# DiltheyLab/MetaMaps

Hardware: AMD Instinct MI355X
Metric: Gbp long reads mapped+classified per sec (whole node), miniSeq+H DB (higher is better)
Workload: dtype u32

## Files before the change

### include/metamaps_hip.h

```cpp
#ifndef METAMAPS_HIP_H
#define METAMAPS_HIP_H

#include <stddef.h>
#include <stdint.h>

#ifdef __cplusplus
extern "C" {
#endif

#define MM_ABI_VERSION 6

typedef enum {
  MM_OK = 0,
  MM_ERR_ARG = -1,
  MM_ERR_DEVICE = -2,
  MM_ERR_NOMEM = -3,
  MM_ERR_STATE = -4,
  MM_ERR_LIMIT = -5,
  MM_ERR_NUMERIC = -6,
  MM_ERR_COMM = -7,
  MM_ERR_DATA = -8
} mm_status;

typedef struct mm_ctx mm_ctx;
// ... 82 lines not shown
} mm_synth_community_params;
int mm_synth_community(mm_ctx* ctx, const mm_synth_community_params* p, mm_seqset** out, int32_t* contig_genome);
int mm_synth_community_species(const mm_synth_community_params* p, int32_t* genome_species);
int mm_synth_reads(mm_ctx* ctx, const mm_seqset* reference, const mm_synth_read_params* p, mm_seqset** out,
                   int32_t* truth_genome);

int mm_minimizers(mm_ctx* ctx, const mm_seqset* s, int k, int w, int64_t* offsets, uint32_t* hash, int32_t* wpos,
                  int32_t* strand, int64_t cap);

typedef struct {
  int64_t n_contigs, n_entries, n_unique_hashes, n_dup_flagged;
  int64_t hbm_bytes;
} mm_index_info;
int mm_index_build(mm_ctx* ctx, const mm_seqset* contigs, int k, int w, mm_index** out);
void mm_index_destroy(mm_index* idx);
int mm_index_save(mm_index* idx, const char* path);
int mm_index_load(mm_ctx* ctx, const char* path, mm_index** out);
int mm_index_plan_chunks(mm_ctx* ctx, const mm_index* whole, uint64_t max_memory_bytes, int32_t* first_contig, int32_t cap, int32_t* n_chunks);
int mm_index_get_info(const mm_index* idx, mm_index_info* out);
int mm_index_freq_hist(mm_index* idx, int64_t* counts, int64_t* n_hashes, int64_t cap, int64_t* n_out);
int mm_freq_threshold_from_hist(const int64_t* counts, const int64_t* n_hashes, int64_t n, int64_t n_unique_hashes,
                                int prev_threshold);
int mm_index_set_freq_threshold(mm_index* idx, int threshold);
int mm_index_entries(mm_index* idx, uint32_t* hash, int32_t* contig, int32_t* wpos, int32_t* strand, int64_t cap);
int mm_index_dup_neighbours(mm_index* idx, int32_t* prev_dist, int32_t* next_dist, int64_t cap);

int mm_recommended_window(double p_value, int k, float pi, int min_read_len, uint64_t reference_size);
double mm_estimate_pvalue(int s, int k, float pi, int min_read_len, uint64_t reference_size);
int mm_min_hits_relaxed(int s, int k, float pi);
void mm_identity(int shared, int s, int k, float* ident, float* ident_upper );

typedef struct {
  int32_t k, w;
  float perc_identity;
  int32_t min_read_len;
} mm_map_params;

typedef struct {
  int32_t read;
  int32_t ref_contig;
  int32_t ref_start;
  int32_t shared;
  int32_t sketch;
  int32_t strand;
  double mapq;
} mm_map_record;

typedef struct {
  int64_t n_reads, n_reads_long_enough, n_reads_mapped, n_mappings;
  int64_t bases_long_enough;
  int64_t sum_sketch, sum_hits, n_candidates, sum_l2_stream_entries, sum_l2_evals;
  int64_t n_ambiguous_sketch_reads;
  int64_t sum_hits_kept;
  int64_t n_l2_rebuilds;
  int64_t n_l2_wide_redo;
  double ms_minimizer, ms_sketch, ms_probe_gather, ms_sort_hits, ms_l1_scan, ms_l2, ms_compact, ms_total, ms_hit_filter;
  int64_t n_reads_giant;
} mm_map_stats;

int mm_map_batch(mm_ctx* ctx, const mm_index* idx, const mm_seqset* reads, const mm_map_params* p, mm_mapping** out);
int mm_map_batch_phased(mm_ctx* ctx, const mm_index* idx, const mm_seqset* reads, const mm_map_params* p, void (*at_stage)(void* user, int stage), void* user,
                        mm_mapping** out);
int mm_map_batch_reusing(mm_ctx* ctx, const mm_index* idx, const mm_seqset* reads, const mm_map_params* p, const mm_mapping* sketch_of, mm_mapping** out);
int mm_sketch_batch(mm_ctx* ctx, const mm_seqset* reads, const mm_map_params* p, mm_mapping** out);
void mm_mapping_destroy(mm_mapping* m);
int mm_mapping_get_stats(const mm_mapping* m, mm_map_stats* out);
int mm_mapping_release_intermediates(mm_mapping* m);
int mm_mapping_fetch(mm_mapping* m, int64_t* offsets, mm_map_record* records, int64_t cap);
int mm_mapping_add_qualities(mm_ctx* ctx, mm_mapping* m, const mm_seqset* reads, int k);
int mm_mapping_keep_best(mm_ctx* ctx, mm_mapping* m, int k);
int mm_mapping_concat(mm_ctx* ctx, mm_mapping* const* parts, const int32_t* contig_base, int n_parts, mm_mapping** out);
int mm_mapping_from_parts(mm_ctx* ctx, int64_t n_reads, const int32_t* read_len, const mm_map_params* p, int n_parts,
                          const int64_t* const* offsets, const mm_map_record* const* records, const int32_t* contig_base, mm_mapping** out);

int mm_mapping_gather(mm_ctx* ctx, int owner, int64_t n_reads, const int32_t* read_len, const mm_map_params* p, mm_mapping* const* parts, const int32_t* chunk_id,
                      int n_parts, int n_chunks, const int32_t* chunk_rank, const int32_t* contig_base, mm_mapping** out);

int mm_debug_sketch(mm_mapping* m, int64_t* offsets, uint32_t* hash, int32_t* strand, int64_t cap);
int mm_debug_hits(mm_mapping* m, int64_t* offsets, int32_t* contig, int32_t* wpos, int64_t cap);
int mm_debug_candidates(mm_mapping* m, int64_t* offsets, int32_t* triples , int64_t cap);
int mm_debug_l2(mm_mapping* m, int64_t* per_cand , int64_t cap);
int mm_debug_min_hits(mm_mapping* m, int32_t* min_hits );
int mm_debug_probed_lists(mm_mapping* m, const mm_index* idx, int64_t* hist, int32_t n_bins);

int mm_em_create(mm_ctx* ctx, int64_t n_reads, const int64_t* read_off, const int32_t* taxon, const double* mapq,
                 const double* inv_nloc, int32_t n_taxa, mm_em** out);
int mm_em_create_from_mapping(mm_ctx* ctx, const mm_mapping* m, const int32_t* contig_taxon, const int32_t* contig_len, int32_t n_contigs,
                              int32_t n_taxa, mm_em** out);
int mm_em_taxon_counts(mm_em* em, int64_t* counts);
int mm_em_sizes(const mm_em* em, int64_t* n_reads, int64_t* n_entries, int32_t* n_taxa);
void mm_em_destroy(mm_em* em);
int mm_em_iterate(mm_em* em, const double* f, double* f_partial, double* ll_partial);
int mm_em_iterate_allreduce(mm_em* em, const double* f, double* f_next, double* ll);
int mm_em_run(mm_em* em, const double* f0, int max_iter, double* f_out, double* ll_trace, int ll_cap, int* n_iter);
int mm_em_continue(mm_em* em, int max_iter, double* f_out, double* ll_trace, int ll_cap, int* n_iter, int* stopped);
int mm_em_posteriors(mm_em* em, const double* f, double* post , int64_t* best );
int mm_em_bootstrap(mm_em* em, const double* f_start, int32_t rep0, int32_t n_rep, uint64_t seed, const uint8_t* weights,
                    int max_iter, double* f_out, double* ll_out, int32_t* n_iter, int32_t* stopped);
int mm_em_lca(mm_em* em, const double* f, int32_t n_nodes, const int32_t* parent, const int32_t* taxon_node, double threshold,
              int32_t* node_out, double* mass_out, int64_t* direct_out);

int mm_gene_overlap(mm_ctx* ctx, int32_t n_contigs, const int64_t* contig_gene_off, const int32_t* gene_start, const int32_t* gene_stop,
                    const int32_t* gene_group, int32_t n_groups,
                    const int64_t* group_feat_off , const int32_t* group_feat, int32_t n_feats,
                    int64_t n_maps, const int32_t* map_contig, const int32_t* map_start, const int32_t* map_stop, const double* map_ident,
                    int64_t* group_reads , double* group_median ,
                    int64_t* feat_reads , int64_t* maps_on_annotated );

int mm_ident_filter(mm_ctx* ctx, int64_t n_reads, const int64_t* read_off , const int32_t* taxon, const double* ident,
                    const int64_t* best , int32_t n_taxa, double thr_percent,
                    double* sorted_max , int64_t* n_with_entries, int64_t* n_le,
                    int64_t* taxon_reads , double* taxon_median , uint8_t* taxon_removed ,
                    uint8_t* read_removed ,
                    int64_t* read_src, int64_t* entry_src, int64_t* read_off_out, int64_t* n_reads_out, int64_t* n_entries_out);

int mm_edit_infix(mm_ctx* ctx, const mm_seqset* reads, const mm_seqset* reference, int64_t n_jobs, const int32_t* read, const int32_t* strand,
                  const int32_t* contig, const int64_t* ws, const int64_t* we, const int32_t* max_dist,
                  int32_t* dist_out, int64_t* begin_out, int64_t* end_out);
int mm_mapping_edit_distances(mm_ctx* ctx, const mm_mapping* mapping, const mm_seqset* reads, const mm_seqset* reference, float perc_identity,
                              int32_t* dist_out, int64_t* first_out, int64_t* last_out, int64_t cap);

int mm_edit_infix_align(mm_ctx* ctx, const mm_seqset* reads, const mm_seqset* reference, int64_t n_jobs, const int32_t* read, const int32_t* strand,
                        const int32_t* contig, const int64_t* ws, const int64_t* we, const int32_t* max_dist, mm_alignment** out);
int mm_mapping_align(mm_ctx* ctx, const mm_mapping* mapping, const mm_seqset* reads, const mm_seqset* reference, float perc_identity, mm_alignment** out);
int mm_alignment_sizes(const mm_alignment* al, int64_t* n_jobs, int64_t* n_ops);
int mm_alignment_fetch(const mm_alignment* al, int32_t* dist , int64_t* first, int64_t* last, int64_t* op_off , uint32_t* ops );
void mm_alignment_destroy(mm_alignment* al);

int mm_bam_encode(mm_ctx* ctx, const mm_seqset* reads, const mm_seqset* reference, int64_t n_jobs,
                  const int32_t* read, const int32_t* strand, const int32_t* contig,
                  const int32_t* dist, const int64_t* first,
                  const int64_t* op_off , const uint32_t* ops,
                  const uint16_t* flag, const uint8_t* mapq,
                  const int64_t* name_off , const char* names,
                  int64_t group_bytes, mm_bam** out);
int mm_bam_sizes(const mm_bam* bam, int64_t* n_records, int64_t* raw_bytes, int64_t* bgzf_bytes);
int mm_bam_fetch(const mm_bam* bam, uint8_t* bgzf );
void mm_bam_destroy(mm_bam* bam);

#define MM_COMM_ID_BYTES 128
int mm_comm_unique_id(char id[MM_COMM_ID_BYTES]);
int mm_comm_init(mm_ctx* ctx, const char id[MM_COMM_ID_BYTES], int rank, int nranks);
int mm_comm_info(mm_ctx* ctx, int* n_ranks, int* rank);
int mm_comm_share(mm_ctx* ctx, mm_ctx* owner);
int mm_comm_allreduce_f64(mm_ctx* ctx, double* host_inout, int64_t n);
void mm_comm_destroy(mm_ctx* ctx);

#ifdef __cplusplus
}
#endif
#endif
```

### metamaps_amd/capi.py

```python
from __future__ import annotations

import ctypes as C
import os
import re

import numpy as np

_HERE = os.path.dirname(os.path.abspath(__file__))
LIB_PATH = os.path.join(_HERE, "csrc", "libmetamaps_hip.so")
HEADER_PATH = os.path.join(os.path.dirname(_HERE), "include", "metamaps_hip.h")

COMM_ID_BYTES = 128
MM_ERR_ARG = -1
MM_ERR_LIMIT = -5
MM_ERR_DATA = -8


class MMError(RuntimeError):
    def __init__(self, status: int, msg: str):
        super().__init__(f"libmetamaps_hip status {status}: {msg}")
        self.status = status


SEED_STAGE_CB = C.CFUNCTYPE(None, C.c_void_p, C.c_int)
# ... 64 lines not shown
            raise FileNotFoundError(f"{path} is missing — run `python -c 'import __graft_entry__ as g; g.build()'`")
        L = C.CDLL(path)
        vp, i32, i64, u64, f32, f64 = C.c_void_p, C.c_int32, C.c_int64, C.c_uint64, C.c_float, C.c_double
        P = C.POINTER
        sig = {
            "mm_abi_version": (C.c_int, []),
            "mm_ctx_release_cached": (C.c_int, [vp]),
            "mm_device_count": (C.c_int, []),
            "mm_ctx_create": (C.c_int, [C.c_int, P(vp)]),
            "mm_ctx_destroy": (None, [vp]),
            "mm_last_error": (C.c_char_p, [vp]),
            "mm_ctx_device_info": (C.c_int, [vp, C.c_char_p, C.c_size_t, P(C.c_int), P(u64), P(u64)]),
            "mm_ctx_synchronize": (C.c_int, [vp]),
            "mm_ctx_stream": (vp, [vp]),
            "mm_seqset_create": (C.c_int, [vp, P(vp)]),
            "mm_seqset_destroy": (None, [vp]),
            "mm_seqset_add": (C.c_int, [vp, C.c_char_p, i64]),
            "mm_seqset_add_view": (C.c_int, [vp, C.c_char_p, i64]),
            "mm_seqset_add_nt16": (C.c_int, [vp, C.c_char_p, i64, C.c_int]),
            "mm_bgzf_inflate": (C.c_int, [vp, C.c_char_p, i64, vp, vp, C.c_int32, vp, i64, vp, vp]),
            "mm_bgzf_deflate_bound": (i64, [i64]),
            "mm_bgzf_deflate": (C.c_int, [vp, C.c_char_p, i64, vp, i64, P(i64), P(C.c_int32)]),
            "mm_gzip_open": (C.c_int, [vp, i64, i64, P(vp)]),
            "mm_gzip_feed": (C.c_int, [vp, C.c_char_p, i64, C.c_int, P(i64)]),
            "mm_gzip_read": (C.c_int, [vp, vp, i64, P(i64)]),
            "mm_gzip_stats": (C.c_int, [vp, P(i64), P(f64)]),
            "mm_gzip_close": (None, [vp]),
            "mm_seqset_save": (C.c_int, [vp, C.c_char_p]),
            "mm_seqset_load": (C.c_int, [vp, C.c_char_p, P(vp)]),
            "mm_seqset_upload": (C.c_int, [vp]),
            "mm_seqset_slice": (C.c_int, [vp, vp, i64, i64, P(vp)]),
            "mm_seqset_concat": (C.c_int, [vp, P(vp), C.c_int, P(vp)]),
            "mm_seqset_count": (i64, [vp]),
            "mm_seqset_total_bases": (i64, [vp]),
            "mm_seqset_lengths": (C.c_int, [vp, vp]),
            "mm_seqset_fetch": (C.c_int, [vp, i64, C.c_char_p, i64]),
            "mm_seqset_fetch_range": (C.c_int, [vp, i64, i64, C.c_void_p, i64]),
            "mm_seqset_hpc": (C.c_int, [vp, vp, P(vp), P(vp)]),
            "mm_hpc_map_to_raw": (C.c_int, [vp, vp, vp, i64, vp, vp]),
            "mm_hpc_map_lengths": (C.c_int, [vp, vp, vp]),
            "mm_hpc_map_device_bytes": (i64, [vp]),
            "mm_mapping_to_raw": (C.c_int, [vp, vp, vp, vp, i64]),
            "mm_hpc_map_destroy": (None, [vp]),
            "mm_synth_reference": (C.c_int, [vp, P(SynthRefParams), P(vp)]),
            "mm_synth_reads": (C.c_int, [vp, vp, P(SynthReadParams), P(vp), vp]),
            "mm_synth_community": (C.c_int, [vp, P(SynthCommunityParams), P(vp), vp]),
            "mm_synth_community_species": (C.c_int, [P(SynthCommunityParams), vp]),
            "mm_minimizers": (C.c_int, [vp, vp, C.c_int, C.c_int, vp, vp, vp, vp, i64]),
            "mm_index_build": (C.c_int, [vp, vp, C.c_int, C.c_int, P(vp)]),
            "mm_index_save": (C.c_int, [vp, C.c_char_p]),
            "mm_index_load": (C.c_int, [vp, C.c_char_p, P(vp)]),
            "mm_index_destroy": (None, [vp]),
            "mm_index_get_info": (C.c_int, [vp, P(IndexInfo)]),
            "mm_index_freq_hist": (C.c_int, [vp, vp, vp, i64, P(i64)]),
            "mm_freq_threshold_from_hist": (C.c_int, [vp, vp, i64, i64, C.c_int]),
            "mm_index_set_freq_threshold": (C.c_int, [vp, C.c_int]),
            "mm_index_entries": (C.c_int, [vp, vp, vp, vp, vp, i64]),
            "mm_index_dup_neighbours": (C.c_int, [vp, vp, vp, i64]),
            "mm_recommended_window": (C.c_int, [f64, C.c_int, f32, C.c_int, u64]),
            "mm_estimate_pvalue": (f64, [C.c_int, C.c_int, f32, C.c_int, u64]),
            "mm_min_hits_relaxed": (C.c_int, [C.c_int, C.c_int, f32]),
            "mm_identity": (None, [C.c_int, C.c_int, C.c_int, P(f32), P(f32)]),
            "mm_map_batch": (C.c_int, [vp, vp, vp, P(MapParams), P(vp)]),
            "mm_map_batch_phased": (C.c_int, [vp, vp, vp, P(MapParams), SEED_STAGE_CB, vp, P(vp)]),
            "mm_map_batch_reusing": (C.c_int, [vp, vp, vp, P(MapParams), vp, P(vp)]),
            "mm_sketch_batch": (C.c_int, [vp, vp, P(MapParams), P(vp)]),
            "mm_mapping_destroy": (None, [vp]),
            "mm_mapping_get_stats": (C.c_int, [vp, P(MapStats)]),
            "mm_comm_info": (C.c_int, [vp, C.POINTER(C.c_int), C.POINTER(C.c_int)]),
            "mm_mapping_gather": (C.c_int, [vp, C.c_int, i64, vp, vp, vp, vp, C.c_int, C.c_int, vp, vp, vp]),
            "mm_mapping_release_intermediates": (C.c_int, [vp]),
            "mm_mapping_fetch": (C.c_int, [vp, vp, vp, i64]),
            "mm_mapping_add_qualities": (C.c_int, [vp, vp, vp, C.c_int]),
            "mm_mapping_concat": (C.c_int, [vp, P(vp), vp, C.c_int, P(vp)]),
            "mm_mapping_keep_best": (C.c_int, [vp, vp, C.c_int]),
            "mm_mapping_from_parts": (C.c_int, [vp, i64, vp, P(MapParams), C.c_int, P(vp), P(vp), vp, P(vp)]),
            "mm_index_plan_chunks": (C.c_int, [vp, vp, u64, vp, i32, P(i32)]),
            "mm_debug_sketch": (C.c_int, [vp, vp, vp, vp, i64]),
            "mm_debug_hits": (C.c_int, [vp, vp, vp, vp, i64]),
            "mm_debug_candidates": (C.c_int, [vp, vp, vp, i64]),
            "mm_debug_l2": (C.c_int, [vp, vp, i64]),
            "mm_debug_min_hits": (C.c_int, [vp, vp]),
            "mm_debug_probed_lists": (C.c_int, [vp, vp, vp, i32]),
            "mm_em_create": (C.c_int, [vp, i64, vp, vp, vp, vp, i32, P(vp)]),
            "mm_em_create_from_mapping": (C.c_int, [vp, vp, vp, vp, i32, i32, P(vp)]),
            "mm_em_taxon_counts": (C.c_int, [vp, vp]),
            "mm_em_sizes": (C.c_int, [vp, P(i64), P(i64), P(i32)]),
            "mm_em_destroy": (None, [vp]),
            "mm_em_iterate": (C.c_int, [vp, vp, vp, P(f64)]),
            "mm_em_iterate_allreduce": (C.c_int, [vp, vp, vp, P(f64)]),
            "mm_em_posteriors": (C.c_int, [vp, vp, vp, vp]),
            "mm_em_run": (C.c_int, [vp, vp, C.c_int, vp, vp, C.c_int, P(C.c_int)]),
            "mm_em_continue": (C.c_int, [vp, C.c_int, vp, vp, C.c_int, P(C.c_int), P(C.c_int)]),
            "mm_em_bootstrap": (C.c_int, [vp, vp, i32, i32, u64, vp, C.c_int, vp, vp, vp, vp]),
            "mm_em_lca": (C.c_int, [vp, vp, i32, vp, vp, f64, vp, vp, vp]),
            "mm_gene_overlap": (C.c_int, [vp, i32, vp, vp, vp, vp, i32, vp, vp, i32, i64, vp, vp, vp, vp, vp, vp, vp, P(i64)]),
            "mm_ident_filter": (C.c_int, [vp, i64, vp, vp, vp, vp, i32, f64, vp, P(i64), P(i64), vp, vp, vp, vp, vp, vp, vp, P(i64), P(i64)]),
            "mm_edit_infix": (C.c_int, [vp, vp, vp, i64, vp, vp, vp, vp, vp, vp, vp, vp, vp]),
            "mm_mapping_edit_distances": (C.c_int, [vp, vp, vp, vp, f32, vp, vp, vp, i64]),
            "mm_edit_infix_align": (C.c_int, [vp, vp, vp, i64, vp, vp, vp, vp, vp, vp, vp]),
            "mm_mapping_align": (C.c_int, [vp, vp, vp, vp, f32, vp]),
            "mm_alignment_sizes": (C.c_int, [vp, vp, vp]),
            "mm_alignment_fetch": (C.c_int, [vp, vp, vp, vp, vp, vp]),
            "mm_alignment_destroy": (None, [vp]),
            "mm_bam_encode": (C.c_int, [vp, vp, vp, i64, vp, vp, vp, vp, vp, vp, vp, vp, vp, vp, vp, i64, vp]),
            "mm_bam_sizes": (C.c_int, [vp, vp, vp, vp]),
            "mm_bam_fetch": (C.c_int, [vp, vp]),
            "mm_bam_destroy": (None, [vp]),
            "mm_comm_unique_id": (C.c_int, [C.c_char_p]),
            "mm_comm_init": (C.c_int, [vp, C.c_char_p, C.c_int, C.c_int]),
            "mm_comm_allreduce_f64": (C.c_int, [vp, vp, i64]),
            "mm_comm_share": (C.c_int, [vp, vp]),
            "mm_comm_destroy": (None, [vp]),
        }
        for name, (res, args) in sig.items():
            fn = getattr(L, name)
            fn.restype = res
            fn.argtypes = args
        _lib = L
    return _lib


def _ptr(a):
    return None if a is None else a.ctypes.data_as(C.c_void_p)


class Context:
    def __init__(self, device: int = 0):
        self.h = C.c_void_p()
        st = lib().mm_ctx_create(device, C.byref(self.h))
        if st != 0:
            raise MMError(st, "mm_ctx_create failed (no gfx950 GPU visible? this library has no CPU fallback)")

    def check(self, st: int):
        if st != 0:
            raise MMError(st, lib().mm_last_error(self.h).decode(errors="replace"))

    def close(self):
        if self.h:
            lib().mm_ctx_destroy(self.h)
            self.h = C.c_void_p()

    def device_info(self) -> dict:
        name = C.create_string_buffer(256)
        cus = C.c_int()
        tot, free = C.c_uint64(), C.c_uint64()
        self.check(lib().mm_ctx_device_info(self.h, name, 256, C.byref(cus), C.byref(tot), C.byref(free)))
        return {"name": name.value.decode(), "cus": cus.value, "hbm_total": tot.value, "hbm_free": free.value}

    def release_cached(self):
        self.check(lib().mm_ctx_release_cached(self.h))

    def synchronize(self):
        self.check(lib().mm_ctx_synchronize(self.h))

    @property
    def stream(self) -> int:
        return lib().mm_ctx_stream(self.h) or 0

    def seqset(self, seqs) -> "SeqSet":
        h = C.c_void_p()
        self.check(lib().mm_seqset_create(self.h, C.byref(h)))
        s = SeqSet(self, h)
        for q in seqs:
            if isinstance(q, str):
                q = q.encode()
# ... 632 lines not shown
```

### metamaps_amd/csrc/mm_api.hip

```cpp
#include "mm_env.hpp"
#include "mm_map.hpp"
#include "mm_em.hpp"
#include "mm_stats.hpp"
#include "mm_synth.hpp"
#include "mm_hpc.hpp"
#include "mm_lca.hpp"
#include "mm_gene.hpp"
#include "mm_ident.hpp"
#include "mm_edit.hpp"
#include "mm_bam.hpp"
#include <chrono>
#include <new>
#include <rccl/rccl.h>
#include "mm_prims.hpp"

namespace mm {
void seqset_upload(mm_seqset* s);
void seqset_upload_nt16(mm_seqset* s);
int64_t bgzf_inflate(mm_ctx* ctx, const uint8_t* comp, int64_t comp_bytes, const int64_t* comp_off, const int32_t* comp_len, int32_t n,
                     uint8_t* out, int64_t out_cap, const int64_t* out_off, int32_t* status);
void bgzf_deflate(mm_ctx* ctx, const uint8_t* in, int64_t in_bytes, uint8_t* out, int64_t out_cap, int64_t* out_bytes, int32_t* n_blocks);
int64_t bgzf_deflate_bound(int64_t in_bytes);
mm_gzip* gzip_open(mm_ctx* ctx, int64_t chunk, int64_t segment);
void gzip_close(mm_gzip* g);
// ... 12 lines not shown
namespace {
void bind(mm_ctx* ctx) {
  if (ctx->device >= 0 && ctx->stream) (void)hipSetDevice(ctx->device);
  mm::current_stream() = ctx->stream; mm::current_alloc() = &ctx->alloc;
}
template <typename F>
int guarded(mm_ctx* ctx, F&& f) {
  if (ctx) bind(ctx);
  try { f(); return MM_OK; }
  catch (const mm::Error& e) { if (ctx) ctx->err = e.what(); return e.status; }
  catch (const std::bad_alloc&) { if (ctx) ctx->err = "host allocation failed"; return MM_ERR_NOMEM; }
  catch (const std::exception& e) { if (ctx) ctx->err = e.what(); return MM_ERR_DEVICE; }
}
}

extern "C" {

int mm_abi_version(void) { return MM_ABI_VERSION; }

namespace {
struct CtxTrace {
  const bool on = getenv("MM_CTX_TRACE") != nullptr;
  std::chrono::steady_clock::time_point t = std::chrono::steady_clock::now();
  void lap(const char* what) {
    if (!on) return;
    const auto n = std::chrono::steady_clock::now();
    fprintf(stderr, "MM_CTX_TRACE %s %.3f ms\n", what, std::chrono::duration<double, std::milli>(n - t).count());
    t = n;
  }
};
}

int mm_device_count(void) {
  int n = 0;
  CtxTrace tr;
  if (hipGetDeviceCount(&n) != hipSuccess) { (void)hipGetLastError(); return 0; }
  tr.lap("hipGetDeviceCount");
  return n;
}
int mm_ctx_create(int device_id, mm_ctx** out) {
  if (!out) return MM_ERR_ARG;
  *out = nullptr;
  if (mm::env_strict()) {
    const std::string bad = mm::env_unknown();
    if (!bad.empty()) { fprintf(stderr, "mm_ctx_create: unknown MM_* environment switch(es): %s (MM_STRICT_ENV is set; the table is metamaps_amd/csrc/mm_env.hpp / INTEGRATION.md)\n", bad.c_str()); return MM_ERR_ARG; }
  }
  int n = 0;
  if (hipGetDeviceCount(&n) != hipSuccess || n <= 0) return MM_ERR_DEVICE;
  if (device_id < 0 || device_id >= n) return MM_ERR_ARG;
  mm_ctx* c = new (std::nothrow) mm_ctx;
  if (!c) return MM_ERR_NOMEM;
  c->device = device_id;
  int st = guarded(c, [&] {
    CtxTrace tr;
    MM_HIP(hipSetDevice(device_id));
    tr.lap("hipSetDevice");
    hipDeviceProp_t p;
    MM_HIP(hipGetDeviceProperties(&p, device_id));
    tr.lap("hipGetDeviceProperties");
    MM_REQUIRE(std::string(p.gcnArchName).rfind("gfx950", 0) == 0, MM_ERR_DEVICE,
               std::string("device is ") + p.gcnArchName + ", this library is built for gfx950 only");
    c->cus = p.multiProcessorCount;
    MM_HIP(hipStreamCreateWithFlags(&c->stream, hipStreamNonBlocking));
    mm::stream_event_register(c->stream);
    tr.lap("hipStreamCreateWithFlags");
    if (tr.on) { void* q = nullptr; if (hipMalloc(&q, 1 << 20) == hipSuccess) { tr.lap("first hipMalloc (1 MiB)"); (void)hipFree(q); } }
    c->alloc.stream = c->stream;
    mm::alloc_register(&c->alloc, c->device);
  });
  if (st != MM_OK) { delete c; return st; }
  *out = c;
  return MM_OK;
}
void mm_ctx_destroy(mm_ctx* ctx) {
  if (!ctx) return;
  mm::alloc_unregister(&ctx->alloc);
  (void)hipSetDevice(ctx->device);
  (void)mm::stream_sync(ctx->stream);
  ctx->alloc.trim();
  mm::big_pool_trim(ctx->device);
  mm::comm_destroy(ctx);
  if (ctx->pinned) (void)hipHostFree(ctx->pinned);
  if (ctx->pinned_up) (void)hipHostFree(ctx->pinned_up);
  ctx->l2_codes.release(); ctx->l2_masks.release();
  if (ctx->ev_fork) (void)hipEventDestroy(ctx->ev_fork);
  if (ctx->ev_join) (void)hipEventDestroy(ctx->ev_join);
  if (ctx->aux_stream) { mm::stream_event_unregister(ctx->aux_stream); (void)hipStreamDestroy(ctx->aux_stream); }
  if (ctx->stream) { mm::stream_event_unregister(ctx->stream); (void)hipStreamDestroy(ctx->stream); }
  delete ctx;
}
const char* mm_last_error(const mm_ctx* ctx) { return ctx ? ctx->err.c_str() : "null context"; }
int mm_ctx_device_info(mm_ctx* ctx, char* name, size_t name_cap, int* cus, uint64_t* hbm_total, uint64_t* hbm_free) {
  if (!ctx) return MM_ERR_ARG;
  return guarded(ctx, [&] {
    MM_HIP(hipSetDevice(ctx->device));
    hipDeviceProp_t p;
    MM_HIP(hipGetDeviceProperties(&p, ctx->device));
    if (name && name_cap) { snprintf(name, name_cap, "%s (%s)", p.name, p.gcnArchName); }
    if (cus) *cus = p.multiProcessorCount;
    size_t f = 0, t = 0;
    MM_HIP(mm::dev_mem_info(&f, &t));
    if (hbm_total) *hbm_total = t;
    if (hbm_free) *hbm_free = f;
  });
}
int mm_ctx_synchronize(mm_ctx* ctx) {
  if (!ctx) return MM_ERR_ARG;
  return guarded(ctx, [&] { MM_HIP(mm::stream_sync(ctx->stream)); });
}
int mm_ctx_release_cached(mm_ctx* ctx) {
  if (!ctx) return MM_ERR_ARG;
  return guarded(ctx, [&] { MM_HIP(hipSetDevice(ctx->device)); ctx->alloc.trim(); mm::big_pool_trim(ctx->device); });
}
void* mm_ctx_stream(mm_ctx* ctx) { return ctx ? (void*)ctx->stream : nullptr; }

int mm_seqset_create(mm_ctx* ctx, mm_seqset** out) {
  if (!ctx || !out) return MM_ERR_ARG;
  return guarded(ctx, [&] { auto* s = new mm_seqset; s->ctx = ctx; *out = s; });
}
void mm_seqset_destroy(mm_seqset* s) { if (s) { bind(s->ctx); delete s; } }
int mm_seqset_add(mm_seqset* s, const char* ascii, int64_t len) {
  if (!s || (!ascii && len > 0) || len < 0) return MM_ERR_ARG;
  return guarded(s->ctx, [&] {
    MM_REQUIRE(!s->frozen, MM_ERR_STATE, "sequence set already uploaded");
    MM_REQUIRE(s->staged_kind != 2, MM_ERR_STATE, "this sequence set holds 4-bit codes (mm_seqset_add_nt16): ASCII cannot join it");
    s->staged_kind = 1;
    s->owned.emplace_back(ascii ? ascii : "", (size_t)len);
    s->staged.emplace_back(s->owned.back().data(), (size_t)len);
  });
}
int mm_seqset_add_view(mm_seqset* s, const char* ascii, int64_t len) {
  if (!s || (!ascii && len > 0) || len < 0) return MM_ERR_ARG;
  return guarded(s->ctx, [&] {
    MM_REQUIRE(!s->frozen, MM_ERR_STATE, "sequence set already uploaded");
    MM_REQUIRE(s->staged_kind != 2, MM_ERR_STATE, "this sequence set holds 4-bit codes (mm_seqset_add_nt16): ASCII cannot join it");
    s->staged_kind = 1;
    s->staged.emplace_back(ascii, (size_t)len);
  });
}
int mm_seqset_add_nt16(mm_seqset* s, const uint8_t* nt16, int64_t n_bases, int reverse) {
  if (!s || (!nt16 && n_bases > 0) || n_bases < 0) return MM_ERR_ARG;
  return guarded(s->ctx, [&] {
    MM_REQUIRE(!s->frozen, MM_ERR_STATE, "sequence set already uploaded");
    MM_REQUIRE(s->staged_kind != 1, MM_ERR_STATE, "this sequence set holds ASCII sequences: 4-bit codes (mm_seqset_add_nt16) cannot join it");
    s->staged_kind = 2;
    s->staged.emplace_back((const char*)nt16, (size_t)n_bases);
    s->staged_rev.push_back(reverse ? 1 : 0);
  });
}
int mm_bgzf_inflate(mm_ctx* ctx, const uint8_t* comp, int64_t comp_bytes, const int64_t* comp_off, const int32_t* comp_len, int32_t n,
                    uint8_t* out, int64_t out_cap, const int64_t* out_off, int32_t* status) {
  if (!ctx || n < 0 || comp_bytes < 0 || out_cap < 0 || (n > 0 && (!comp || !comp_off || !comp_len || !out_off)) || (!out && out_cap > 0)) return MM_ERR_ARG;
  int64_t bad = 0;
  const int rc = guarded(ctx, [&] { MM_HIP(hipSetDevice(ctx->device)); bad = mm::bgzf_inflate(ctx, comp, comp_bytes, comp_off, comp_len, n, out, out_cap, out_off, status); });
  if (rc != MM_OK) return rc;
  if (bad) { ctx->err = "mm_bgzf_inflate: " + std::to_string(bad) + " corrupt BGZF block(s)"; return MM_ERR_DATA; }
  return MM_OK;
}
int64_t mm_bgzf_deflate_bound(int64_t in_bytes) { return in_bytes < 0 ? 0 : mm::bgzf_deflate_bound(in_bytes); }
int mm_bgzf_deflate(mm_ctx* ctx, const uint8_t* in, int64_t in_bytes, uint8_t* out, int64_t out_cap, int64_t* out_bytes, int32_t* n_blocks) {
  if (!ctx || !out_bytes || !n_blocks || in_bytes < 0 || (in_bytes > 0 && (!in || !out))) return MM_ERR_ARG;
  return guarded(ctx, [&] { MM_HIP(hipSetDevice(ctx->device)); mm::bgzf_deflate(ctx, in, in_bytes, out, out_cap, out_bytes, n_blocks); });
}
int mm_gzip_open(mm_ctx* ctx, int64_t chunk_bytes, int64_t segment_bytes, mm_gzip** out) {
  if (!ctx || !out || chunk_bytes < 0 || segment_bytes < 0) return MM_ERR_ARG;
  *out = nullptr;
// ... 566 lines not shown
    m->n_rec = (int64_t)kept.size();
    m->rec.alloc(std::max<size_t>(kept.size(), 1)); m->rec.upload(kept.data(), kept.size(), ctx->stream);
    m->rec_off.upload(off.data(), off.size(), ctx->stream);
    m->h_rec_off = off;
    m->stats.n_mappings = m->n_rec; m->stats.n_reads_mapped = mapped;
    MM_HIP(mm::stream_sync(ctx->stream));
  });
}

int mm_debug_sketch(mm_mapping* m, int64_t* offsets, uint32_t* hash, int32_t* strand, int64_t cap) {
  if (m && m->released) return MM_ERR_STATE;
  if (!m) return MM_ERR_ARG;
  return guarded(m->ctx, [&] {
    hipStream_t st = m->ctx->stream;
    int64_t tot = 0;
    for (int64_t r = 0; r < m->n_reads; ++r) { if (offsets) offsets[r] = tot; tot += m->h_sk_n[(size_t)r]; }
    if (offsets) offsets[m->n_reads] = tot;
    if (!hash && !strand) return;
    MM_REQUIRE(cap >= tot, MM_ERR_ARG, "output capacity too small");
    auto hh = m->sk_hash.to_host(st); auto hs = m->sk_strand.to_host(st);
    int64_t o = 0;
    for (int64_t r = 0; r < m->n_reads; ++r)
      for (int i = 0; i < m->h_sk_n[(size_t)r]; ++i, ++o) {
        size_t src = (size_t)m->mz.h_off[(size_t)r] + (size_t)i;
        if (hash) hash[o] = hh[src];
        if (strand) strand[o] = (hs[src] & 1) ? 1 : -1;
      }
  });
}
int mm_debug_hits(mm_mapping* m, int64_t* offsets, int32_t* contig, int32_t* wpos, int64_t cap) {
  if (m && m->released) return MM_ERR_STATE;
  if (!m) return MM_ERR_ARG;
  return guarded(m->ctx, [&] {
    const int64_t tot = (int64_t)m->h_read_hit_off[(size_t)m->n_reads];
    if (offsets) for (size_t i = 0; i < m->h_read_hit_off.size(); ++i) offsets[i] = (int64_t)m->h_read_hit_off[i];
    if (!contig && !wpos) return;
    MM_REQUIRE(cap >= tot, MM_ERR_ARG, "output capacity too small");
    auto h = m->hits.to_host(m->ctx->stream, (size_t)tot);
    for (int64_t i = 0; i < tot; ++i) {
      if (contig) contig[i] = (int32_t)(h[(size_t)i] >> 32);
      if (wpos) wpos[i] = mm::pw_wpos((uint32_t)h[(size_t)i]);
    }
  });
}
int mm_debug_candidates(mm_mapping* m, int64_t* offsets, int32_t* triples, int64_t cap) {
  if (m && m->released) return MM_ERR_STATE;
  if (!m) return MM_ERR_ARG;
  return guarded(m->ctx, [&] {
    if (offsets) for (size_t i = 0; i < m->h_cand_off.size(); ++i) offsets[i] = (int64_t)m->h_cand_off[i];
    if (!triples) return;
    MM_REQUIRE(cap >= m->n_cand, MM_ERR_ARG, "output capacity too small");
    m->cand.download(triples, (size_t)(3 * m->n_cand), m->ctx->stream);
    MM_HIP(mm::stream_sync(m->ctx->stream));
  });
}
int mm_debug_l2(mm_mapping* m, int64_t* per_cand, int64_t cap) {
  if (m && m->released) return MM_ERR_STATE;
  if (!m || !per_cand) return MM_ERR_ARG;
  return guarded(m->ctx, [&] {
    MM_REQUIRE(cap >= m->n_cand, MM_ERR_ARG, "output capacity too small");
    auto h = m->l2.to_host(m->ctx->stream, (size_t)m->n_cand);
    for (int64_t i = 0; i < m->n_cand; ++i) {
      per_cand[6 * i] = h[(size_t)i].contig; per_cand[6 * i + 1] = h[(size_t)i].mean_pos; per_cand[6 * i + 2] = h[(size_t)i].shared;
      per_cand[6 * i + 3] = h[(size_t)i].opt_beg; per_cand[6 * i + 4] = h[(size_t)i].opt_end; per_cand[6 * i + 5] = h[(size_t)i].accepted;
    }
  });
}
int mm_debug_min_hits(mm_mapping* m, int32_t* min_hits) {
  if (m && m->released) return MM_ERR_STATE;
  if (!m || !min_hits) return MM_ERR_ARG;
  memcpy(min_hits, m->h_min_hits.data(), m->h_min_hits.size() * sizeof(int32_t));
  return MM_OK;
}

int mm_debug_probed_lists(mm_mapping* m, const mm_index* idx, int64_t* hist, int32_t n_bins) {
  if (m && m->released) return MM_ERR_STATE;
  if (!m || !idx || !hist || n_bins < 3) return MM_ERR_ARG;
  return guarded(m->ctx, [&] {
    MM_HIP(hipSetDevice(m->ctx->device));
    mm::probed_list_hist(m->ctx, idx, m, n_bins, hist);
  });
}

int mm_em_create(mm_ctx* ctx, int64_t n_reads, const int64_t* read_off, const int32_t* taxon, const double* mapq, const double* inv_nloc,
                 int32_t n_taxa, mm_em** out) {
  if (!ctx || !read_off || !out || n_reads < 0 || n_taxa <= 0) return MM_ERR_ARG;
  return guarded(ctx, [&] {
    MM_HIP(hipSetDevice(ctx->device));
    auto* E = new mm_em;
    try { mm::em_create(ctx, n_reads, read_off, taxon, mapq, inv_nloc, n_taxa, E); } catch (...) { delete E; throw; }
    *out = E;
  });
}
int mm_em_create_from_mapping(mm_ctx* ctx, const mm_mapping* m, const int32_t* contig_taxon, const int32_t* contig_len, int32_t n_contigs,
                              int32_t n_taxa, mm_em** out) {
  if (!ctx || !m || !contig_taxon || !contig_len || !out || n_contigs < 0 || n_taxa <= 0) return MM_ERR_ARG;
  return guarded(ctx, [&] {
    MM_HIP(hipSetDevice(ctx->device));
    auto* E = new mm_em;
    try { mm::em_create_from_mapping(ctx, m, contig_taxon, contig_len, n_contigs, n_taxa, E); } catch (...) { delete E; throw; }
    *out = E;
  });
}
int mm_em_taxon_counts(mm_em* em, int64_t* counts) {
  if (!em || !counts) return MM_ERR_ARG;
  return guarded(em->ctx, [&] {
    auto ts = em->tstart.to_host(em->ctx->stream, (size_t)em->n_taxa + 1);
    for (int32_t t = 0; t < em->n_taxa; ++t) counts[t] = ts[(size_t)t + 1] - ts[(size_t)t];
  });
}
int mm_em_sizes(const mm_em* em, int64_t* n_reads, int64_t* n_entries, int32_t* n_taxa) {
  if (!em) return MM_ERR_ARG;
  if (n_reads) *n_reads = em->n_reads;
  if (n_entries) *n_entries = em->n_entries;
  if (n_taxa) *n_taxa = em->n_taxa;
  return MM_OK;
}
void mm_em_destroy(mm_em* em) { if (em) { bind(em->ctx); delete em; } }
int mm_em_iterate(mm_em* em, const double* f, double* f_partial, double* ll_partial) {
  if (!em || !f || !f_partial || !ll_partial) return MM_ERR_ARG;
  return guarded(em->ctx, [&] { MM_HIP(hipSetDevice(em->ctx->device)); mm::em_iterate(em, f, f_partial, ll_partial); });
}
int mm_em_iterate_allreduce(mm_em* em, const double* f, double* f_next, double* ll) {
  if (!em || !f || !f_next || !ll) return MM_ERR_ARG;
  return guarded(em->ctx, [&] { MM_HIP(hipSetDevice(em->ctx->device)); mm::em_iterate_allreduce(em, f, f_next, ll); });
}
int mm_em_run(mm_em* em, const double* f0, int max_iter, double* f_out, double* ll_trace, int ll_cap, int* n_iter) {
  if (!em || !f0 || max_iter <= 0 || !n_iter) return MM_ERR_ARG;
  return guarded(em->ctx, [&] { MM_HIP(hipSetDevice(em->ctx->device)); *n_iter = mm::em_run(em, f0, max_iter, f_out, ll_trace, ll_cap, nullptr); });
}
int mm_em_continue(mm_em* em, int max_iter, double* f_out, double* ll_trace, int ll_cap, int* n_iter, int* stopped) {
  if (!em || max_iter <= 0 || !n_iter) return MM_ERR_ARG;
  return guarded(em->ctx, [&] {
    MM_HIP(hipSetDevice(em->ctx->device));
    bool st = false;
    *n_iter = mm::em_run(em, nullptr, max_iter, f_out, ll_trace, ll_cap, &st);
    if (stopped) *stopped = st ? 1 : 0;
  });
}
int mm_em_posteriors(mm_em* em, const double* f, double* post, int64_t* best) {
  if (!em || !f) return MM_ERR_ARG;
  return guarded(em->ctx, [&] { MM_HIP(hipSetDevice(em->ctx->device)); mm::em_posteriors(em, f, post, best); });
}
int mm_em_bootstrap(mm_em* em, const double* f_start, int32_t rep0, int32_t n_rep, uint64_t seed, const uint8_t* weights,
                    int max_iter, double* f_out, double* ll_out, int32_t* n_iter, int32_t* stopped) {
  if (!em || !f_start || n_rep <= 0 || rep0 < 0 || (int64_t)rep0 + n_rep - 1 > INT32_MAX || max_iter <= 0 || !f_out || !ll_out || !n_iter || !stopped) return MM_ERR_ARG;
  return guarded(em->ctx, [&] { MM_HIP(hipSetDevice(em->ctx->device)); mm::boot_run(em, f_start, rep0, n_rep, seed, weights, max_iter, f_out, ll_out, n_iter, stopped); });
}
int mm_em_lca(mm_em* em, const double* f, int32_t n_nodes, const int32_t* parent, const int32_t* taxon_node, double threshold,
              int32_t* node_out, double* mass_out, int64_t* direct_out) {
  if (!em || !f || !parent || !taxon_node || !node_out || n_nodes <= 0) return MM_ERR_ARG;
  return guarded(em->ctx, [&] { MM_HIP(hipSetDevice(em->ctx->device)); mm::lca_run(em, f, n_nodes, parent, taxon_node, threshold, node_out, mass_out, direct_out); });
}
int mm_gene_overlap(mm_ctx* ctx, int32_t n_contigs, const int64_t* contig_gene_off, const int32_t* gene_start, const int32_t* gene_stop,
                    const int32_t* gene_group, int32_t n_groups, const int64_t* group_feat_off, const int32_t* group_feat, int32_t n_feats,
                    int64_t n_maps, const int32_t* map_contig, const int32_t* map_start, const int32_t* map_stop, const double* map_ident,
                    int64_t* group_reads, double* group_median, int64_t* feat_reads, int64_t* maps_on_annotated) {
  if (!ctx) return MM_ERR_ARG;
  return guarded(ctx, [&] {
    MM_HIP(hipSetDevice(ctx->device));
    MM_REQUIRE(n_contigs >= 0 && n_groups >= 0 && n_feats >= 0 && n_maps >= 0 && contig_gene_off && group_feat_off, MM_ERR_ARG, "mm_gene_overlap: a negative size or no offsets");
    const int64_t ng = n_contigs > 0 ? contig_gene_off[n_contigs] : 0;
    MM_REQUIRE((ng <= 0 || (gene_start && gene_stop && gene_group)) && (n_maps == 0 || (map_contig && map_start && map_stop && map_ident)) &&
               (n_groups == 0 || (group_reads && group_median)) && (group_feat_off[n_groups] <= 0 || group_feat), MM_ERR_ARG, "mm_gene_overlap: a null array");
    mm::gene_overlap_run(ctx, mm::GeneIn{n_contigs, contig_gene_off, gene_start, gene_stop, gene_group, n_groups, group_feat_off, group_feat, n_feats,
                                         n_maps, map_contig, map_start, map_stop, map_ident}, group_reads, group_median, feat_reads, maps_on_annotated);
// ... 141 lines not shown
```

### metamaps_amd/csrc/mm_common.hpp

```cpp
#pragma once
#include <hip/hip_runtime.h>
#include <cstdint>
#include <cstdio>
#include <cstdlib>
#include <cstring>
#include <string>
#include <deque>
#include <vector>
#include <stdexcept>
#include <memory>
#include <chrono>
#include <map>
#include <iterator>
#include <mutex>
#include <atomic>
#include <algorithm>
#include "../../include/metamaps_hip.h"
#include "mm_slab.hpp"
#include "task_pool.hpp"
#include "cpu_budget.hpp"

namespace mm {

struct Error : std::runtime_error {
// ... 23 lines not shown
__host__ __device__ inline int32_t pw_strand(uint32_t pw) { return (pw & PW_STRAND) ? 1 : -1; }

__host__ __device__ inline uint64_t rotl64(uint64_t v, int r) { return (v << r) | (v >> (64 - r)); }
__host__ __device__ inline uint64_t fmix64(uint64_t v) {
  v ^= v >> 33; v *= 0xff51afd7ed558ccdULL;
  v ^= v >> 33; v *= 0xc4ceb9fe1a85ec53ULL;
  v ^= v >> 33;
  return v;
}
constexpr uint64_t MUR_C1 = 0x87c37b91114253d5ULL, MUR_C2 = 0x4cf5ad432745937fULL;
constexpr uint32_t MUR_SEED = 42u;

__host__ __device__ inline uint32_t murmur16(uint64_t lo, uint64_t hi) {
  uint64_t a = MUR_SEED, b = MUR_SEED;
  lo *= MUR_C1; lo = rotl64(lo, 31); lo *= MUR_C2; a ^= lo;
  a = rotl64(a, 27); a += b; a = a * 5 + 0x52dce729;
  hi *= MUR_C2; hi = rotl64(hi, 33); hi *= MUR_C1; b ^= hi;
  b = rotl64(b, 31); b += a; b = b * 5 + 0x38495ab5;
  a ^= 16; b ^= 16;
  a += b; b += a;
  a = fmix64(a); b = fmix64(b);
  a += b;
  return (uint32_t)a;
}
template <bool REV>
__host__ __device__ inline uint32_t murmur_bytes(const uint8_t* p, int k) {
  auto at = [&](int i) -> uint64_t { return REV ? p[-i] : p[i]; };
  uint64_t a = MUR_SEED, b = MUR_SEED;
  int nb = k >> 4;
  for (int blk = 0; blk < nb; ++blk) {
    uint64_t lo = 0, hi = 0;
    for (int j = 0; j < 8; ++j) { lo |= at(16 * blk + j) << (8 * j); hi |= at(16 * blk + 8 + j) << (8 * j); }
    lo *= MUR_C1; lo = rotl64(lo, 31); lo *= MUR_C2; a ^= lo;
    a = rotl64(a, 27); a += b; a = a * 5 + 0x52dce729;
    hi *= MUR_C2; hi = rotl64(hi, 33); hi *= MUR_C1; b ^= hi;
    b = rotl64(b, 31); b += a; b = b * 5 + 0x38495ab5;
  }
  int rem = k & 15, base = nb << 4;
  uint64_t lo = 0, hi = 0;
  for (int j = 8; j < rem; ++j) hi |= at(base + j) << (8 * (j - 8));
  if (rem > 8) { hi *= MUR_C2; hi = rotl64(hi, 33); hi *= MUR_C1; b ^= hi; }
  for (int j = 0; j < rem && j < 8; ++j) lo |= at(base + j) << (8 * j);
  if (rem > 0) { lo *= MUR_C1; lo = rotl64(lo, 31); lo *= MUR_C2; a ^= lo; }
  a ^= (uint64_t)k; b ^= (uint64_t)k;
  a += b; b += a;
  a = fmix64(a); b = fmix64(b);
  a += b;
  return (uint32_t)a;
}

__host__ __device__ inline uint8_t ascii_of_code(uint32_t c) {
  return (uint8_t)(0x41 + 2 * (c & 1) + 6 * (c >> 1) + 11 * ((c & 1) & (c >> 1)));
}
__host__ __device__ inline uint8_t complement_ascii(uint8_t c) {
  return c == 'A' ? 'T' : c == 'T' ? 'A' : c == 'C' ? 'G' : c == 'G' ? 'C' : c;
}

inline int64_t ceil_div(int64_t a, int64_t b) { return (a + b - 1) / b; }

}

struct mm_ctx {
  int device = -1;
  hipStream_t stream = nullptr;
  hipStream_t aux_stream = nullptr;
  hipEvent_t ev_fork = nullptr, ev_join = nullptr;
  void aux_ready() {
    if (aux_stream) return;
    MM_HIP(hipStreamCreateWithFlags(&aux_stream, hipStreamNonBlocking));
    mm::stream_event_register(aux_stream);
    MM_HIP(hipEventCreateWithFlags(&ev_fork, hipEventDisableTiming));
    MM_HIP(hipEventCreateWithFlags(&ev_join, hipEventDisableTiming));
  }
  mm::DevAlloc alloc;
  std::string err;
  int cus = 0;
  void* comm = nullptr;
  bool comm_shared = false;
  int comm_rank = 0, comm_size = 1;
  std::shared_ptr<void> lut_cache;
  int lut_k = 0; float lut_pi = 0;
  mm::GrowBuf l2_codes, l2_masks;
  void* pinned = nullptr; size_t pinned_bytes = 0;
  void* pinned_up = nullptr; size_t pinned_up_bytes = 0;
  std::unique_ptr<TaskPool> pack_pool;
  void* pinned_up_at_least(size_t bytes) {
    if (bytes > pinned_up_bytes) {
      if (pinned_up) { MM_HIP(mm::stream_sync(stream)); (void)hipHostFree(pinned_up); }
      pinned_up = nullptr; pinned_up_bytes = 0;
      const size_t want = bytes + bytes / 8;
      MM_HIP(hipHostMalloc(&pinned_up, want, hipHostMallocDefault));
      pinned_up_bytes = want;
    }
    return pinned_up;
  }
  void* pinned_at_least(size_t bytes) {
    if (bytes > pinned_bytes) {
      if (pinned) (void)hipHostFree(pinned);
      pinned = nullptr; pinned_bytes = 0;
      size_t want = bytes + bytes / 2 + (1 << 20);
      MM_HIP(hipHostMalloc(&pinned, want, hipHostMallocDefault));
      pinned_bytes = want;
    }
    return pinned;
  }
};

struct mm_seqset {
  mm_ctx* ctx = nullptr;
  bool frozen = false;
  std::deque<std::string> owned;
  std::vector<std::pair<const char*, size_t>> staged;
  std::vector<uint8_t> staged_rev;
  int staged_kind = 0;
  std::vector<int32_t> len;
  std::vector<uint64_t> base;
  int64_t total_bases = 0;
  mm::DBuf<uint32_t> packed;
  mm::DBuf<uint64_t> d_base;
  mm::DBuf<int32_t> d_len;
  mm::DBuf<uint64_t> exc_start;
  mm::DBuf<uint32_t> exc_len;
  mm::DBuf<uint8_t> exc_byte;
  int64_t n_exc = 0;
  int64_t count() const { return (int64_t)len.size(); }
};
```

### metamaps_amd/csrc/mm_map.hip

```cpp
#include "mm_map.hpp"
#include <functional>
#include <memory>
#include "mm_prims.hpp"
#include "mm_l2_core.hpp"
#include "mm_size_classes.hpp"
#include "mm_l2.hpp"
#include "mm_l2z.hpp"
#include "mm_l2_dense.hpp"
#include <cstdlib>
#include <atomic>
#include <thread>
#include "mm_stats.hpp"
#include <algorithm>
#include <numeric>
#include "mm_sketch.hpp"
#include "mm_seed.hpp"
#include "mm_l1.hpp"

namespace mm {

namespace {
struct HostLap {
  const bool on = getenv("MM_HOST_TIMING") != nullptr; std::chrono::steady_clock::time_point t = std::chrono::steady_clock::now();
  void operator()(const char* what) { if (!on) return; const auto n = std::chrono::steady_clock::now(); fprintf(stderr, "host %-28s %8.1f us\n", what, std::chrono::duration<double, std::micro>(n - t).count()); t = n; }
};

struct ReadBins { std::vector<int32_t> order; std::vector<std::pair<int, size_t>> runs; };
template <typename F>
ReadBins bin_reads(int64_t n, int n_classes, F&& class_of) {
  ReadBins b;
  std::vector<size_t> start((size_t)n_classes + 2, 0);
  std::vector<uint8_t> cls((size_t)std::max<int64_t>(n, 0));
  for (int64_t r = 0; r < n; ++r) { const unsigned c = (unsigned)class_of(r); cls[(size_t)r] = (uint8_t)c; ++start[(size_t)c + 1]; }
  for (int c = 0; c <= n_classes; ++c) start[(size_t)c + 1] += start[(size_t)c];
  b.order.resize((size_t)std::max<int64_t>(n, 0));
  std::vector<size_t> at(start.begin(), start.end() - 1);
  for (int64_t r = 0; r < n; ++r) b.order[at[cls[(size_t)r]]++] = (int32_t)r;
  b.order.resize(start[(size_t)n_classes]);
  for (int c = 0; c < n_classes; ++c) if (start[(size_t)c + 1] > start[(size_t)c]) b.runs.emplace_back(c, start[(size_t)c + 1] - start[(size_t)c]);
  return b;
}

struct HostMz { uint32_t hash; int32_t wpos, strand; };
static bool host_less_by_hash(const HostMz& a, const HostMz& b) { return a.hash < b.hash; }
static bool host_eq_by_hash(const HostMz& a, const HostMz& b) { return a.hash == b.hash; }
}

namespace {
struct StageTimer {
  hipStream_t st;
  std::vector<std::pair<hipEvent_t, hipEvent_t>> ev;
  std::vector<double*> dst;
  explicit StageTimer(hipStream_t s) : st(s) {}
  ~StageTimer() { for (auto& e : ev) { (void)hipEventDestroy(e.first); (void)hipEventDestroy(e.second); } }
  size_t begin(double* target) {
    hipEvent_t a, b;
    MM_HIP(hipEventCreate(&a)); MM_HIP(hipEventCreate(&b));
    ev.push_back({a, b}); dst.push_back(target);
    MM_HIP(hipEventRecord(a, st));
    return ev.size() - 1;
  }
  void end(size_t i) { MM_HIP(hipEventRecord(ev[i].second, st)); }
  void collect() {
    MM_HIP(mm::stream_sync(st));
    for (size_t i = 0; i < ev.size(); ++i) { float ms = 0; MM_HIP(hipEventElapsedTime(&ms, ev[i].first, ev[i].second)); *dst[i] += ms; }
  }
};
}

struct AmbState {
  std::thread bg;
  std::vector<Rec> hr; std::vector<uint64_t> dof; std::vector<int32_t> expect; DBuf<uint64_t> d_so, d_do;
  std::vector<uint8_t> sv; std::vector<int32_t> scnt; std::atomic<int> mismatch{0};
  ~AmbState() { if (bg.joinable()) bg.join(); }
};

namespace {
struct MapSwitches {
  struct OptInt { bool set; int v; };
  static bool on(const char* e) { return e != nullptr; }
  static bool is1(const char* e) { return e && e[0] == '1'; }
  static int num(const char* e, int dflt) { return e ? atoi(e) : dflt; }
  static OptInt opt(const char* e) { return OptInt{e != nullptr, e ? atoi(e) : 0}; }
  const bool eager_tiebreak = on(getenv("MM_EAGER_TIEBREAK"));
  const bool use_filter = !is1(getenv("MM_NO_HIT_FILTER"));
  const bool use_fused = use_filter && !on(getenv("MM_NO_FUSED_FILTER"));
  const int hf_wide_env = num(getenv("MM_HF_WIDE_FROM"), 13000);
  const int hf_wide_from = hf_wide_env > 0 ? hf_wide_env : INT_MAX;
  const OptInt hf_stage_cap = opt(getenv("MM_HF_STAGE_CAP"));
  const int hf_dbg = num(getenv("MM_HF_DBG"), 0);
  const bool sf_prof = on(getenv("MM_SF_PROF"));
  const OptInt sf_grid = opt(getenv("MM_SF_GRID"));
  const OptInt segsort_max_env = opt(getenv("MM_SEGSORT_MAX_KEYS"));
  const uint64_t segsort_max_keys = segsort_max_env.set ? (uint64_t)std::max(segsort_max_env.v, 1) : 0xffffffffull;
  const bool l1_serial = on(getenv("MM_L1_SERIAL"));
  const bool l2_no_fuse = on(getenv("MM_L2_NO_FUSE"));
  const bool l2_no_ranges = on(getenv("MM_L2_NO_RANGES"));
  const bool l2_skip = !is1(getenv("MM_L2_FULL"));
  const int dense_from = num(getenv("MM_L2_DENSE_FROM"), 13000);
  const bool dense_no_stop = on(getenv("MM_L2_DENSE_NO_STOP"));
  const bool no_small_groups = on(getenv("MM_L2_NO_SMALL_GROUPS"));
  const bool dev_groups = l2_skip && !on(getenv("MM_L2_HOST_GROUPS"));
  const bool l2_no_slots = on(getenv("MM_L2_NO_SLOTS"));
  const OptInt l2_slots_env = opt(getenv("MM_L2_SLOTS"));
  const size_t l2_slots = l2_slots_env.set ? ((size_t)std::max(l2_slots_env.v, 1) + 7) / 8 * 8 : 0;
  const bool v2 = !on(getenv("MM_L2_V1"));
  const bool v2_long = v2 && !on(getenv("MM_L2_V1_LONG"));
  const bool sort_groups = !on(getenv("MM_L2_NO_GROUP_SORT"));
  const OptInt group_sort_env = opt(getenv("MM_L2_GROUP_SORT_MIN"));
  const size_t group_sort_from = group_sort_env.set ? (size_t)std::max(group_sort_env.v, 1) : 2048;
  const bool one_stream = on(getenv("MM_L2_ONE_STREAM"));
  const OptInt l2_stop = opt(getenv("MM_L2_STOP"));
  const bool l2_phases = on(getenv("MM_L2_PHASES"));
  const bool force_amb_redo = on(getenv("MM_FORCE_AMB_REDO"));
  const OptInt l2z_dbg = opt(getenv("MM_L2Z_DBG"));
  const bool l2z_force_handback = on(getenv("MM_L2Z_FORCE_HANDBACK"));
  const bool l2z_walk_search = on(getenv("MM_L2Z_WALK_SEARCH"));
  bool has_l2_debug_word() const { return l2_stop.set || l2_phases || force_amb_redo || l2z_dbg.set || l2z_force_handback || l2z_walk_search; }
  unsigned long long l2_debug_word() const {
    int v = l2_stop.set ? l2_stop.v & 0xff : 0;
    if (l2_phases) v |= 0x100;
    if (force_amb_redo) v |= 0x200;
    if (l2z_dbg.set) v |= l2z_dbg.v == 2 ? 0xc00 : 0x400;
    if (l2z_force_handback) v |= 0x1000;
    if (l2z_walk_search) v |= 0x2000;
    return (unsigned long long)v;
  }
};

template <int First, int... Rest, typename F>
void dispatch(int ipt, F&& f) {
  if constexpr (sizeof...(Rest) == 0) f(std::integral_constant<int, First>{});
  else if (ipt == First) f(std::integral_constant<int, First>{});
  else dispatch<Rest...>(ipt, f);
}

void set_lds(const void* fn, size_t bytes) { if (bytes > 64 * 1024) MM_HIP(hipFuncSetAttribute(fn, hipFuncAttributeMaxDynamicSharedMemorySize, (int)bytes)); }

struct MapRun {
  mm_ctx* const ctx; const mm_index* const I; const mm_seqset* const reads; const mm_map_params& P; mm_mapping* const M;
  const hipStream_t st;
  const MapSwitches sw;
  StageTimer T;
  const int64_t n;
  size_t t_total = 0, t_l1 = 0;
  int64_t total_mz = 0, total_hits = 0, ncand = 0;
  HostLap hl;
  std::vector<uint8_t> h_amb;
  std::function<void()> amb_finish;
  std::vector<int64_t> eager_reads, lazy_reads;
  std::vector<std::unique_ptr<AmbState>> amb_states;
  IndexView IV{};
  DBuf<uint32_t> probe_cnt;
  DBuf<uint64_t> probe_start;
  DBuf<uint64_t> hit_off, scan_tmp;
  DBuf<uint8_t> need_old; DBuf<uint32_t> raw_per_read;
  int64_t n_fused = 0, n_wide = 0;
  uint64_t raw_hits = 0;
  DBuf<unsigned long long> raw_sum;
  DBuf<uint32_t> surv;
  DBuf<uint64_t> stage, stage_off;
  const uint8_t* only = nullptr;
  DBuf<uint32_t> cand_n;
  DBuf<int32_t> cand_hint;
  DBuf<int64_t> cand_rng;
  DBuf<int32_t> d_gA0, d_gAn, d_gS0, d_gSn;
  DBuf<unsigned int> grp_ctr;
  std::vector<int32_t> listG; int smG = 0;
  DBuf<unsigned long long> counters;
  DBuf<int32_t> ovf;
  DBuf<unsigned int> ovf_n;
  DBuf<uint8_t> amb_used;
  uint8_t* amb_used_p = nullptr;
  struct SkipClasses {
    DBuf<unsigned int> slot_flags;
    DBuf<int32_t> big;
    DBuf<unsigned int> big_n;
    std::vector<int32_t> gA0, gAn, gB0, gBn, gD0, gDn, listC, gS0, gSn;
    int smA = 0, smB = 0, smC = 0, smD = 0;
    std::vector<int32_t> listL; int smL = 0;
    std::vector<unsigned int> gctr = std::vector<unsigned int>(4, 0);
    size_t nA = 0, nS = 0;
    DBuf<int32_t> d_gB0, d_gBn, d_listC, d_gD0, d_gDn;
    int64_t n_fallback = 0, n_big = 0, n_redo = 0;
  };
  std::unique_ptr<SkipClasses> sk;

  MapRun(mm_ctx* ctx_, const mm_index* I_, const mm_seqset* reads_, const mm_map_params& P_, mm_mapping* M_)
      : ctx(ctx_), I(I_), reads(reads_), P(P_), M(M_), st(ctx_->stream), T(st), n(reads_->count()) {}

  const std::vector<uint64_t>& hoff() const { return M->mz.h_off; }
  int min_mapped_len() const { return P.w + P.k + 1; }
  bool dense_read(int64_t r, int sr) const { return sr >= sw.dense_from && sr < L2_SKETCH_LIMIT && M->read_len[(size_t)r] >= min_mapped_len(); }
  bool filtering() const { return sw.use_filter && n > 0; }

  void begin() {
    MM_REQUIRE(M->sketch_only || (I && I->k == P.k && I->w == P.w), MM_ERR_ARG, "index was built with different k / window size");
    MM_REQUIRE(n < (1LL << 31), MM_ERR_LIMIT, "more than 2^31 reads in one batch");
    M->ctx = ctx; M->n_reads = n; M->params = P; M->stats = mm_map_stats{};
    M->stats.n_reads = n;
    M->read_len = reads->len;
    M->active.assign((size_t)n, 0);
    for (int64_t r = 0; r < n; ++r) {
      int L = reads->len[(size_t)r];
      bool ok = !(L < P.w || L < P.k || L < P.min_read_len);
      M->active[(size_t)r] = ok;
      if (ok) { M->stats.n_reads_long_enough++; M->stats.bases_long_enough += L; }
    }
    t_total = T.begin(&M->stats.ms_total);
  }

  void minimizers() {
    const mm_mapping* const donor = M->sketch_donor;
    if (donor) {
      const size_t t = T.begin(&M->stats.ms_minimizer);
      auto dcopy = [&](auto& dst, const auto& src) { dst.alloc(src.n); if (src.n) MM_HIP(hipMemcpyAsync(dst.p, src.p, src.bytes(), hipMemcpyDeviceToDevice, st)); };
      mm_mapping* const dn = const_cast<mm_mapping*>(donor);
      const bool same_ctx = donor->ctx == ctx;
      if (same_ctx) M->mz.rec.share_from(dn->mz.rec); else dcopy(M->mz.rec, donor->mz.rec);
      dcopy(M->mz.off, donor->mz.off);
      M->mz.h_off = donor->mz.h_off; M->mz.total = donor->mz.total;
      if (same_ctx) M->sk_hash.share_from(dn->sk_hash); else dcopy(M->sk_hash, donor->sk_hash);
      dcopy(M->sk_strand, donor->sk_strand); dcopy(M->sk_n, donor->sk_n); dcopy(M->amb, donor->amb);
      T.end(t);
    } else { size_t t = T.begin(&M->stats.ms_minimizer); run_minimizers(ctx, reads, P.k, P.w, M->active, false, M->mz); T.end(t); }
    total_mz = M->mz.total;
    if (!donor) {
      M->sk_hash.alloc((size_t)std::max<int64_t>(total_mz, 1));
      M->sk_strand.alloc((size_t)std::max<int64_t>(total_mz, 1));
      M->sk_n.alloc((size_t)std::max<int64_t>(n, 1)); M->sk_n.zero(st);
      M->amb.alloc((size_t)std::max<int64_t>(n, 1)); M->amb.zero(st);
    }
  }

  void sketch() {
    if (M->sketch_donor) return;
    size_t t_sk = T.begin(&M->stats.ms_sketch);
    static_assert(ipt_list_is<4, 6, 8, 10, 12, 16, 20, 24, 32, 40, 48, 64>(SKETCH_IPTS), "the dispatch below lists the classes of mm_size_classes.hpp");
    uint64_t big_seen = 0;
    HostLap hl;
    const ReadBins RB = bin_reads(n, N_SKETCH_CLASSES, [&](int64_t r) -> int {
      const uint64_t c = hoff()[(size_t)r + 1] - hoff()[(size_t)r];
      big_seen |= (uint64_t)(c > SKETCH_LDS_MAX);
      return sketch_class_index(c);
    });
    const bool any_big = big_seen != 0;
    {
      hl("K2 bin");
      DBuf<int32_t> list(std::max<size_t>(RB.order.size(), 1));
      list.upload(RB.order.data(), RB.order.size(), st);
      hl("K2 list upload");
      size_t at = 0;
      for (auto& run : RB.runs) {
        const unsigned nb = (unsigned)run.second;
        const int32_t* lp = list.p + at;
        dispatch<4, 6, 8, 10, 12, 16, 20, 24, 32, 40, 48, 64>(SKETCH_IPTS[run.first], [&](auto ipt_tag) {
          constexpr int IPT = decltype(ipt_tag)::value;
          using SortT = rocprim::block_radix_sort<uint32_t, 256, IPT, uint16_t>;
          using ScanT = rocprim::block_scan<int, 256>;
          const size_t lds = std::max(sizeof(typename SortT::storage_type), sizeof(typename ScanT::storage_type)) + 16;
          if (lds > 48 * 1024) MM_HIP(hipFuncSetAttribute((const void*)sketch_radix_kernel<IPT>, hipFuncAttributeMaxDynamicSharedMemorySize, (int)lds));
          sketch_radix_kernel<IPT><<<dim3(nb), dim3(256), lds, st>>>(M->mz.rec.p, M->mz.off.p, lp, M->sk_hash.p, M->sk_strand.p, M->sk_n.p, M->amb.p);
        });
        MM_KERNEL_CHECK();
        at += run.second;
      }
      hl("K2 launches");
      MM_HIP(mm::stream_sync(st));
      hl("K2 sync (kernels)");
    }
    if (any_big) sketch_big_segmented();
    T.end(t_sk);
  }

  void sketch_big_segmented() {
    std::vector<int32_t> big; std::vector<uint64_t> koff{0};
    for (int64_t r = 0; r < n; ++r) { const uint64_t c = hoff()[(size_t)r + 1] - hoff()[(size_t)r]; if (c > SKETCH_LDS_MAX) { big.push_back((int32_t)r); koff.push_back(koff.back() + c); } }
    const size_t nb = big.size(); const uint64_t nk = koff.back();
    MM_REQUIRE(nk < ((uint64_t)1 << 32), MM_ERR_LIMIT, "more than 2^32 minimizers of reads beyond 16384 minimizers in one batch");
    DBuf<int32_t> d_big(nb); d_big.upload(big.data(), nb, st);
    DBuf<uint64_t> d_koff(nb + 1); d_koff.upload(koff.data(), nb + 1, st);
    DBuf<uint64_t> keys((size_t)nk), sorted((size_t)nk);
    sketch_keys_kernel<<<dim3((unsigned)nb), dim3(256), 0, st>>>(M->mz.rec.p, M->mz.off.p, d_big.p, d_koff.p, keys.p);
    MM_KERNEL_CHECK();
    DBuf<uint8_t> tmp;
    with_scratch(tmp, [&](void* t, size_t& b) { return rocprim::segmented_radix_sort_keys(t, b, keys.p, sorted.p, (unsigned int)nk, (unsigned int)nb, d_koff.p, d_koff.p + 1, 0, 64, st); });
    sketch_finish_kernel<<<dim3((unsigned)nb), dim3(256), 0, st>>>(M->mz.rec.p, M->mz.off.p, d_big.p, d_koff.p, sorted.p, M->sk_hash.p, M->sk_strand.p, M->sk_n.p, M->amb.p);
    MM_KERNEL_CHECK();
    MM_HIP(mm::stream_sync(st));
  }

  bool after_sketch() {
    hl.t = std::chrono::steady_clock::now();
    M->h_sk_n = M->sk_n.to_host(st, (size_t)n);
    if (M->sketch_only) {
      for (int64_t r = 0; r < n; ++r) M->stats.sum_sketch += M->h_sk_n[(size_t)r];
      M->h_rec_off.assign((size_t)n + 1, 0); M->n_rec = 0;
      T.end(t_total);
      T.collect();
      return false;
    }
    if (M->at_stage) M->at_stage(M->at_stage_user, 1);
    h_amb = M->amb.to_host(st, (size_t)n);
    hl("post-K2 downloads");
    int64_t giant = 0;
    for (int64_t r = 0; r < n; ++r) if (M->h_sk_n[(size_t)r] >= L2_SKETCH_LIMIT) ++giant;
    M->stats.n_reads_giant = giant;
    return true;
// ... 17 lines not shown
      dof[i + 1] = dof[i] + (hoff()[(size_t)r + 1] - hoff()[(size_t)r]);
      expect[i] = M->h_sk_n[(size_t)r];
    }
    DBuf<uint64_t> d_so(na), d_do(na + 1);
    d_so.upload(so.data(), na, st); d_do.upload(dof.data(), na + 1, st);
    DBuf<Rec> comp((size_t)dof[na]);
    gather_amb_kernel<<<dim3((unsigned)na), dim3(256), 0, st>>>(M->mz.rec.p, d_so.p, d_do.p, comp.p);
    MM_KERNEL_CHECK();
    amb_states.push_back(std::make_unique<AmbState>());
    AmbState* const A = amb_states.back().get();
    A->hr = comp.to_host(st);
    A->dof = dof; A->expect = std::move(expect); A->d_so = std::move(d_so); A->d_do = std::move(d_do);
    A->sv.assign((size_t)dof[na], 0);
    A->scnt.assign(na, 0);
    A->bg = std::thread([A, na]() {
      std::atomic<size_t> next{0};
      auto worker = [&]() {
        std::vector<HostMz> v;
        for (size_t i = next.fetch_add(1); i < na; i = next.fetch_add(1)) {
          const size_t cntr = (size_t)(A->dof[i + 1] - A->dof[i]);
          v.resize(cntr);
          for (size_t j = 0; j < cntr; ++j) { const Rec& x = A->hr[(size_t)A->dof[i] + j]; v[j] = HostMz{x.hash, pw_wpos(x.pw), pw_strand(x.pw)}; }
          std::sort(v.begin(), v.end(), host_less_by_hash);
          auto ue = std::unique(v.begin(), v.end(), host_eq_by_hash);
          const size_t sN = (size_t)(ue - v.begin());
          if ((int64_t)sN != A->expect[i]) A->mismatch = 1;
          for (size_t j = 0; j < sN; ++j) A->sv[(size_t)A->dof[i] + j] = v[j].strand == 1 ? 1 : 0;
          A->scnt[i] = (int32_t)sN;
        }
      };
      const unsigned nthr = std::max(1u, std::min(32u, std::min<unsigned>(mm::cpu_budget(), (unsigned)((na + 15) / 16))));
      std::vector<std::thread> pool;
      for (unsigned t = 1; t < nthr; ++t) pool.emplace_back(worker);
      worker();
      for (auto& t : pool) t.join();
    });
    return [M = M, A, na, st = st]() {
      if (A->bg.joinable()) A->bg.join();
      MM_REQUIRE(A->mismatch == 0, MM_ERR_DEVICE, "sketch size disagrees between device and host tie-break");
      DBuf<uint8_t> d_sv(A->sv.size()); d_sv.upload(A->sv.data(), A->sv.size(), st);
      DBuf<int32_t> d_cnt(na); d_cnt.upload(A->scnt.data(), na, st);
      scatter_strand_kernel<<<dim3((unsigned)na), dim3(256), 0, st>>>(d_sv.p, A->d_so.p, A->d_do.p, d_cnt.p, M->sk_strand.p);
      MM_KERNEL_CHECK();
      MM_HIP(mm::stream_sync(st));
    };
  }
  void finish_tiebreak() { if (amb_finish) { amb_finish(); amb_finish = nullptr; } }

  void thresholds() {
    if (!ctx->lut_cache || ctx->lut_k != P.k || ctx->lut_pi != P.perc_identity) {
      ctx->lut_cache = stats::LutCache::for_params(P.k, P.perc_identity);
      ctx->lut_k = P.k; ctx->lut_pi = P.perc_identity;
    }
    stats::LutCache& lut = *static_cast<stats::LutCache*>(ctx->lut_cache.get());
    std::vector<int32_t> mh((size_t)n, 0), am((size_t)n, 0);
    int smax = 0, s_hi = 0;
    for (int64_t r = 0; r < n; ++r) s_hi = std::max(s_hi, (int)M->h_sk_n[(size_t)r]);
    std::vector<int32_t> slot((size_t)s_hi + 1, -1);
    std::vector<int> sizes;
    for (int64_t r = 0; r < n; ++r) { const int s = M->h_sk_n[(size_t)r]; if (s > 0 && slot[(size_t)s] < 0) { slot[(size_t)s] = (int32_t)sizes.size(); sizes.push_back(s); } }
    const std::vector<stats::SketchLut> luts = lut.get_many(sizes);
    for (int64_t r = 0; r < n; ++r) {
      int s = M->h_sk_n[(size_t)r];
      if (s <= 0) continue;
      const stats::SketchLut L = luts[(size_t)slot[(size_t)s]];
      mh[(size_t)r] = L.min_hits; am[(size_t)r] = L.accept_min;
      if (s < L2_SKETCH_LIMIT) smax = std::max(smax, s);
      M->stats.sum_sketch += s;
    }
    M->smax = smax;
    M->min_hits.alloc((size_t)std::max<int64_t>(n, 1)); M->min_hits.upload(mh.data(), (size_t)n, st);
    M->accept_min.alloc((size_t)std::max<int64_t>(n, 1)); M->accept_min.upload(am.data(), (size_t)n, st);
    M->h_min_hits = mh;
    MM_HIP(mm::stream_sync(st));
    hl("K7 thresholds + uploads");
    M->d_read_len.alloc((size_t)std::max<int64_t>(n, 1));
    M->d_read_len.upload(reads->len.data(), (size_t)n, st);
    IV = make_view(I);
  }

  void seed_hits() {
    probe_cnt.alloc((size_t)total_mz + 1);
    probe_start.alloc((size_t)total_mz + 1);
    if (filtering()) { raw_per_read.alloc((size_t)n); raw_per_read.zero(st); }
    else if (total_mz > 0) probe_cnt.zero(st);
    if (filtering()) {
      std::vector<uint8_t> h_need((size_t)n, 0);
      for (int64_t r = 0; r < n; ++r) {
        const int sr = M->h_sk_n[(size_t)r];
        const uint8_t c = sr > sw.hf_wide_from ? 2 : ((sw.use_fused && sr <= SF_SMAX) ? 0 : 1);
        h_need[(size_t)r] = c; n_fused += c == 0; n_wide += c == 2;
      }
      need_old.alloc((size_t)n + 4); need_old.upload(h_need.data(), (size_t)n, st);
      MM_HIP(mm::stream_sync(st));
    }
    hl("K3 prep (need_old etc.)");
    const size_t t_pg = T.begin(&M->stats.ms_probe_gather);
    M->read_hit_off.alloc((size_t)n + 1);
    raw_sum.alloc(1);
    if (filtering()) seed_stage_and_fused();
    only = filtering() ? need_old.p : nullptr;
    if (n > 0 && total_mz > 0) {
      probe_kernel<<<dim3((unsigned)n), dim3(256), 0, st>>>(IV, M->sk_hash.p, M->mz.off.p, M->sk_n.p, probe_cnt.p, probe_start.p, only);
      MM_KERNEL_CHECK();
    }
    if (!filtering()) {
      hit_off.alloc((size_t)total_mz + 2);
      exclusive_scan_u32_u64(probe_cnt.p, total_mz, hit_off.p, scan_tmp, st);
      MM_HIP(hipMemcpyAsync(&raw_hits, hit_off.p + total_mz, sizeof raw_hits, hipMemcpyDeviceToHost, st));
    }
    if (filtering()) {
      const bool time_old = !(sw.use_fused && n_fused > 0);
      const size_t t_hf = time_old ? T.begin(&M->stats.ms_hit_filter) : 0;
      launch_hit_filter<false>(nullptr, nullptr, sw.hf_dbg, raw_per_read.p);
      if (time_old) T.end(t_hf);
      raw_sum.zero(st);
      sum_u32_kernel<<<dim3(256), dim3(256), 0, st>>>(raw_per_read.p, n, raw_sum.p);
      MM_KERNEL_CHECK();
      MM_HIP(hipMemcpyAsync(&raw_hits, raw_sum.p, sizeof raw_hits, hipMemcpyDeviceToHost, st));
      exclusive_scan_u32_u64(surv.p, n, M->read_hit_off.p, scan_tmp, st);
    } else {
      read_hit_bounds_kernel<<<dim3((unsigned)ceil_div(n + 1, 256)), dim3(256), 0, st>>>(M->mz.off.p, hit_off.p, n, M->read_hit_off.p);
      MM_KERNEL_CHECK();
    }
    hl("K3 launches");
    M->h_read_hit_off = M->read_hit_off.to_host(st);
    hl("K3 wait + hit_off download");
    total_hits = (int64_t)M->h_read_hit_off[(size_t)n];
    M->stats.sum_hits = (int64_t)raw_hits;
    M->stats.sum_hits_kept = total_hits;
    M->hits.alloc((size_t)std::max<int64_t>(total_hits, 1));
    if (total_hits > 0) {
      if (sw.use_filter) launch_hit_filter<true>(M->read_hit_off.p, M->hits.p, 100, nullptr);
      else {
        gather_hits_kernel<<<dim3((unsigned)n), dim3(256), 0, st>>>(IV, M->mz.off.p, M->sk_n.p, probe_cnt.p, probe_start.p, hit_off.p, M->hits.p);
        MM_KERNEL_CHECK();
      }
    }
    T.end(t_pg);
  }

  template <bool WRITE>
  void launch_hit_filter(const uint64_t* hit_off_p, uint64_t* hits_p, int dbg, uint32_t* raw_p) {
    using HfN = HitFilterCfg<HF_SLOT_BITS_NARROW>; using HfW = HitFilterCfg<HF_SLOT_BITS_WIDE>;
    hit_filter_kernel<WRITE, HF_SLOT_BITS_NARROW><<<dim3((unsigned)n), dim3(HfN::THREADS), HfN::LDS, st>>>(IV, M->mz.off.p, M->sk_n.p, probe_cnt.p, probe_start.p, M->d_read_len.p,
                                                                   M->min_hits.p, surv.p, hit_off_p, hits_p, stage.p, stage_off.p, dbg, only, raw_p);
    if (n_wide > 0) {
      MM_KERNEL_CHECK();
      MM_HIP(hipFuncSetAttribute((const void*)hit_filter_kernel<WRITE, HF_SLOT_BITS_WIDE>, hipFuncAttributeMaxDynamicSharedMemorySize, (int)HfW::LDS));
      hit_filter_kernel<WRITE, HF_SLOT_BITS_WIDE><<<dim3((unsigned)n), dim3(HfW::THREADS), HfW::LDS, st>>>(IV, M->mz.off.p, M->sk_n.p, probe_cnt.p, probe_start.p, M->d_read_len.p,
                                                                   M->min_hits.p, surv.p, hit_off_p, hits_p, stage.p, stage_off.p, dbg, only, raw_p);
    }
    MM_KERNEL_CHECK();
  }

  void seed_stage_and_fused() {
    surv.alloc((size_t)n + 1); surv.zero(st);
    std::vector<uint64_t> h_stage_off((size_t)n + 1, 0);
    for (int64_t r = 0; r < n; ++r)
      h_stage_off[(size_t)r + 1] = h_stage_off[(size_t)r] + (M->h_sk_n[(size_t)r] > 0 ? (sw.hf_stage_cap.set ? (uint64_t)sw.hf_stage_cap.v : 1024 + 2 * (uint64_t)M->h_sk_n[(size_t)r]) : 0);
    stage_off.alloc((size_t)n + 1); stage_off.upload(h_stage_off.data(), h_stage_off.size(), st);
    stage.alloc((size_t)std::max<uint64_t>(h_stage_off[(size_t)n], 1));
    MM_HIP(mm::stream_sync(st));
    hl("K3 stage_off loop + upload");
    if (!(sw.use_fused && n_fused > 0)) return;
    const size_t lds = sizeof(SeedFilterStreamLds);
    MM_HIP(hipFuncSetAttribute((const void*)seed_filter_stream_kernel<false>, hipFuncAttributeMaxDynamicSharedMemorySize, (int)lds));
    MM_HIP(hipFuncSetAttribute((const void*)seed_filter_stream_kernel<true>, hipFuncAttributeMaxDynamicSharedMemorySize, (int)lds));
    DBuf<uint32_t> sf_ticket(1);
    sf_ticket.zero(st);
    DBuf<unsigned long long> sf_prof;
    if (sw.sf_prof) { sf_prof.alloc(16); sf_prof.zero(st); }
    int sf_grid = (int)std::min<int64_t>(n, std::max(ctx->cus, 1));
    if (sw.sf_grid.set) sf_grid = std::max(1, std::min(sf_grid, sw.sf_grid.v));
    const size_t t_sf = T.begin(&M->stats.ms_hit_filter);
    if (sf_prof.p)
      seed_filter_stream_kernel<true><<<dim3((unsigned)sf_grid), dim3(SF_THREADS), lds, st>>>(IV, M->sk_hash.p, M->mz.off.p, M->sk_n.p, M->d_read_len.p, M->min_hits.p, surv.p, stage.p, stage_off.p,
                                                                         need_old.p, reinterpret_cast<const uint32_t*>(need_old.p), raw_per_read.p, (int)n, sf_ticket.p, sf_prof.p);
    else
      seed_filter_stream_kernel<false><<<dim3((unsigned)sf_grid), dim3(SF_THREADS), lds, st>>>(IV, M->sk_hash.p, M->mz.off.p, M->sk_n.p, M->d_read_len.p, M->min_hits.p, surv.p, stage.p, stage_off.p,
                                                                         need_old.p, reinterpret_cast<const uint32_t*>(need_old.p), raw_per_read.p, (int)n, sf_ticket.p, nullptr);
    MM_KERNEL_CHECK();
    T.end(t_sf);
    if (sf_prof.p) {
      auto h = sf_prof.to_host(st);
      const double tot = (double)std::accumulate(h.begin(), h.end(), 0ull);
      fprintf(stderr, "MM_SF_PROF share of cycles: zero+top %.3f | next head + resolve %.3f | scan %.3f | lists+count %.3f | window sums+alive+issue %.3f | phase 2 %.3f | survivors+end %.3f | total %.3g cycles over %d workgroups\n",
              h[0] / tot, (h[1] + h[7]) / tot, h[2] / tot, (h[3] + h[8]) / tot, (h[4] + h[9] + h[10] + h[11]) / tot, (h[5] + h[12]) / tot, h[6] / tot, tot, sf_grid);
      fprintf(stderr, "MM_SF_PROF in detail: top %.3f | first answers + second probes issued %.3f, their answers %.3f | scan %.3f | pieces loaded, counted, parked %.3f, next hashes asked for + barrier %.3f | "
                      "window sums %.3f, alive %.3f, barrier %.3f, hashes there + look-ups issued %.3f | bit tests + slots %.3f, barrier %.3f | survivors+end %.3f\n",
              h[0] / tot, h[7] / tot, h[1] / tot, h[2] / tot, h[8] / tot, h[3] / tot, h[9] / tot, h[10] / tot, h[4] / tot, h[11] / tot, h[12] / tot, h[5] / tot, h[6] / tot);
    }
  }

  int64_t hits_of(int64_t r) const { return (int64_t)(M->h_read_hit_off[(size_t)r + 1] - M->h_read_hit_off[(size_t)r]); }

  void sort_hits() {
    if (total_hits > 0) {
      const size_t t_sh = T.begin(&M->stats.ms_sort_hits);
      hl("K4 hits alloc + emit launch");
      int key_bits = 32; while (key_bits < 64 && ((int64_t)1 << (key_bits - 32)) < I->n_contigs) ++key_bits;
      if (sort_hits_radix(key_bits)) sort_hits_segmented(key_bits);
      T.end(t_sh);
    }
    hl("K4 launches + sync");
  }

  bool sort_hits_radix(int key_bits) {
    static_assert(ipt_list_is<1, 2, 3, 4, 6, 8, 12, 16>(HIT_SORT_IPTS), "the dispatch below lists the classes of mm_size_classes.hpp");
    uint64_t left_seen = 0;
    const ReadBins RB = bin_reads(n, N_HIT_SORT_CLASSES, [&](int64_t r) -> int {
      const uint64_t c = (uint64_t)hits_of(r);
      left_seen |= (uint64_t)(c > HIT_SORT_LDS_MAX);
      return hit_sort_class_index(c);
    });
    hl("K4 bin");
    DBuf<int32_t> list(std::max<size_t>(RB.order.size(), 1));
    list.upload(RB.order.data(), RB.order.size(), st);
    hl("K4 list upload");
    size_t at = 0;
    for (auto& run : RB.runs) {
      const int32_t* lp = list.p + at;
      dispatch<1, 2, 3, 4, 6, 8, 12, 16>(HIT_SORT_IPTS[run.first], [&](auto tag) {
        constexpr int IPT = decltype(tag)::value;
        using SortT = rocprim::block_radix_sort<uint64_t, 256, IPT>;
        const size_t lds = sizeof(typename SortT::storage_type) + 16;
        if (lds > 48 * 1024) MM_HIP(hipFuncSetAttribute((const void*)sort_hits_radix_kernel<IPT>, hipFuncAttributeMaxDynamicSharedMemorySize, (int)lds));
        sort_hits_radix_kernel<IPT><<<dim3((unsigned)run.second), dim3(256), lds, st>>>(M->hits.p, M->read_hit_off.p, lp, key_bits, sw.use_filter ? stage.p : nullptr, sw.use_filter ? stage_off.p : nullptr);
      });
      MM_KERNEL_CHECK();
      at += run.second;
    }
    MM_HIP(mm::stream_sync(st));
    return left_seen != 0;
  }

  void sort_hits_segmented(int key_bits) {
    const uint64_t max_keys = sw.segsort_max_keys;
    std::vector<int32_t> seg_reads;
    std::vector<uint64_t> hb, he, cb, ce;
    std::vector<size_t> run_at{0};
    uint64_t in_run = 0, longest_run = 0;
    for (int64_t r = 0; r < n; ++r) {
      const uint64_t c = (uint64_t)hits_of(r);
      if (c <= HIT_SORT_LDS_MAX) continue;
      MM_REQUIRE(c < max_keys, MM_ERR_LIMIT, "one read has more seed hits than a segmented sort takes (2^32 - 1, or MM_SEGSORT_MAX_KEYS)");
      if (in_run + c >= max_keys) { run_at.push_back(seg_reads.size()); in_run = 0; }
      seg_reads.push_back((int32_t)r);
      hb.push_back(M->h_read_hit_off[(size_t)r]); he.push_back(M->h_read_hit_off[(size_t)r + 1]);
      cb.push_back(in_run); in_run += c; ce.push_back(in_run);
      longest_run = std::max(longest_run, in_run);
    }
    const size_t ns = seg_reads.size();
    run_at.push_back(ns);
    const bool compact = run_at.size() > 2 || 2 * longest_run <= (uint64_t)total_hits || (uint64_t)total_hits >= max_keys;
    DBuf<uint64_t> d_hb(ns), d_he(ns), d_cb(ns), d_ce(ns);
    d_hb.upload(hb.data(), ns, st); d_he.upload(he.data(), ns, st);
    auto seg_sort = [&](uint64_t* in, uint64_t* out, uint64_t count, size_t nseg, uint64_t* begins, uint64_t* ends) {
      with_scratch([&](void* t, size_t& b) { return rocprim::segmented_radix_sort_keys(t, b, in, out, (unsigned int)count, (unsigned int)nseg, begins, ends, 0, key_bits, st); });
    };
    if (compact) {
      d_cb.upload(cb.data(), ns, st); d_ce.upload(ce.data(), ns, st);
      DBuf<uint64_t> packed((size_t)longest_run), sorted((size_t)longest_run);
      for (size_t k = 0; k + 1 < run_at.size(); ++k) {
        const size_t i0 = run_at[k], nr = run_at[k + 1] - i0;
        move_ranges_kernel<<<dim3((unsigned)nr), dim3(256), 0, st>>>(M->hits.p, d_hb.p + i0, d_he.p + i0, packed.p, d_cb.p + i0);
        MM_KERNEL_CHECK();
        seg_sort(packed.p, sorted.p, ce[i0 + nr - 1], nr, d_cb.p + i0, d_ce.p + i0);
        move_ranges_kernel<<<dim3((unsigned)nr), dim3(256), 0, st>>>(sorted.p, d_cb.p + i0, d_ce.p + i0, M->hits.p, d_hb.p + i0);
        MM_KERNEL_CHECK();
      }
      MM_HIP(mm::stream_sync(st));
    } else {
      DBuf<uint64_t> sorted((size_t)total_hits);
      seg_sort(M->hits.p, sorted.p, (uint64_t)total_hits, ns, d_hb.p, d_he.p);
      move_ranges_kernel<<<dim3((unsigned)ns), dim3(256), 0, st>>>(sorted.p, d_hb.p, d_he.p, M->hits.p, d_hb.p);
      MM_KERNEL_CHECK();
      MM_HIP(mm::stream_sync(st));
    }
  }

  void l1_candidates() {
    t_l1 = T.begin(&M->stats.ms_l1_scan);
    cand_n.alloc((size_t)n + 1); cand_n.zero(st);
    M->cand_off.alloc((size_t)n + 2);
    const unsigned rblk = (unsigned)ceil_div(std::max<int64_t>(n, 1), 128);
    if (n > 0) {
      if (sw.l1_serial) l1_scan_kernel<false><<<dim3(rblk), dim3(128), 0, st>>>(M->hits.p, M->read_hit_off.p, M->d_read_len.p, M->min_hits.p, n, cand_n.p, nullptr, nullptr, nullptr);
      else l1_wave_kernel<false><<<dim3((unsigned)ceil_div(n, 4)), dim3(256), 0, st>>>(M->hits.p, M->read_hit_off.p, M->d_read_len.p, M->min_hits.p, n, cand_n.p, nullptr, nullptr, nullptr, nullptr);
      MM_KERNEL_CHECK();
    }
    exclusive_scan_u32_u64(cand_n.p, n, M->cand_off.p, scan_tmp, st);
    M->h_cand_off = M->cand_off.to_host(st, (size_t)n + 1);
    hl("L1 count + cand_off download");
    ncand = (int64_t)M->h_cand_off[(size_t)n];
    M->n_cand = ncand;
    M->stats.n_candidates = ncand;
    MM_REQUIRE(ncand < (1LL << 31), MM_ERR_LIMIT, "more than 2^31 L1 candidates in one batch");
    M->cand.alloc((size_t)std::max<int64_t>(3 * ncand, 1));
    M->cand_read.alloc((size_t)std::max<int64_t>(ncand, 1));
    M->l2.alloc((size_t)std::max<int64_t>(ncand, 1));
    cand_hint.alloc((size_t)std::max<int64_t>(ncand, 1));
    const bool no_hint = sw.l1_serial || sw.l2_no_fuse;
    if (no_hint) cand_hint.zero(st);
    M->rec_off.alloc((size_t)n + 1);
    if (ncand == 0) return;
    if (sw.l1_serial) l1_scan_kernel<true><<<dim3(rblk), dim3(128), 0, st>>>(M->hits.p, M->read_hit_off.p, M->d_read_len.p, M->min_hits.p, n, nullptr, M->cand_off.p, M->cand.p, M->cand_read.p);
    else l1_wave_kernel<true><<<dim3((unsigned)ceil_div(n, 4)), dim3(256), 0, st>>>(M->hits.p, M->read_hit_off.p, M->d_read_len.p, M->min_hits.p, n, nullptr, M->cand_off.p, M->cand.p, M->cand_read.p, no_hint ? nullptr : cand_hint.p);
    MM_KERNEL_CHECK();
    T.end(t_l1);
  }

  template <bool SKIP, typename CNT, int NW, int NWQ>
  void launch_l2(size_t grid, hipStream_t s, int sm, const int32_t* g0, const int32_t* gn, const int32_t* list, uint8_t* amb_ptr, void* codes, uint8_t* masks, int n_slots) {
    const size_t lds = l2_lds_bytes<CNT>(sm, SKIP, NW, NWQ);
    set_lds((const void*)l2_kernel<SKIP, CNT, NW, NWQ>, lds);
    l2_kernel<SKIP, CNT, NW, NWQ><<<dim3((unsigned)grid), dim3(64 * NW), lds, s>>>(IV, M->cand.p, M->cand_read.p, M->sk_hash.p, M->sk_strand.p,
        M->mz.off.p, M->sk_n.p, M->d_read_len.p, M->accept_min.p, P.k, P.w, sm, M->l2.p, counters.p, g0, gn, list, SKIP ? ovf.p : nullptr, SKIP ? ovf_n.p : nullptr, amb_ptr,
        codes, masks, SKIP ? slot_flags_p() : nullptr, n_slots);
    MM_KERNEL_CHECK();
  }
  template <int NW, int NWQ, bool QLDS>
  void launch_l2z(size_t grid, hipStream_t s, int sm, const int32_t* g0, const int32_t* gn, void* lists, uint8_t* masks, int n_slots) {
    const int bbl = l2z_bloom_log2(sm);
    const size_t lds = l2z_lds_bytes(sm, NWQ, QLDS, bbl, NW);
    set_lds((const void*)l2z_kernel<NW, NWQ, QLDS>, lds);
    l2z_kernel<NW, NWQ, QLDS><<<dim3((unsigned)grid), dim3(64 * NW), lds, s>>>(IV, M->cand.p, M->cand_read.p, M->sk_hash.p, M->sk_strand.p, M->mz.off.p, M->sk_n.p, M->d_read_len.p,
        M->accept_min.p, P.k, P.w, sm, bbl, M->l2.p, counters.p, g0, gn, ovf.p, ovf_n.p, sk->big.p, sk->big_n.p, amb_used_p, (uint32_t*)lists, masks, slot_flags_p(), n_slots, cand_hint.p, cand_rng.p);
    MM_KERNEL_CHECK();
  }
  void launch_l2_wide(const int32_t* list, size_t nl, int sm, uint8_t* amb_ptr) {
    launch_l2<true, uint16_t, 1, 8>(nl, st, sm, nullptr, nullptr, list, amb_ptr, nullptr, masks_for(nl), (int)slots_of(nl));
  }
  void launch_l2_full(const int32_t* list, size_t nl, uint8_t* amb_ptr) {
    launch_l2<false, uint16_t, 1, 8>(nl, st, M->smax, nullptr, nullptr, list, amb_ptr, nullptr, nullptr, 0);
  }

  unsigned int* slot_flags_p() const { return sw.l2_no_slots ? nullptr : sk->slot_flags.p; }
  size_t max_slots(int nwq) const { return sw.l2_no_slots ? (size_t)1 << 40 : sw.l2_slots ? sw.l2_slots : (size_t)ctx->cus * (nwq == 2 ? 64 : 32); }
  size_t slots_of(size_t n_waves, int nwq = 8) const { return std::min((std::max<size_t>(n_waves, 1) + 7) / 8 * 8, max_slots(nwq)); }
  uint8_t* masks_for(size_t n_waves, int nwq = 8) { return (uint8_t*)ctx->l2_masks.at_least(ctx->alloc, slots_of(n_waves, nwq) * l2_skip_bytes(nwq)); }
  void* codes_for(size_t n_waves, int nwq) {
    return ctx->l2_codes.at_least(ctx->alloc, slots_of(n_waves, nwq) * (size_t)(64 * 64 * nwq) * (nwq == 2 ? sizeof(uint16_t) : sizeof(uint32_t)));
  }
  void* lists_for(size_t n_waves, int nwq) { return ctx->l2_codes.at_least(ctx->alloc, slots_of(n_waves, nwq) * l2z_list_bytes(nwq)); }
  uint8_t* zmasks_for(size_t n_waves, int nwq) { return (uint8_t*)ctx->l2_masks.at_least(ctx->alloc, slots_of(n_waves, nwq) * l2z_mask_bytes(nwq)); }

  void l2() {
    l2_setup();
    const size_t t_l2 = T.begin(&M->stats.ms_l2);
    l2_dense_beyond_limit();
    if (!sw.l2_skip) l2_full_slide(); else l2_skip_classes();
    l2_stats_kernel<<<dim3((unsigned)std::min<int64_t>(ceil_div(ncand, 256), 1024)), dim3(256), 0, st>>>(M->l2.p, ncand, counters.p);
    MM_KERNEL_CHECK();
    T.end(t_l2);
    hl("K5 wait");
    auto hc = counters.to_host(st);
    M->stats.sum_l2_stream_entries = (int64_t)hc[0];
    M->stats.sum_l2_evals = (int64_t)hc[1];
    M->stats.n_l2_rebuilds = (int64_t)hc[2];
    if (sw.l2_phases) { fprintf(stderr, "l2 rounds %llu zone passes %llu; ", hc[15], hc[12]); fprintf(stderr, "l2 phase clocks [setup passA bounds rebuild slide passB vote]:"); for (int i = 0; i < 7; ++i) fprintf(stderr, " %.3g", (double)hc[3 + i]); fprintf(stderr, "\n"); }
  }

  void l2_setup() {
    if (!sw.l2_no_ranges) {
      cand_rng.alloc(2 * (size_t)ncand);
      l2_ranges_kernel<<<dim3((unsigned)ceil_div(ncand, 256)), dim3(256), 0, st>>>(IV, M->cand.p, M->cand_read.p, M->d_read_len.p, ncand, cand_rng.p);
      MM_KERNEL_CHECK();
    }
    grp_ctr.alloc(4);
    if (sw.dev_groups) {
      d_gA0.alloc((size_t)ncand); d_gAn.alloc((size_t)ncand); d_gS0.alloc((size_t)ncand); d_gSn.alloc((size_t)ncand);
      grp_ctr.zero(st);
      l2_group_kernel<<<dim3((unsigned)ceil_div(n, 256)), dim3(256), 0, st>>>(M->cand_off.p, M->sk_n.p, M->d_read_len.p, n, min_mapped_len(), sw.dense_from,
                                                                            sw.no_small_groups ? 1 : 0, d_gA0.p, d_gAn.p, d_gS0.p, d_gSn.p, grp_ctr.p);
      MM_KERNEL_CHECK();
    }
    const size_t lds_wide = l2_lds_bytes<uint16_t>(M->smax, sw.l2_skip, 1, 8);
    for (int64_t r = 0; r < n && M->stats.n_reads_giant > 0; ++r) {
      const int sr = M->h_sk_n[(size_t)r];
      if (sr < L2_SKETCH_LIMIT) continue;
      smG = std::max(smG, sr);
      for (uint64_t c0 = M->h_cand_off[(size_t)r]; c0 < M->h_cand_off[(size_t)r + 1]; ++c0) listG.push_back((int32_t)c0);
    }
    MM_REQUIRE(lds_wide <= 160 * 1024, MM_ERR_LIMIT, "L2 window state does not fit LDS");
    counters.alloc(16); counters.zero(st);
    if (sw.has_l2_debug_word()) {
      const unsigned long long v = sw.l2_debug_word();
      MM_HIP(hipMemcpyAsync(counters.p + 11, &v, sizeof v, hipMemcpyHostToDevice, st));
      MM_HIP(mm::stream_sync(st));
    }
    ovf.alloc((size_t)ncand);
    ovf_n.alloc(1); ovf_n.zero(st);
    if (!lazy_reads.empty()) { amb_used.alloc((size_t)n); amb_used.zero(st); }
    amb_used_p = lazy_reads.empty() ? nullptr : amb_used.p;
    finish_tiebreak();
  }

  void l2_dense(const std::vector<int32_t>& list, int smax_l, uint8_t* amb_ptr) {
    if (list.empty()) return;
    const size_t nl = list.size();
    DBuf<int32_t> d_list(nl); d_list.upload(list.data(), nl, st);
    DBuf<L2Range> d_rng(nl);
    l2_range_kernel<<<dim3((unsigned)ceil_div((int64_t)nl, 4)), dim3(256), 0, st>>>(IV, M->cand.p, M->cand_read.p, M->d_read_len.p, d_list.p, (int)nl, d_rng.p);
    MM_KERNEL_CHECK();
    std::vector<L2Range> rng = d_rng.to_host(st);
    std::vector<uint64_t> coff(nl + 1, 0);
    for (size_t i = 0; i < nl; ++i) coff[i + 1] = coff[i] + (uint64_t)std::max(rng[i].m, 0);
    std::vector<int32_t> cr = M->cand_read.to_host(st, (size_t)ncand);
    std::vector<int32_t> gfirst;
    for (size_t i = 0; i < nl; ++i) if (i == 0 || cr[(size_t)list[i]] != cr[(size_t)list[i - 1]]) gfirst.push_back((int32_t)i);
    gfirst.push_back((int32_t)nl);
    DBuf<uint64_t> d_coff(nl + 1); d_coff.upload(coff.data(), nl + 1, st);
    DBuf<int32_t> d_gf(gfirst.size()); d_gf.upload(gfirst.data(), gfirst.size(), st);
    DBuf<uint32_t> codes((size_t)std::max<uint64_t>(coff[nl], 1));
    const int q_in_lds = smax_l <= LD_Q_LDS_MAX ? 1 : 0;
    const size_t lds = ((size_t)((LD_TSIZE + 3) & ~3) + (q_in_lds ? (size_t)smax_l + 4 : 0)) * 4;
    set_lds((const void*)l2_codes_kernel, lds);
    l2_codes_kernel<<<dim3((unsigned)(gfirst.size() - 1)), dim3(256), lds, st>>>(IV, M->cand_read.p, M->sk_hash.p, M->mz.off.p, M->sk_n.p, d_list.p, d_gf.p,
                                                                                d_rng.p, d_coff.p, codes.p, q_in_lds);
    MM_KERNEL_CHECK();
    const unsigned slots = (unsigned)std::min<size_t>(nl, (size_t)ctx->cus * 12);
    DBuf<uint32_t> scratch((size_t)slots * l2_dense_slot_words(smax_l));
    DBuf<unsigned int> next(1); next.zero(st);
    l2_dense_kernel<<<dim3(slots), dim3(64), 0, st>>>(IV, M->cand.p, M->cand_read.p, M->sk_strand.p, M->mz.off.p, M->sk_n.p, M->d_read_len.p, M->accept_min.p,
                                                    P.k, P.w, smax_l, M->l2.p, d_list.p, (int)nl, d_rng.p, d_coff.p, codes.p, scratch.p, next.p, amb_ptr, sw.force_amb_redo ? 1 : 0,
                                                    sw.dense_no_stop ? 0 : 1);
    MM_KERNEL_CHECK();
    MM_HIP(mm::stream_sync(st));
  }

  void l2_dense_beyond_limit() { l2_dense(listG, smG, amb_used_p); }

  void l2_full_slide() {
    std::vector<int32_t> listF;
    for (int64_t r = 0; r < n; ++r) if (M->h_sk_n[(size_t)r] < L2_SKETCH_LIMIT)
      for (uint64_t c0 = M->h_cand_off[(size_t)r]; c0 < M->h_cand_off[(size_t)r + 1]; ++c0) listF.push_back((int32_t)c0);
    DBuf<int32_t> d_listF(listF.size());
    if (!listF.empty()) {
      d_listF.upload(listF.data(), listF.size(), st);
      launch_l2_full(d_listF.p, listF.size(), amb_used_p);
    }
    MM_HIP(mm::stream_sync(st));
  }

  void l2_skip_classes() {
    sk = std::make_unique<SkipClasses>();
    sk->slot_flags.alloc(std::max((size_t)ctx->cus * 64, sw.l2_slots)); sk->slot_flags.zero(st);
    sk->big.alloc((size_t)(sw.v2 ? ncand : 1));
    sk->big_n.alloc(1); sk->big_n.zero(st);
    l2_host_groups();
    l2_dense(sk->listL, sk->smL, amb_used_p);
    sk->d_gB0.alloc(sk->gB0.size()); sk->d_gBn.alloc(sk->gBn.size()); sk->d_listC.alloc(sk->listC.size());
    sk->nA = sk->gctr[0]; sk->nS = sk->gctr[1];
    if (!sw.dev_groups) {
      const size_t nA = sk->nA = sk->gA0.size(), nS = sk->nS = sk->gS0.size();
      d_gA0.alloc(std::max<size_t>(nA, 1)); d_gAn.alloc(std::max<size_t>(nA, 1)); d_gS0.alloc(std::max<size_t>(nS, 1)); d_gSn.alloc(std::max<size_t>(nS, 1));
      d_gA0.upload(sk->gA0.data(), nA, st); d_gAn.upload(sk->gAn.data(), nA, st); d_gS0.upload(sk->gS0.data(), nS, st); d_gSn.upload(sk->gSn.data(), nS, st);
    }
    sort_by_position(d_gA0, d_gAn, sk->nA);
    sort_by_position(d_gS0, d_gSn, sk->nS);
    l2_short_class();
    l2_long_class(sk->gB0, sk->gBn, sk->d_gB0, sk->d_gBn, sk->smB);
    sk->d_gD0.alloc(sk->gD0.size()); sk->d_gDn.alloc(sk->gDn.size());
    l2_long_class(sk->gD0, sk->gDn, sk->d_gD0, sk->d_gDn, sk->smD);
    if (!sk->listC.empty()) {
      sk->d_listC.upload(sk->listC.data(), sk->listC.size(), st);
      launch_l2_wide(sk->d_listC.p, sk->listC.size(), sk->smC, amb_used_p);
    }
    hl("K5 uploads + launches");
    if (M->at_stage) M->at_stage(M->at_stage_user, 2);
    l2_handbacks();
    l2_redo_ambiguous();
    M->stats.n_l2_wide_redo = sk->n_redo + sk->n_fallback + sk->n_big;
    sk.reset();
  }

  void l2_host_groups() {
    SkipClasses& s = *sk;
    hl("K5 prep before grouping");
    if (sw.dev_groups) s.gctr = grp_ctr.to_host(st);
    s.smA = (int)s.gctr[3];
    for (int64_t r = 0; r < n && (!sw.dev_groups || s.gctr[2] > 0); ++r) {
      const uint64_t c_lo = M->h_cand_off[(size_t)r], c_hi = M->h_cand_off[(size_t)r + 1];
      if (c_lo == c_hi) continue;
      const int sr = M->h_sk_n[(size_t)r];
      if (sw.dev_groups && sr <= 3072 && !dense_read(r, sr)) continue;
      if (dense_read(r, sr)) {
        s.smL = std::max(s.smL, sr);
        for (uint64_t c0 = c_lo; c0 < c_hi; ++c0) s.listL.push_back((int32_t)c0);
        continue;
      }
      if (sr <= 7168) {
        auto& g0 = sr <= 3072 ? s.gA0 : s.gB0; auto& gn = sr <= 3072 ? s.gAn : s.gBn;
        (sr <= 3072 ? s.smA : s.smB) = std::max(sr <= 3072 ? s.smA : s.smB, sr);
        for (uint64_t c0 = c_lo; c0 < c_hi; c0 += 4) {
          const int32_t cnt = (int32_t)std::min<uint64_t>(4, c_hi - c0);
          if (sr <= 3072 && cnt <= 2 && !sw.no_small_groups) { s.gS0.push_back((int32_t)c0); s.gSn.push_back(cnt); }
          else { g0.push_back((int32_t)c0); gn.push_back(cnt); }
        }
      } else if (sr <= 16384) {
        s.smD = std::max(s.smD, sr);
        for (uint64_t c0 = c_lo; c0 < c_hi; c0 += 4) { s.gD0.push_back((int32_t)c0); s.gDn.push_back((int32_t)std::min<uint64_t>(4, c_hi - c0)); }
      } else if (sr < L2_SKETCH_LIMIT) {
        s.smC = std::max(s.smC, sr);
        for (uint64_t c0 = c_lo; c0 < c_hi; ++c0) s.listC.push_back((int32_t)c0);
      }
    }
    hl("K5 grouping");
  }

  void sort_by_position(DBuf<int32_t>& g0, DBuf<int32_t>& gn, size_t ng) {
    if (!sw.sort_groups || ng < sw.group_sort_from || I->n_contigs <= 0) return;
    DBuf<uint64_t> key(ng), val(ng), key2(ng), val2(ng);
    l2_group_keys_kernel<<<dim3((unsigned)ceil_div((int64_t)ng, 256)), dim3(256), 0, st>>>(g0.p, gn.p, M->cand.p, (int64_t)ng, key.p, val.p);
    int cbits = 1; while (cbits < 31 && ((int64_t)1 << cbits) < I->n_contigs) ++cbits;
    DBuf<uint8_t> tmp;
    sort_pairs(tmp, key.p, key2.p, val.p, val2.p, ng, 12, 32 + cbits, st);
    l2_group_unpack_kernel<<<dim3((unsigned)ceil_div((int64_t)ng, 256)), dim3(256), 0, st>>>(val2.p, (int64_t)ng, g0.p, gn.p);
    MM_KERNEL_CHECK();
  }

  void l2_short_class() {
    const size_t nA = sk->nA, nS = sk->nS; const int smA = sk->smA;
    const bool side_by_side = nA && nS && !sw.l2_no_slots && !sw.one_stream;
    const size_t n_waves = side_by_side ? nA * 4 + nS * 2 : std::max(nA * 4, nS * 2);
    void* const codes = !(nA || nS) ? nullptr : sw.v2 ? lists_for(n_waves, 2) : codes_for(n_waves, 2);
    uint8_t* const masks = !(nA || nS) ? nullptr : sw.v2 ? zmasks_for(n_waves, 2) : masks_for(n_waves, 2);
    const int n_slots = (int)slots_of(n_waves, 2);
    hipStream_t st_small = st;
    if (side_by_side) {
      ctx->aux_ready();
      st_small = ctx->aux_stream;
      MM_HIP(hipEventRecord(ctx->ev_fork, st));
      MM_HIP(hipStreamWaitEvent(st_small, ctx->ev_fork, 0));
    }
    if (sw.v2) {
      if (nA) launch_l2z<4, 2, true>(nA, st, smA, d_gA0.p, d_gAn.p, codes, masks, n_slots);
      if (nS) launch_l2z<2, 2, false>(nS, st_small, smA, d_gS0.p, d_gSn.p, codes, masks, n_slots);
    } else {
      if (nA) launch_l2<true, uint8_t, 4, 2>(nA, st, smA, d_gA0.p, d_gAn.p, nullptr, amb_used_p, codes, masks, n_slots);
      if (nS) launch_l2<true, uint8_t, 2, 2>(nS, st_small, smA, d_gS0.p, d_gSn.p, nullptr, amb_used_p, codes, masks, n_slots);
    }
    if (side_by_side) {
      MM_HIP(hipEventRecord(ctx->ev_join, st_small));
      MM_HIP(hipStreamWaitEvent(st, ctx->ev_join, 0));
    }
  }

  void l2_long_class(const std::vector<int32_t>& g0, const std::vector<int32_t>& gn, DBuf<int32_t>& d_g0, DBuf<int32_t>& d_gn, int sm) {
    if (g0.empty()) return;
    const size_t ng = g0.size();
    d_g0.upload(g0.data(), ng, st); d_gn.upload(gn.data(), gn.size(), st);
    sort_by_position(d_g0, d_gn, ng);
    if (sw.v2_long) launch_l2z<4, 8, false>(ng, st, sm, d_g0.p, d_gn.p, lists_for(ng * 4, 8), zmasks_for(ng * 4, 8), (int)slots_of(ng * 4));
    else launch_l2<true, uint8_t, 4, 8>(ng, st, sm, d_g0.p, d_gn.p, nullptr, amb_used_p, codes_for(ng * 4, 8), masks_for(ng * 4), (int)slots_of(ng * 4));
  }

  void l2_fallback(uint8_t* amb_ptr, bool read_ovf, unsigned int h_ovf) {
    if (read_ovf) {
      MM_HIP(hipMemcpyAsync(&h_ovf, ovf_n.p, sizeof h_ovf, hipMemcpyDeviceToHost, st));
      MM_HIP(mm::stream_sync(st));
    }
    if (!h_ovf) return;
    launch_l2_full(ovf.p, h_ovf, amb_ptr);
    ovf_n.zero(st);
    sk->n_fallback += h_ovf;
  }

  void l2_handbacks() {
    unsigned int h_ovf0 = 0;
    if (sw.v2) {
      unsigned int h_big = 0;
      MM_HIP(hipMemcpyAsync(&h_big, sk->big_n.p, sizeof h_big, hipMemcpyDeviceToHost, st));
      MM_HIP(hipMemcpyAsync(&h_ovf0, ovf_n.p, sizeof h_ovf0, hipMemcpyDeviceToHost, st));
      MM_HIP(mm::stream_sync(st));
      if (h_big) {
        launch_l2_wide(sk->big.p, h_big, std::max(std::max(sk->smA, sk->smB), sk->smD), amb_used_p);
        sk->n_big = h_big;
      }
    }
    l2_fallback(amb_used_p, !sw.v2, h_ovf0);
  }

  void l2_redo_ambiguous() {
    if (lazy_reads.empty()) return;
    std::vector<uint8_t> used = amb_used.to_host(st, (size_t)n);
    std::vector<int64_t> fix;
    for (int64_t r : lazy_reads) if (used[(size_t)r]) fix.push_back(r);
    if (fix.empty()) return;
    start_tiebreak(fix)();
    std::vector<int32_t> redo, redoL; int smR = 0, smRL = 0;
    for (int64_t r : fix) {
      const int sr = M->h_sk_n[(size_t)r];
      const bool dense_r = sr >= L2_SKETCH_LIMIT || (sr >= sw.dense_from && M->read_len[(size_t)r] >= min_mapped_len());
      (dense_r ? smRL : smR) = std::max(dense_r ? smRL : smR, sr);
      for (uint64_t c0 = M->h_cand_off[(size_t)r]; c0 < M->h_cand_off[(size_t)r + 1]; ++c0) (dense_r ? redoL : redo).push_back((int32_t)c0);
    }
    l2_dense(redoL, smRL, nullptr);
    sk->n_redo += (int64_t)redoL.size();
    DBuf<int32_t> d_redo(std::max<size_t>(redo.size(), 1)); d_redo.upload(redo.data(), redo.size(), st);
    if (!redo.empty()) {
      launch_l2_wide(d_redo.p, redo.size(), smR, nullptr);
      l2_fallback(nullptr, true, 0);
    }
    MM_HIP(mm::stream_sync(st));
    sk->n_redo += (int64_t)redo.size();
  }

  void compact() {
    finish_tiebreak();
    const size_t t_cp = T.begin(&M->stats.ms_compact);
    DBuf<uint32_t> flag((size_t)ncand);
    DBuf<uint64_t> rank((size_t)ncand + 1);
    accept_flags_kernel<<<dim3((unsigned)ceil_div(ncand, 256)), dim3(256), 0, st>>>(M->l2.p, ncand, flag.p);
    MM_KERNEL_CHECK();
    exclusive_scan_u32_u64(flag.p, ncand, rank.p, scan_tmp, st);
    uint64_t nrec = 0;
    MM_HIP(hipMemcpyAsync(&nrec, rank.p + ncand, sizeof nrec, hipMemcpyDeviceToHost, st));
    MM_HIP(mm::stream_sync(st));
    M->n_rec = (int64_t)nrec;
    M->rec.alloc((size_t)std::max<uint64_t>(nrec, 1));
    write_records_kernel<<<dim3((unsigned)ceil_div(ncand, 256)), dim3(256), 0, st>>>(M->l2.p, M->cand_read.p, M->sk_n.p, flag.p, rank.p, ncand, M->rec.p);
    MM_KERNEL_CHECK();
    read_rec_bounds_kernel<<<dim3((unsigned)ceil_div(n + 1, 256)), dim3(256), 0, st>>>(M->cand_off.p, rank.p, n, M->rec_off.p);
    MM_KERNEL_CHECK();
    T.end(t_cp);
    MM_HIP(mm::stream_sync(st));
  }

  void no_candidates() {
    T.end(t_l1);
    finish_tiebreak();
    M->n_rec = 0;
    M->rec.alloc(1);
    M->rec_off.zero(st);
    MM_HIP(mm::stream_sync(st));
  }

  void finish() {
    M->h_rec_off = M->rec_off.to_host(st, (size_t)n + 1);
    T.end(t_total);
    T.collect();
    M->stats.n_mappings = M->n_rec;
    for (int64_t r = 0; r < n; ++r) if (M->h_rec_off[(size_t)r + 1] > M->h_rec_off[(size_t)r]) M->stats.n_reads_mapped++;
  }
};
}

void map_batch(mm_ctx* ctx, const mm_index* I, const mm_seqset* reads, const mm_map_params& P, mm_mapping* M) {
  MapRun R(ctx, I, reads, P, M);
  R.begin();
  R.minimizers();
  R.sketch();
  if (!R.after_sketch()) return;
  R.tiebreak_lists();
  R.thresholds();
  R.seed_hits();
  R.sort_hits();
  R.l1_candidates();
  if (R.ncand > 0) { R.l2(); R.compact(); } else R.no_candidates();
  R.finish();
}

void probed_list_hist(mm_ctx* ctx, const mm_index* I, const mm_mapping* M, int nb, int64_t* hist) {
  hipStream_t st = ctx->stream;
  DBuf<unsigned long long> d((size_t)nb);
  d.zero(st);
  if (M->n_reads > 0)
    probed_list_hist_kernel<<<dim3((unsigned)M->n_reads), dim3(256), 0, st>>>(make_view(I), M->sk_hash.p, M->mz.off.p, M->sk_n.p, nb, d.p);
  MM_KERNEL_CHECK();
  auto h = d.to_host(st);
  for (int i = 0; i < nb; ++i) hist[i] = (int64_t)h[(size_t)i];
}

}
```

### metamaps_amd/csrc/mm_minimizer.hpp

```cpp
#pragma once
#include <type_traits>
#include "mm_common.hpp"
#include "mm_scan.hpp"

namespace mm {

constexpr int MZ_THREADS = 256;
constexpr int MZ_TILE = 2048;
constexpr int MZ_MAX_W = 4096;
constexpr int MZ_STAGE = 1024;
constexpr int MZ_MAX_K = 64;

struct SeqView {
  const uint32_t* packed;
  const uint64_t* base;
  const int32_t* len;
  const uint64_t* exc_start;
  const uint32_t* exc_len;
  const uint8_t* exc_byte;
  int64_t n_exc;
  int64_t n;
};

__device__ inline uint32_t code_at(const SeqView& S, uint64_t g) { return (S.packed[g >> 4] >> (2 * (g & 15))) & 3u; }
// ... 277 lines not shown
    }
    cps[j] = c;
  }
  __syncthreads();
  if (dbgs == 3) { if (MODE != 1 && tid == 0) tile_count[tile] = 0; return; }
  const int js = jstar[s];
  const int j0 = (P0 - H0) + tid * (MZ_TILE / MZ_THREADS);
  uint32_t mask = 0;
  static_assert(MZ_TILE / MZ_THREADS == 8, "eight positions per thread");
  bool fast = false;
  if (w >= 2 && j0 + 8 <= np && H0 + j0 - 1 >= w - 1 && j0 >= 1) {
    const uint2 fw = *reinterpret_cast<const uint2*>(flg + j0);
    const uint32_t fprev = flg[j0 - 1];
    fast = (fw.x & fw.y & 0x01010101u) == 0x01010101u && (fprev & 1u);
    if (fast) {
      const uint4 cw = *reinterpret_cast<const uint4*>(cps + j0);
      const uint32_t cprev = cps[j0 - 1];
      const uint32_t c[9] = {cprev, cw.x & 0xffffu, cw.x >> 16, cw.y & 0xffffu, cw.y >> 16, cw.z & 0xffffu, cw.z >> 16, cw.w & 0xffffu, cw.w >> 16};
#pragma unroll
      for (int i = 0; i < 8; ++i) {
        const int p = H0 + j0 + i;
        const bool emit = c[i] != c[i + 1] && !(p > w - 1 && p < js);
        mask |= (emit ? 1u : 0u) << i;
      }
    }
  }
  if (!fast) {
#pragma unroll
  for (int i = 0; i < MZ_TILE / MZ_THREADS; ++i) {
    int j = j0 + i, p = H0 + j;
    if (j < np && p >= w - 1 && (flg[j] & 1)) {
      int pj = -1;
      const int qlo = max(max(j - w + 1, 0), (w - 1) - H0);
      for (int q = j - 1; q >= qlo; --q) if (flg[q] & 1) { pj = q; break; }
      bool emit = (pj < 0) || (cps[pj] != cps[j]);
      if (p > w - 1 && p < js) emit = false;
      if (emit) mask |= 1u << i;
    }
  }
  }
  const uint32_t cnt = __popc(mask);
  uint64_t tot;
  uint64_t ex = block_excl_scan_u64(cnt, &tot);
  if (dbgs == 4) { if (MODE != 1 && tid == 0) tile_count[tile] = 0; return; }
  if (MODE != 1 && tid == 0) tile_count[tile] = (uint32_t)tot;
  if (MODE == 2 && tot > MZ_STAGE) { if (tid == 0) atomicExch(stage_overflow, 1); return; }
  if (MODE != 0) {
    uint64_t o = (MODE == 1 ? tile_out[tile] : tile * (uint64_t)MZ_STAGE) + ex;
#pragma unroll
    for (int i = 0; i < MZ_TILE / MZ_THREADS; ++i) {
      if (mask & (1u << i)) {
        int j = j0 + i, p = H0 + j, c = cps[j];
        uint32_t pw = ((uint32_t)(p - w + 1) << PW_SHIFT) | ((flg[c] & 2) ? PW_STRAND : 0u);
        out[o] = Rec{hsh[c], pw};
        if (out_seq) out_seq[o] = (uint32_t)s;
        ++o;
      }
    }
  }
}

static __global__ void __launch_bounds__(256) compact_tiles_kernel(const Rec* __restrict__ stage, const uint32_t* __restrict__ tile_count,
                                                                   const uint64_t* __restrict__ tile_out, Rec* __restrict__ out) {
  const uint64_t tile = blockIdx.x;
  const uint32_t n = tile_count[tile];
  const uint64_t o = tile_out[tile];
  for (uint32_t i = threadIdx.x; i < n; i += 256) out[o + i] = stage[tile * (uint64_t)MZ_STAGE + i];
}

inline size_t minimizer_lds_bytes(int k, int w) {
  int halo = (2 * (w - 1) + 7) & ~7, NP = MZ_TILE + halo, NB = ((NP + k - 1 + 8) + 15) & ~15;
  return (size_t)2 * NB + (size_t)NP * 4 + (size_t)NP * 2 + (size_t)NP;
}

struct MinimizerSet {
  DBuf<Rec> rec;
  DBuf<uint64_t> off;
  DBuf<uint32_t> rec_seq;
  std::vector<uint64_t> h_off;
  int64_t total = 0;
};

void run_minimizers(mm_ctx* ctx, const mm_seqset* S, int k, int w, const std::vector<uint8_t>& active, bool want_rec_seq,
                    MinimizerSet& out);

SeqView make_view(const mm_seqset* S);

}
```

### metamaps_amd/csrc/mm_scan.hpp

```cpp
#pragma once
#include "mm_common.hpp"

namespace mm {

constexpr int SCAN_THREADS = 256;
constexpr int SCAN_ITEMS = 8;
constexpr int SCAN_TILE = SCAN_THREADS * SCAN_ITEMS;

__device__ inline uint64_t wave_incl_scan_u64(uint64_t v) {
  const int lane = threadIdx.x & 63;
#pragma unroll
  for (int d = 1; d < 64; d <<= 1) {
    uint64_t o = __shfl_up(v, d, 64);
    if (lane >= d) v += o;
  }
  return v;
}

__device__ inline uint64_t block_excl_scan_u64(uint64_t v, uint64_t* total) {
  __shared__ uint64_t wsum[SCAN_THREADS / 64];
  const int lane = threadIdx.x & 63, wid = threadIdx.x >> 6;
  uint64_t inc = wave_incl_scan_u64(v);
  if (lane == 63) wsum[wid] = inc;
  __syncthreads();
  uint64_t base = 0, tot = 0;
#pragma unroll
  for (int i = 0; i < SCAN_THREADS / 64; ++i) { if (i < wid) base += wsum[i]; tot += wsum[i]; }
  __syncthreads();
  if (total) *total = tot;
  return base + inc - v;
}

static __global__ void __launch_bounds__(SCAN_THREADS) scan_reduce_kernel(const uint32_t* __restrict__ in, int64_t n, uint64_t* __restrict__ tile_sum) {
  int64_t base = (int64_t)blockIdx.x * SCAN_TILE;
  uint64_t s = 0;
#pragma unroll
  for (int i = 0; i < SCAN_ITEMS; ++i) {
    int64_t j = base + (int64_t)i * SCAN_THREADS + threadIdx.x;
    if (j < n) s += in[j];
  }
  uint64_t tot;
  block_excl_scan_u64(s, &tot);
  if (threadIdx.x == 0) tile_sum[blockIdx.x] = tot;
}

static __global__ void __launch_bounds__(SCAN_THREADS) scan_tiles_kernel(uint64_t* __restrict__ tile_sum, int64_t ntiles, uint64_t* __restrict__ grand) {
  uint64_t carry = 0;
  for (int64_t base = 0; base < ntiles; base += SCAN_THREADS) {
    int64_t j = base + threadIdx.x;
    uint64_t v = j < ntiles ? tile_sum[j] : 0;
    uint64_t tot;
    uint64_t ex = block_excl_scan_u64(v, &tot);
    if (j < ntiles) tile_sum[j] = carry + ex;
    carry += tot;
    __syncthreads();
  }
  if (threadIdx.x == 0 && grand) *grand = carry;
}

static __global__ void __launch_bounds__(SCAN_THREADS) scan_apply_kernel(const uint32_t* __restrict__ in, int64_t n, const uint64_t* __restrict__ tile_sum,
                                                                  uint64_t* __restrict__ out) {
  int64_t base = (int64_t)blockIdx.x * SCAN_TILE + (int64_t)threadIdx.x * SCAN_ITEMS;
  uint32_t v[SCAN_ITEMS];
  uint64_t s = 0;
#pragma unroll
  for (int i = 0; i < SCAN_ITEMS; ++i) { int64_t j = base + i; v[i] = j < n ? in[j] : 0u; s += v[i]; }
  uint64_t ex = block_excl_scan_u64(s, nullptr) + tile_sum[blockIdx.x];
#pragma unroll
  for (int i = 0; i < SCAN_ITEMS; ++i) { int64_t j = base + i; if (j < n) out[j] = ex; ex += v[i]; }
}

inline void exclusive_scan_u32_u64(const uint32_t* in, int64_t n, uint64_t* out, DBuf<uint64_t>& tile_tmp, hipStream_t st) {
  if (n <= 0) { MM_HIP(hipMemsetAsync(out, 0, sizeof(uint64_t), st)); return; }
  int64_t ntiles = ceil_div(n, SCAN_TILE);
  if ((int64_t)tile_tmp.n < ntiles) tile_tmp.alloc((size_t)ntiles);
  scan_reduce_kernel<<<dim3((unsigned)ntiles), dim3(SCAN_THREADS), 0, st>>>(in, n, tile_tmp.p);
  MM_KERNEL_CHECK();
  scan_tiles_kernel<<<dim3(1), dim3(SCAN_THREADS), 0, st>>>(tile_tmp.p, ntiles, out + n);
  MM_KERNEL_CHECK();
  scan_apply_kernel<<<dim3((unsigned)ntiles), dim3(SCAN_THREADS), 0, st>>>(in, n, tile_tmp.p, out);
  MM_KERNEL_CHECK();
}

}
```

### metamaps_amd/csrc/mm_seed.hpp

```cpp
#pragma once
#include "mm_map.hpp"

namespace mm {

__global__ void __launch_bounds__(256) probe_kernel(IndexView I, const uint32_t* __restrict__ sk_hash, const uint64_t* __restrict__ off,
                                                    const int32_t* __restrict__ sk_n, uint32_t* __restrict__ probe_cnt,
                                                    uint64_t* __restrict__ probe_start, const uint8_t* __restrict__ only ) {
  const int r = blockIdx.x;
  if (only && !only[r]) return;
  const uint64_t o = off[r];
  const int s = sk_n[r];
  const int grp = threadIdx.x >> 2, sub = threadIdx.x & 3, gshift = (threadIdx.x & 63) & ~3;
  const ulonglong2* __restrict__ tab = reinterpret_cast<const ulonglong2*>(I.tab);
  const uint64_t tslots = (uint64_t)I.tab_buckets << 2;
  constexpr int NP = 4;
  for (int i0 = grp; i0 < s; i0 += 64 * NP) {
    uint32_t hq[NP]; uint64_t sq[NP]; ulonglong2 vq[NP];
#pragma unroll
    for (int u = 0; u < NP; ++u) { hq[u] = i0 + 64 * u < s ? sk_hash[o + i0 + 64 * u] : 0u; sq[u] = tab_slot(hq[u], I.tab_buckets); }
#pragma unroll
    for (int u = 0; u < NP; ++u) vq[u] = tab[sq[u] + sub];
    auto resolve = [&](uint32_t h, uint64_t slot, ulonglong2 v, bool active, int i) {
      bool pending = active;
      while (__any(pending)) {
        const bool match = pending && v.x != 0 && (uint32_t)v.x == h, empty = pending && v.x == 0;
        const uint32_t gm = (uint32_t)(__ballot(match) >> gshift) & 0xfu, ge = (uint32_t)(__ballot(empty) >> gshift) & 0xfu;
        if (pending && (gm | ge)) {
          if (match) {
            const uint32_t cnt = (uint32_t)(v.x >> 32);
            const bool keep = (uint64_t)cnt < (uint64_t)(int64_t)I.freq_threshold;
            probe_cnt[o + i] = keep ? cnt : 0u;
            probe_start[o + i] = keep ? v.y : 0ull;
          } else if (!gm && sub == 0) { probe_cnt[o + i] = 0u; probe_start[o + i] = 0ull; }
          pending = false;
        }
        if (pending) { slot = tab_next_sector(slot, tslots); v = tab[slot + sub]; }
      }
    };
#pragma unroll
    for (int u = 0; u < NP; ++u) resolve(hq[u], sq[u], vq[u], i0 + 64 * u < s, i0 + 64 * u);
  }
}

__global__ void __launch_bounds__(256) gather_hits_kernel(IndexView I, const uint64_t* __restrict__ off, const int32_t* __restrict__ sk_n,
                                                          const uint32_t* __restrict__ probe_cnt, const uint64_t* __restrict__ probe_start,
                                                          const uint64_t* __restrict__ hit_off, uint64_t* __restrict__ hits) {
  const int r = blockIdx.x;
  const uint64_t o = off[r];
  const int s = sk_n[r];
  for (int i = threadIdx.x; i < s; i += 256) {
    uint32_t c = probe_cnt[o + i];
    if (!c) continue;
    const uint64_t* src = I.occ + probe_start[o + i];
    uint64_t* dst = hits + hit_off[o + i];
    for (uint32_t j = 0; j < c; ++j) dst[j] = src[j] & ~(uint64_t)(PW_DP | PW_DN);
  }
}

template <int SLOT_BITS> struct HitFilterCfg {
  static constexpr int SLOTS = 1 << SLOT_BITS, THREADS = SLOTS / 32;
  static constexpr int EPL = SLOT_BITS == HF_SLOT_BITS_NARROW ? 8 : 2;
  static constexpr int CLS = SLOT_BITS == HF_SLOT_BITS_NARROW ? 1 : 2;
  static constexpr size_t LDS = (size_t)SLOTS * 4 + (size_t)THREADS * 8 + 16;
};
template <bool WRITE, int SLOT_BITS>
__global__ void __launch_bounds__(HitFilterCfg<SLOT_BITS>::THREADS) hit_filter_kernel(IndexView I, const uint64_t* __restrict__ off, const int32_t* __restrict__ sk_n,
                                                         const uint32_t* __restrict__ probe_cnt, const uint64_t* __restrict__ probe_start,
                                                         const int32_t* __restrict__ read_len, const int32_t* __restrict__ min_hits,
                                                         uint32_t* __restrict__ surv_n, const uint64_t* __restrict__ read_hit_off,
                                                         uint64_t* __restrict__ hits, uint64_t* __restrict__ stage, const uint64_t* __restrict__ stage_off, int dbg,
                                                         const uint8_t* __restrict__ cls ,
                                                         uint32_t* __restrict__ raw_hits ) {
  using Cfg = HitFilterCfg<SLOT_BITS>;
  constexpr int SLOTS = Cfg::SLOTS, THREADS = Cfg::THREADS, EPL = Cfg::EPL;
  constexpr bool NARROW = SLOT_BITS == HF_SLOT_BITS_NARROW;
  extern __shared__ __align__(16) uint32_t hf_lds[];
  uint32_t* const cnt = hf_lds;
  uint32_t* const good = cnt + SLOTS;
  uint32_t* const alive = good + THREADS;
  uint32_t& cursor = alive[THREADS];
  const int r = blockIdx.x;
  const int my_cls = cls[r];
  if (!WRITE && my_cls != Cfg::CLS) return;
  if (WRITE && (my_cls == 2) != (Cfg::CLS == 2)) return;
  if (WRITE) {
    const uint32_t n_s = surv_n[r];
    if (n_s <= (uint32_t)(stage_off[r + 1] - stage_off[r])) {
      if (dbg == 100 && n_s >= 2u && n_s <= 4096u) return;
      const uint64_t wb = read_hit_off[r];
      for (uint32_t i = threadIdx.x; i < n_s; i += THREADS) hits[wb + i] = stage[stage_off[r] + i];
      return;
    }
  }
  const uint64_t o = off[r];
  const int s = sk_n[r];
  const uint32_t len = (uint32_t)max(read_len[r], 1);
  const int nb = min((int)((len - 1) >> HF_BIN_SHIFT) + 2, SLOTS);
  int m = min_hits[r]; if (m < 1) m = 1;
  for (int i = threadIdx.x; i < SLOTS; i += THREADS) cnt[i] = 0;
  if (threadIdx.x == 0) cursor = 0;
  __syncthreads();
  constexpr int GROUPS = THREADS / 4, PER_REQ = 4 * EPL;
  const int grp = threadIdx.x >> 2, sub = threadIdx.x & 3;
  auto for_each_chunk = [&](auto&& fn) {
    auto meta = [&](int i, uint32_t& c, uint64_t& st0) { c = 0; st0 = 0; if (i < s) { c = probe_cnt[o + i]; st0 = probe_start[o + i]; } };
    auto issue = [&](uint32_t c, uint64_t st0, uint32_t j0, ulonglong2& v) {
      if (c) {
        const uint64_t e = st0 + min(j0 + (uint32_t)EPL * sub, (c - 1) & ~(uint32_t)(EPL - 1));
        v = NARROW ? *reinterpret_cast<const ulonglong2*>(I.occ16 + e) : *reinterpret_cast<const ulonglong2*>(I.occ + e);
      }
    };
    uint32_t c0, c1, c2, c3; uint64_t s0, s1, s2, s3;
    ulonglong2 v0 = make_ulonglong2(0, 0), v1 = v0, v2 = v0;
    meta(grp, c0, s0); meta(grp + GROUPS, c1, s1); meta(grp + 2 * GROUPS, c2, s2);
    issue(c0, s0, 0, v0); issue(c1, s1, 0, v1);
    for (int ib = 0; ib < s; ib += GROUPS) {
      meta(ib + grp + 3 * GROUPS, c3, s3);
      issue(c2, s2, 0, v2);
      fn(c0, s0, 0u, v0);
      for (uint32_t j0 = PER_REQ; __any(j0 < c0); j0 += PER_REQ) {
        const uint32_t cl = j0 < c0 ? c0 : 0u;
        ulonglong2 v = make_ulonglong2(0, 0); issue(cl, s0, j0, v); fn(cl, s0, j0, v);
      }
      c0 = c1; s0 = s1; v0 = v1; c1 = c2; s1 = s2; v1 = v2; c2 = c3; s2 = s3;
    }
  };
  auto code_of = [](const ulonglong2& v, int t) -> uint32_t {
    if (NARROW) return (uint32_t)((t < 4 ? v.x : v.y) >> (16 * (t & 3))) & (uint32_t)(SLOTS - 1);
    const uint64_t e = t ? v.y : v.x;
    return (((uint32_t)e >> (3 + HF_BIN_SHIFT)) + (uint32_t)(e >> 32) * 40503u) & (uint32_t)(SLOTS - 1);
  };
  if (dbg == 2) {
    uint32_t a = 0;
    for_each_chunk([&](uint32_t c, uint64_t, uint32_t j0, const ulonglong2& v) { for (int t = 0; t < EPL; ++t) if (j0 + (uint32_t)EPL * sub + t < c) a += code_of(v, t); });
    if (a == 0x12345678u) cnt[0] = 1;
  } else for_each_chunk([&](uint32_t c, uint64_t, uint32_t j0, const ulonglong2& v) {
#pragma unroll
    for (int t = 0; t < EPL; ++t) if (j0 + (uint32_t)EPL * sub + t < c) atomicAdd(&cnt[code_of(v, t)], 1u);
  });
  __syncthreads();
  if (dbg == 1 || dbg == 2) { if (!WRITE && threadIdx.x == 0) surv_n[r] = 0; return; }
  {
    const int b0 = threadIdx.x * 32;
    uint32_t sum = 0, bits = 0;
    for (int i = 0; i < nb; ++i) sum += cnt[(b0 + i) & (SLOTS - 1)];
    for (int t = 0; t < 32; ++t) {
      bits |= (sum >= (uint32_t)m ? 1u : 0u) << t;
      sum += cnt[(b0 + t + nb) & (SLOTS - 1)] - cnt[(b0 + t) & (SLOTS - 1)];
    }
    good[threadIdx.x] = bits;
    __syncthreads();
    uint32_t al = 0;
    for (int j = 0; j < nb; ++j) {
      const int wsh = j >> 5, bsh = j & 31;
      const uint32_t g0 = good[(threadIdx.x - wsh) & (THREADS - 1)], g1 = good[(threadIdx.x - wsh - 1) & (THREADS - 1)];
      al |= bsh ? (g0 << bsh) | (g1 >> (32 - bsh)) : g0;
    }
    alive[threadIdx.x] = al;
    __syncthreads();
  }
  const uint64_t wbase = WRITE ? read_hit_off[r] : 0;
  const uint64_t stage_base = stage_off[r];
  const uint32_t stage_cap = (uint32_t)(stage_off[r + 1] - stage_base);
  uint64_t* const dst = WRITE ? hits + wbase : stage + stage_base;
  const uint32_t dst_cap = WRITE ? 0xffffffffu : stage_cap;
  const int lane = threadIdx.x & 63;
  for_each_chunk([&](uint32_t c, uint64_t st0, uint32_t j0, const ulonglong2& v) {
    const uint32_t e0 = j0 + (uint32_t)EPL * sub;
    uint32_t mask = 0;
#pragma unroll
    for (int t = 0; t < EPL; ++t) { const uint32_t b = code_of(v, t); mask |= ((e0 + t < c) ? (alive[b >> 5] >> (b & 31)) & 1u : 0u) << t; }
    if (dbg == 4) { if (mask == 0xdeadu) cnt[1] = 1; return; }
    const int mine = __popc(mask);
    const int incl = wave_incl_scan(mine);
    const int total = __builtin_amdgcn_readlane(incl, 63);
    if (total == 0) return;
    uint32_t base = 0;
    if (lane == 63) base = atomicAdd(&cursor, (uint32_t)total);
    base = (uint32_t)__builtin_amdgcn_readlane((int)base, 63);
    uint32_t pos = base + (uint32_t)(incl - mine);
    while (mask) {
      const int t = __ffs(mask) - 1; mask &= mask - 1;
      if (pos < dst_cap) dst[pos] = st0 + e0 + t;
      ++pos;
    }
  });
  __syncthreads();
  const uint32_t n_s = min(cursor, dst_cap);
  if (dbg == 3 || dbg == 4) { if (!WRITE && threadIdx.x == 0) surv_n[r] = 0; return; }
  for (uint32_t j = threadIdx.x; j < n_s; j += THREADS) dst[j] = I.occ[dst[j]] & ~(uint64_t)(PW_DP | PW_DN);
  if (!WRITE && threadIdx.x == 0) surv_n[r] = cursor;
  if (!WRITE && raw_hits) {
    __syncthreads();
    uint32_t acc = 0;
    for (int i = threadIdx.x; i < SLOTS; i += THREADS) acc += cnt[i];
    for (int d = 32; d > 0; d >>= 1) acc += __shfl_xor(acc, d, 64);
    if ((threadIdx.x & 63) == 0 && acc) atomicAdd(&raw_hits[r], acc);
  }
}

constexpr int SF_THREADS = 1024, SF_GROUPS = SF_THREADS / 4;
constexpr int SF_LPG = 11;
constexpr int SF_SMAX = SF_GROUPS * SF_LPG;
constexpr int SF_CHUNKS = 6144;
__device__ __forceinline__ void lds_barrier() { asm volatile("s_waitcnt lgkmcnt(0)\n\ts_barrier" ::: "memory"); }

#ifndef SF_STREAM_WAVES_PER_EU
#define SF_STREAM_WAVES_PER_EU 4
#endif
struct SeedFilterStreamLds {
  uint32_t cnt[HF_SLOTS + HF_PAD_SLOTS];
  uint32_t good[HF_SLOTS / 32], alive[HF_SLOTS / 32 + 4];
  uint32_t lstart8[SF_SMAX];
  uint16_t lcnt[SF_SMAX];
  uint16_t coff8[SF_SMAX + 8];
  uint16_t anchor[SF_CHUNKS / 4];
  uint32_t wsum[SF_THREADS / 64], wsum2[SF_THREADS / 64];
  uint32_t cursor, fallback, total8, hraw, tick[2], pad_[2];
  ulonglong2 codes[SF_CHUNKS];
};
static_assert(sizeof(SeedFilterStreamLds) <= 160 * 1024, "the streaming seed filter's LDS must fit one CU");
template <bool PROF>
__global__ void __launch_bounds__(SF_THREADS) __attribute__((amdgpu_waves_per_eu(SF_STREAM_WAVES_PER_EU, SF_STREAM_WAVES_PER_EU))) seed_filter_stream_kernel(IndexView I, const uint32_t* __restrict__ sk_hash, const uint64_t* __restrict__ off,
                                                                        const int32_t* __restrict__ sk_n, const int32_t* __restrict__ read_len,
                                                                        const int32_t* __restrict__ min_hits, uint32_t* __restrict__ surv_n,
                                                                        uint64_t* __restrict__ stage, const uint64_t* __restrict__ stage_off,
                                                                        uint8_t* need_old, const uint32_t* __restrict__ cls_words ,
                                                                        uint32_t* __restrict__ raw_hits, int n_reads, uint32_t* __restrict__ ticket,
                                                                        unsigned long long* __restrict__ prof ) {
  extern __shared__ __align__(16) unsigned char sf_dyn[];
  SeedFilterStreamLds& L = *reinterpret_cast<SeedFilterStreamLds*>(sf_dyn);
  const ulonglong2* __restrict__ tab = reinterpret_cast<const ulonglong2*>(I.tab);
  const uint64_t tslots = (uint64_t)I.tab_buckets << 2;
  uint32_t hq[SF_LPG]; ulonglong2 vq[SF_LPG];
  int r_cur = 0, s_cur = 0; uint64_t o_cur = 0;
  unsigned long long pt[16] = {0, 0, 0, 0, 0, 0, 0, 0, 0, 0, 0, 0, 0, 0, 0, 0}, pt0 = 0;
  auto lapp = [&](int i) { if (PROF) { const unsigned long long t = __builtin_readcyclecounter(); pt[i] += t - pt0; pt0 = t; } };
  if (PROF) pt0 = __builtin_readcyclecounter();
  
  for (int it = -1; it < 0 || r_cur < n_reads; ++it) {
    int tid = (int)threadIdx.x;
    asm volatile("" : "+v"(tid));
    const int lane = tid & 63, wid = tid >> 6;
    const int grp = tid >> 2, sub = tid & 3, gshift = lane & ~3;
    auto uni64 = [](uint64_t v) { return (uint64_t)(uint32_t)__builtin_amdgcn_readfirstlane((int)(uint32_t)v) | (uint64_t)(uint32_t)__builtin_amdgcn_readfirstlane((int)(uint32_t)(v >> 32)) << 32; };
    auto head = [&](int r, int& s, uint64_t& o) {
      const int rr = min(r, n_reads - 1);
      const uint32_t cw = cls_words[rr >> 2]; const int sn = sk_n[rr]; const uint64_t on = off[rr];
      s = 0; o = 0;
      if (r < n_reads && !((cw >> (8 * (rr & 3))) & 0xffu)) {
        s = sn; o = on;
        if (s <= 0) { s = 0; if (tid == 0) { surv_n[r] = 0; raw_hits[r] = 0; } }
      }
    };
    auto load_hashes = [&](int s_, uint64_t o_) {
      const int su = __builtin_amdgcn_readfirstlane(s_);
      const char* __restrict__ hb = reinterpret_cast<const char*>(sk_hash + uni64(o_));
      const uint32_t last = (uint32_t)max(su - 1, 0);
      if (su > 0) {
#pragma unroll
        for (int u = 0; u < SF_LPG; ++u) hq[u] = *reinterpret_cast<const uint32_t*>(hb + (size_t)(min((uint32_t)(grp + SF_GROUPS * u), last) << 2));
      } else {
#pragma unroll
        for (int u = 0; u < SF_LPG; ++u) hq[u] = 0u;
      }
    };
    auto issue_lookups = [&]() {
#pragma unroll
      for (int u = 0; u < SF_LPG; ++u) asm volatile("" : "+v"(hq[u]));
      int sub_ = (int)threadIdx.x & 3;
      asm volatile("" : "+v"(sub_));
#pragma unroll
      for (int u = 0; u < SF_LPG; ++u) vq[u] = tab[tab_slot(hq[u], I.tab_buckets) + sub_];
    };
    if (it < 0) {
      if (tid == 0) L.tick[0] = atomicAdd(ticket, 1u);
      if (tid < 4) L.alive[HF_SLOTS / 32 + tid] = 0;
      lds_barrier();
      r_cur = __builtin_amdgcn_readfirstlane((int)L.tick[0]);
      head(r_cur, s_cur, o_cur);
      load_hashes(s_cur, o_cur);
      issue_lookups();
      continue;
    }
    if (tid == 0) L.tick[(it + 1) & 1] = atomicAdd(ticket, 1u);
    int r_next = n_reads, s_next = 0; uint64_t o_next = 0;
    bool next_issued = false, next_known = false;
    if (s_cur > 0) {
      const int r = __builtin_amdgcn_readfirstlane(r_cur), s = __builtin_amdgcn_readfirstlane(s_cur);
      const uint64_t stage_base = stage_off[r];
      const uint32_t stage_cap = (uint32_t)(stage_off[r + 1] - stage_base);
      const uint32_t len = (uint32_t)max(read_len[r], 1);
      const int nb = min((int)((len - 1) >> HF_BIN_SHIFT) + 2, HF_SLOTS);
      int m = min_hits[r]; if (m < 1) m = 1;
      {
        uint32_t z = 0;
        asm volatile("" : "+v"(z));
        for (int i = tid; i < (HF_SLOTS + HF_PAD_SLOTS) / 4; i += SF_THREADS) reinterpret_cast<uint4*>(L.cnt)[i] = make_uint4(z, z, z, z);
        if (tid < (int)(sizeof L.lcnt / 16)) reinterpret_cast<uint4*>(L.lcnt)[tid] = make_uint4(z, z, z, z);
        if (tid == 0) { L.cursor = z; L.fallback = z; L.pad_[0] = z; }
      }
      lds_barrier();
      lapp(0);
      r_next = __builtin_amdgcn_readfirstlane((int)L.tick[(it + 1) & 1]);
      head(r_next, s_next, o_next);
      next_known = true;
      auto settle = [&](int i, uint32_t h, const ulonglong2& v, bool pending) -> bool {
        const bool match = pending && v.x != 0 && (uint32_t)v.x == h, empty = pending && v.x == 0;
        const uint32_t done = (uint32_t)(__ballot(match || empty) >> gshift) & 0xfu;
        if (match) {
          const uint32_t cnt = (uint32_t)(v.x >> 32);
          if ((uint64_t)cnt < (uint64_t)(int64_t)I.freq_threshold) {
            if (cnt > 0xffffu) L.fallback = 1;
            L.lcnt[i] = (uint16_t)cnt; L.lstart8[i] = (uint32_t)(v.y >> 3);
          }
        }
        return !pending || done != 0;
      };
      uint32_t pmask = 0;
#pragma unroll
      for (int u = 0; u < SF_LPG; ++u) {
        const int i = grp + SF_GROUPS * u;
        if (!settle(i, hq[u], vq[u], i < s)) { pmask |= 1u << u; vq[u] = tab[tab_next_sector(tab_slot(hq[u], I.tab_buckets), tslots) + sub]; }
      }
      lapp(7);
      if (__any(pmask != 0)) {
#pragma unroll
        for (int u = 0; u < SF_LPG; ++u) {
          const int i = grp + SF_GROUPS * u;
          const uint32_t h = hq[u]; uint64_t slot = tab_next_sector(tab_slot(h, I.tab_buckets), tslots); ulonglong2 v = vq[u];
          bool pending = (pmask >> u) & 1u;
          while (__any(pending)) {
            if (settle(i, h, v, pending)) pending = false;
            if (pending) { slot = tab_next_sector(slot, tslots); v = tab[slot + sub]; }
          }
        }
      }
      lds_barrier();
      lapp(1);
      {
        uint32_t c8[3], hr = 0, mine = 0;
#pragma unroll
        for (int j = 0; j < 3; ++j) { const int i = tid * 3 + j; const uint32_t c = i < s ? L.lcnt[i] : 0u; c8[j] = (c + 7) >> 3; mine += c8[j]; hr += c; }
        const uint32_t inc = (uint32_t)wave_incl_scan((int)mine), inc2 = (uint32_t)wave_incl_scan((int)hr);
        if (lane == 63) { L.wsum[wid] = inc; L.wsum2[wid] = inc2; }
        lds_barrier();
        uint32_t basew = 0, tot = 0, tot2 = 0;
#pragma unroll
        for (int q = 0; q < SF_THREADS / 64; ++q) { const uint32_t x = L.wsum[q]; if (q < wid) basew += x; tot += x; tot2 += L.wsum2[q]; }
        uint32_t ex = basew + inc - mine;
#pragma unroll
        for (int j = 0; j < 3; ++j) {
          const int i = tid * 3 + j;
          if (i <= s) L.coff8[i] = (uint16_t)min(ex, 0xffffu);
          for (uint32_t a = (ex + 3) >> 2, a1 = min((ex + c8[j] + 3) >> 2, (uint32_t)(SF_CHUNKS / 4)); a < a1; ++a) L.anchor[a] = (uint16_t)i;
          ex += c8[j];
        }
        if (tid == 0) { L.total8 = tot; L.hraw = tot2; if (tot > (uint32_t)SF_CHUNKS || tot2 > 65535u) L.fallback = 1; }
      }
      lds_barrier();
      lapp(2);
      if (L.fallback) { if (tid == 0) { need_old[r] = 1; surv_n[r] = 0; raw_hits[r] = 0; } }
      else {
        load_hashes(s_next, o_next);
        {
          constexpr int NP = SF_CHUNKS / SF_THREADS;
          const uint32_t T8u = (uint32_t)__builtin_amdgcn_readfirstlane((int)L.total8);
          ulonglong2 v[NP];
#pragma unroll
          for (int j = 0; j < NP; ++j) {
            v[j] = make_ulonglong2(0, 0);
            if ((uint32_t)(j * SF_THREADS) < T8u) {
              const uint32_t q = min((uint32_t)(tid + j * SF_THREADS), T8u - 1);
              uint32_t li = L.anchor[q >> 2];
              while ((uint32_t)L.coff8[li + 1] <= q) ++li;
              v[j] = *reinterpret_cast<const ulonglong2*>(I.occ16 + ((uint64_t)L.lstart8[li] << 3) + (uint64_t)(q - (uint32_t)L.coff8[li]) * 8u);
            }
          }
#pragma unroll
          for (int j = 0; j < NP; ++j) {
            const uint32_t q = (uint32_t)(tid + j * SF_THREADS);
            if (q < T8u) {
              const ulonglong2 x = v[j];
#pragma unroll
              for (int t = 0; t < 8; ++t) atomicAdd(&L.cnt[(uint32_t)((t < 4 ? x.x : x.y) >> (16 * (t & 3))) & 0xffffu], 1u);
              L.codes[q] = x;
            }
          }
          lapp(8);
        }
        lds_barrier();
        lapp(3);
        {
          const uint32_t* cnt = L.cnt;
#pragma unroll
          for (int kk = 0; kk < HF_SLOTS / SF_THREADS; ++kk) {
            const int b = tid + kk * SF_THREADS;
            uint32_t sum = 0;
            for (int i = 0; i < nb; ++i) sum += cnt[(b + i) & (HF_SLOTS - 1)];
            const uint64_t gb = __ballot(sum >= (uint32_t)m);
            if (lane == 0) { L.good[(b >> 5)] = (uint32_t)gb; L.good[(b >> 5) + 1] = (uint32_t)(gb >> 32); }
          }
        }
        lds_barrier();
        lapp(9);
        if (tid < HF_SLOTS / 32) {
          uint32_t al = 0;
          for (int j = 0; j < nb; ++j) {
            const int wsh = j >> 5, bsh = j & 31;
            const uint32_t g0 = L.good[(tid - wsh) & 255], g1 = L.good[(tid - wsh - 1) & 255];
            al |= bsh ? (g0 << bsh) | (g1 >> (32 - bsh)) : g0;
          }
          L.alive[tid] = al;
        }
        lapp(10);
        lds_barrier();
        lapp(4);
        issue_lookups();
        lapp(11);
        next_issued = true;
        uint64_t* const dst = stage + stage_base;
        uint16_t* const sv = reinterpret_cast<uint16_t*>(L.cnt);
        const uint32_t sv_cap = min(stage_cap, (uint32_t)(2 * (HF_SLOTS + HF_PAD_SLOTS)));
        const uint32_t T8 = L.total8;
        uint32_t cv = 0;
        if (lane == 0) cv = atomicAdd(&L.pad_[0], 1u);
        for (uint32_t c = (uint32_t)__builtin_amdgcn_readfirstlane((int)cv); c * 64u < T8; c = (uint32_t)__builtin_amdgcn_readfirstlane((int)cv)) {
          if (lane == 0) cv = atomicAdd(&L.pad_[0], 1u);
          const uint32_t q = c * 64u + (uint32_t)lane;
          uint32_t mask = 0;
          if (q < T8) {
            const ulonglong2 x = L.codes[q];
#pragma unroll
            for (int t = 0; t < 8; ++t) {
              const uint32_t code = (uint32_t)((t < 4 ? x.x : x.y) >> (16 * (t & 3))) & 0xffffu;
              mask |= ((L.alive[code >> 5] >> (code & 31)) & 1u) << t;
            }
          }
          const int mine = __popc(mask);
          const int incl = wave_incl_scan(mine);
          const int total = __builtin_amdgcn_readlane(incl, 63);
          if (total == 0) continue;
          uint32_t base = 0;
          if (lane == 63) base = atomicAdd(&L.cursor, (uint32_t)total);
          base = (uint32_t)__builtin_amdgcn_readlane((int)base, 63);
          uint32_t pos = base + (uint32_t)(incl - mine);
          while (mask) {
            const int t = __ffs(mask) - 1; mask &= mask - 1;
            if (pos < sv_cap) sv[pos] = (uint16_t)(q << 3 | (uint32_t)t);
            ++pos;
          }
        }
        lapp(12);
        lds_barrier();
        lapp(5);
        const uint32_t n_s = L.cursor;
        if (n_s > sv_cap) { if (tid == 0) { need_old[r] = 1; surv_n[r] = 0; raw_hits[r] = 0; } }
        else {
          for (uint32_t j = tid; j < n_s; j += SF_THREADS) {
            const uint32_t e = sv[j], q = e >> 3;
            uint32_t li = L.anchor[q >> 2];
            while ((uint32_t)L.coff8[li + 1] <= q) ++li;
            dst[j] = I.occ[((uint64_t)L.lstart8[li] << 3) + (uint64_t)(q - (uint32_t)L.coff8[li]) * 8u + (e & 7u)] & ~(uint64_t)(PW_DP | PW_DN);
          }
          if (tid == 0) { surv_n[r] = n_s; raw_hits[r] = L.hraw; }
        }
      }
    }
    if (!next_issued) {
      lds_barrier();
      if (!next_known) { r_next = __builtin_amdgcn_readfirstlane((int)L.tick[(it + 1) & 1]); head(r_next, s_next, o_next); }
      load_hashes(s_next, o_next);
      issue_lookups();
    }
    lds_barrier();
    lapp(6);
    r_cur = r_next; s_cur = s_next; o_cur = o_next;
  }
  if (PROF && threadIdx.x == 0) for (int i = 0; i < 16; ++i) atomicAdd(&prof[i], pt[i]);
}

__global__ void __launch_bounds__(256) move_ranges_kernel(const uint64_t* __restrict__ src, const uint64_t* __restrict__ sb, const uint64_t* __restrict__ se,
                                                          uint64_t* __restrict__ dst, const uint64_t* __restrict__ db) {
  const uint64_t s0 = sb[blockIdx.x], n = se[blockIdx.x] - s0, d0 = db[blockIdx.x];
  for (uint64_t i = threadIdx.x; i < n; i += 256) dst[d0 + i] = src[s0 + i];
}
__global__ void __launch_bounds__(256) sum_u32_kernel(const uint32_t* __restrict__ v, int64_t n, unsigned long long* __restrict__ out) {
  unsigned long long acc = 0;
  for (int64_t i = (int64_t)blockIdx.x * 256 + threadIdx.x; i < n; i += (int64_t)gridDim.x * 256) acc += v[i];
  for (int d = 32; d > 0; d >>= 1) acc += __shfl_xor(acc, d, 64);
  if ((threadIdx.x & 63) == 0 && acc) atomicAdd(out, acc);
}

__global__ void __launch_bounds__(256) probed_list_hist_kernel(IndexView I, const uint32_t* __restrict__ sk_hash, const uint64_t* __restrict__ off,
                                                               const int32_t* __restrict__ sk_n, int nb, unsigned long long* __restrict__ hist) {
  const int r = blockIdx.x, s = sk_n[r];
  const uint64_t o = off[r];
  for (int i = threadIdx.x; i < s; i += 256) {
    uint32_t cnt = 0; uint64_t start = 0;
    int b = 0;
    if (index_find(I, sk_hash[o + i], &cnt, &start)) b = (uint64_t)cnt < (uint64_t)(int64_t)I.freq_threshold ? (int)min(cnt, (uint32_t)(nb - 2)) : nb - 1;
    atomicAdd(&hist[b], 1ull);
  }
}

__global__ void read_hit_bounds_kernel(const uint64_t* __restrict__ off, const uint64_t* __restrict__ hit_off, int64_t n,
                                       uint64_t* __restrict__ read_hit_off) {
  int64_t r = (int64_t)blockIdx.x * blockDim.x + threadIdx.x;
  if (r <= n) read_hit_off[r] = hit_off[off[r]];
}

}
```

### metamaps_amd/csrc/mm_seq.hip

```cpp
#include "mm_minimizer.hpp"
#include <algorithm>
#include <thread>
#include <atomic>
#include <cstdio>
#include <cstring>

extern "C" int mm_host_has_avx2();
extern "C" size_t mm_pack_acgt_blocks(const uint8_t* p, size_t n_bases, uint32_t* out);

namespace mm {

SeqView make_view(const mm_seqset* S) {
  return SeqView{S->packed.p, S->d_base.p, S->d_len.p, S->exc_start.p, S->exc_len.p, S->exc_byte.p, S->n_exc, S->count()};
}

__global__ void gather_offsets_kernel(const uint64_t* __restrict__ tile_first, const uint64_t* __restrict__ tile_out, int64_t n,
                                      uint64_t* __restrict__ off) {
  int64_t s = (int64_t)blockIdx.x * blockDim.x + threadIdx.x;
  if (s <= n) off[s] = tile_out[tile_first[s]];
}

void run_minimizers(mm_ctx* ctx, const mm_seqset* S, int k, int w, const std::vector<uint8_t>& active, bool want_rec_seq,
                    MinimizerSet& out) {
  MM_REQUIRE(S->frozen, MM_ERR_STATE, "sequence set not uploaded");
  MM_REQUIRE(k >= 1 && k <= MZ_MAX_K, MM_ERR_ARG, "k must be in [1,64]");
  MM_REQUIRE(w >= 1 && w <= MZ_MAX_W, MM_ERR_ARG, "window size must be in [1,4096]");
  hipStream_t st = ctx->stream;
  const int64_t n = S->count();
  std::vector<uint64_t> tf((size_t)n + 1, 0);
  for (int64_t i = 0; i < n; ++i) {
    int64_t npos = (int64_t)S->len[i] - k + 1;
    bool on = active.empty() || active[(size_t)i];
    int64_t nt = (on && npos >= w) ? ceil_div(npos, MZ_TILE) : 0;
    tf[i + 1] = tf[i] + (uint64_t)nt;
  }
  const int64_t ntiles = (int64_t)tf[n];
  out.off.alloc((size_t)n + 1);
  out.h_off.assign((size_t)n + 1, 0);
  out.total = 0;
  if (ntiles == 0) { out.off.zero(st); out.rec.alloc(0); MM_HIP(mm::stream_sync(st)); return; }
  MM_REQUIRE(ntiles < (1LL << 31), MM_ERR_LIMIT, "too many tiles for one launch");

  DBuf<uint64_t> d_tf((size_t)n + 1);
  d_tf.upload(tf.data(), tf.size(), st);
  DBuf<uint8_t> d_act;
  if (!active.empty()) { d_act.alloc(active.size()); d_act.upload(active.data(), active.size(), st); }
  DBuf<int32_t> d_js((size_t)n);
  SeqView V = make_view(S);
  jstar_kernel<<<dim3((unsigned)ceil_div(n, 128)), dim3(128), 0, st>>>(V, d_act.p, k, w, d_js.p);
  MM_KERNEL_CHECK();

  const size_t lds = minimizer_lds_bytes(k, w);
  if (lds > 64 * 1024) {
    MM_HIP(hipFuncSetAttribute((const void*)minimizer_kernel<0>, hipFuncAttributeMaxDynamicSharedMemorySize, (int)lds));
    MM_HIP(hipFuncSetAttribute((const void*)minimizer_kernel<1>, hipFuncAttributeMaxDynamicSharedMemorySize, (int)lds));
    MM_HIP(hipFuncSetAttribute((const void*)minimizer_kernel<2>, hipFuncAttributeMaxDynamicSharedMemorySize, (int)lds));
  }
  DBuf<uint32_t> tcount((size_t)ntiles);
  DBuf<uint64_t> tout((size_t)ntiles + 1), tmp;
  bool single_pass = !want_rec_seq && (size_t)ntiles * MZ_STAGE * sizeof(Rec) <= ((size_t)6 << 30);
  DBuf<Rec> stage;
  DBuf<int> d_ovf(1); d_ovf.zero(st);
  if (single_pass) {
    stage.alloc((size_t)ntiles * MZ_STAGE);
    { const char* e = getenv("MM_MZ_DBG"); int v = e ? atoi(e) : 0; MM_HIP(hipMemcpyToSymbolAsync(HIP_SYMBOL(mz_dbg_stop), &v, sizeof v, 0, hipMemcpyHostToDevice, st)); }
    minimizer_kernel<2><<<dim3((unsigned)ntiles), dim3(MZ_THREADS), lds, st>>>(V, d_tf.p, k, w, d_js.p, tcount.p, nullptr, stage.p, nullptr, d_ovf.p);
  } else {
    minimizer_kernel<0><<<dim3((unsigned)ntiles), dim3(MZ_THREADS), lds, st>>>(V, d_tf.p, k, w, d_js.p, tcount.p, nullptr, nullptr, nullptr, nullptr);
  }
  MM_KERNEL_CHECK();
  exclusive_scan_u32_u64(tcount.p, ntiles, tout.p, tmp, st);
  uint64_t total = 0;
  int h_ovf = 0;
  MM_HIP(hipMemcpyAsync(&total, tout.p + ntiles, sizeof total, hipMemcpyDeviceToHost, st));
  MM_HIP(hipMemcpyAsync(&h_ovf, d_ovf.p, sizeof h_ovf, hipMemcpyDeviceToHost, st));
  MM_HIP(mm::stream_sync(st));
  if (h_ovf) single_pass = false;
  out.total = (int64_t)total;
  out.rec.alloc((size_t)total);
  if (want_rec_seq) out.rec_seq.alloc((size_t)total);
  if (total) {
    if (single_pass)
      compact_tiles_kernel<<<dim3((unsigned)ntiles), dim3(256), 0, st>>>(stage.p, tcount.p, tout.p, out.rec.p);
    else
      minimizer_kernel<1><<<dim3((unsigned)ntiles), dim3(MZ_THREADS), lds, st>>>(V, d_tf.p, k, w, d_js.p, nullptr, tout.p, out.rec.p,
                                                                               want_rec_seq ? out.rec_seq.p : nullptr, nullptr);
    MM_KERNEL_CHECK();
  }
  gather_offsets_kernel<<<dim3((unsigned)ceil_div(n + 1, 256)), dim3(256), 0, st>>>(d_tf.p, tout.p, n, out.off.p);
  MM_KERNEL_CHECK();
  out.off.download(out.h_off.data(), (size_t)n + 1, st);
  MM_HIP(mm::stream_sync(st));
}

static inline int code_of(uint8_t c) {
  switch (c) { case 'A': return 0; case 'C': return 1; case 'G': return 2; case 'T': return 3; }
  return -1;
}

void seqset_upload(mm_seqset* s) {
  MM_REQUIRE(!s->frozen, MM_ERR_STATE, "sequence set already uploaded");
  hipStream_t st = s->ctx->stream;
  const size_t n = s->staged.size();
  s->len.resize(n);
  s->base.assign(n + 1, 0);
  s->total_bases = 0;
  for (size_t i = 0; i < n; ++i) {
    MM_REQUIRE((int64_t)s->staged[i].second <= MAX_SEQ_LEN, MM_ERR_LIMIT, "sequence longer than 2^29-1 bases");
    s->len[i] = (int32_t)s->staged[i].second;
    s->base[i + 1] = s->base[i] + (((uint64_t)s->len[i] + 15) & ~15ull);
    s->total_bases += s->len[i];
  }
  const size_t nwords = (size_t)(s->base[n] >> 4);
  uint32_t* const words = (uint32_t*)s->ctx->pinned_up_at_least((nwords + 1) * sizeof(uint32_t));
  words[nwords] = 0;
  std::vector<uint64_t> es; std::vector<uint32_t> el; std::vector<uint8_t> eb;
  {
    static const struct Lut { uint8_t t[256]; Lut() { for (int c = 0; c < 256; ++c) { int u = (c > 96 && c < 123) ? c - 32 : c; int k = code_of((uint8_t)u); t[c] = k >= 0 ? (uint8_t)k : 0x80; } } } lut;
    struct Item { size_t seq; size_t j0, j1; };
    struct Runs { std::vector<uint64_t> es; std::vector<uint32_t> el; std::vector<uint8_t> eb; };
    constexpr size_t PIECE = (size_t)4 << 20;
    std::vector<Item> items;
    for (size_t i = 0; i < n; ++i) { const size_t L = s->staged[i].second; for (size_t j0 = 0; j0 < L; j0 += PIECE) items.push_back(Item{i, j0, std::min(L, j0 + PIECE)}); }
    std::vector<Runs> runs(items.size());
    const unsigned hw = mm::cpu_budget();
    const size_t nthr = (size_t)std::max<uint64_t>(1, std::min<uint64_t>({(uint64_t)std::max(1u, hw / 2), 32, (uint64_t)(s->total_bases >> 22) + 1, (uint64_t)std::max<size_t>(items.size(), 1)}));
    std::atomic<size_t> next_item{0};
    const bool simd = mm_host_has_avx2() != 0 && !getenv("MM_PACK_SCALAR");
    auto work = [&]() {
      for (;;) {
        const size_t it = next_item.fetch_add(1);
        if (it >= items.size()) return;
        const Item I = items[it];
        Runs& R = runs[it];
        const uint8_t* p = (const uint8_t*)s->staged[I.seq].first;
        uint32_t* wp = words + (s->base[I.seq] >> 4);
        const uint64_t b0 = s->base[I.seq];
        bool open = false;
        for (size_t j0 = I.j0; j0 < I.j1; j0 += 16) {
          if (simd && j0 + 32 <= I.j1) {
            const size_t done = mm_pack_acgt_blocks(p + j0, (I.j1 - j0) & ~(size_t)31, wp + (j0 >> 4));
            if (done) { open = false; j0 += done; if (j0 >= I.j1) break; }
          }
          const size_t m = std::min<size_t>(16, I.j1 - j0);
          uint32_t wv = 0; uint8_t bad = 0;
          for (size_t j = 0; j < m; ++j) { const uint8_t k = lut.t[p[j0 + j]]; bad |= k; wv |= (uint32_t)(k & 3) << (2 * j); }
          if (!(bad & 0x80)) { wp[j0 >> 4] = wv; open = false; continue; }
          wv = 0;
          for (size_t j = 0; j < m; ++j) {
            uint8_t c = p[j0 + j];
            if (c > 96 && c < 123) c -= 32;
            const uint8_t k = lut.t[c];
            if (!(k & 0x80)) { wv |= (uint32_t)k << (2 * j); open = false; }
            else if (open && R.eb.back() == c && R.el.back() < 0xFFFFFFFFu) R.el.back()++;
            else { R.es.push_back(b0 + j0 + j); R.el.push_back(1); R.eb.push_back(c); open = true; }
          }
          wp[j0 >> 4] = wv;
        }
      }
// ... 393 lines not shown
```

Baseline: 25.85.

## Pack per-batch small buffers into one arena with pinned mailbox and list-driven fallback kernels

Replaces many small per-batch device allocations and zero-fills with a single zeroed arena that also holds a mailbox of counters. Small device-to-host readbacks go through one pinned host image instead of several pageable copies. The raw-hit sum kernel is folded into the surviving-hit scan as a side sum carried in an extra offset slot. When every read takes the fused path, the probe and hit-filter kernels walk a compact list of fallback reads built atomically by the seed filter, instead of launching one block per read. This trades launch, allocation and sync overhead for added bookkeeping complexity and a fixed cap on hand-back rounds.

```diff
diff --git a/include/metamaps_hip.h b/include/metamaps_hip.h
--- a/include/metamaps_hip.h
+++ b/include/metamaps_hip.h
@@ -188,6 +188,7 @@
 int mm_debug_l2(mm_mapping* m, int64_t* per_cand , int64_t cap);
 int mm_debug_min_hits(mm_mapping* m, int32_t* min_hits );
 int mm_debug_probed_lists(mm_mapping* m, const mm_index* idx, int64_t* hist, int32_t n_bins);
+int mm_debug_scan(mm_ctx* ctx, const uint32_t* in, int64_t n, uint64_t* out, int form, int reps, double* seconds);
 
 int mm_em_create(mm_ctx* ctx, int64_t n_reads, const int64_t* read_off, const int32_t* taxon, const double* mapq,
                  const double* inv_nloc, int32_t n_taxa, mm_em** out);
diff --git a/metamaps_amd/capi.py b/metamaps_amd/capi.py
--- a/metamaps_amd/capi.py
+++ b/metamaps_amd/capi.py
@@ -170,6 +170,7 @@
             "mm_debug_l2": (C.c_int, [vp, vp, i64]),
             "mm_debug_min_hits": (C.c_int, [vp, vp]),
             "mm_debug_probed_lists": (C.c_int, [vp, vp, vp, i32]),
+            "mm_debug_scan": (C.c_int, [vp, vp, i64, vp, C.c_int, C.c_int, P(f64)]),
             "mm_em_create": (C.c_int, [vp, i64, vp, vp, vp, vp, i32, P(vp)]),
             "mm_em_create_from_mapping": (C.c_int, [vp, vp, vp, vp, i32, i32, P(vp)]),
             "mm_em_taxon_counts": (C.c_int, [vp, vp]),
diff --git a/metamaps_amd/csrc/mm_api.hip b/metamaps_amd/csrc/mm_api.hip
--- a/metamaps_amd/csrc/mm_api.hip
+++ b/metamaps_amd/csrc/mm_api.hip
@@ -118,6 +118,7 @@
   mm::comm_destroy(ctx);
   if (ctx->pinned) (void)hipHostFree(ctx->pinned);
   if (ctx->pinned_up) (void)hipHostFree(ctx->pinned_up);
+  if (ctx->mbox_host) (void)hipHostFree(ctx->mbox_host);
   ctx->l2_codes.release(); ctx->l2_masks.release();
   if (ctx->ev_fork) (void)hipEventDestroy(ctx->ev_fork);
   if (ctx->ev_join) (void)hipEventDestroy(ctx->ev_join);
@@ -850,6 +851,29 @@
   });
 }
 
+int mm_debug_scan(mm_ctx* ctx, const uint32_t* in, int64_t n, uint64_t* out, int form, int reps, double* seconds) {
+  if (!ctx || !out || n < 0 || (n > 0 && !in) || reps < 1 || !(form == mm::SCAN_AUTO || form == mm::SCAN_SINGLE || form == mm::SCAN_THREE)) return MM_ERR_ARG;
+  return guarded(ctx, [&] {
+    MM_HIP(hipSetDevice(ctx->device));
+    hipStream_t st = ctx->stream;
+    mm::DBuf<uint32_t> d_in((size_t)std::max<int64_t>(n, 1));
+    mm::DBuf<uint64_t> d_out((size_t)n + 1), tmp;
+    d_in.upload(in, (size_t)n, st);
+    hipEvent_t e0, e1;
+    MM_HIP(hipEventCreate(&e0)); MM_HIP(hipEventCreate(&e1));
+    MM_HIP(hipEventRecord(e0, st));
+    for (int i = 0; i < reps; ++i) mm::exclusive_scan_u32_u64(d_in.p, n, d_out.p, tmp, st, nullptr, form);
+    MM_HIP(hipEventRecord(e1, st));
+    d_out.download(out, (size_t)n + 1, st);
+    const hipError_t e = mm::stream_sync(st);
+    float ms = 0;
+    if (e == hipSuccess) (void)hipEventElapsedTime(&ms, e0, e1);
+    (void)hipEventDestroy(e0); (void)hipEventDestroy(e1);
+    MM_HIP(e);
+    if (seconds) *seconds = ms * 1e-3;
+  });
+}
+
 int mm_em_create(mm_ctx* ctx, int64_t n_reads, const int64_t* read_off, const int32_t* taxon, const double* mapq, const double* inv_nloc,
                  int32_t n_taxa, mm_em** out) {
   if (!ctx || !read_off || !out || n_reads < 0 || n_taxa <= 0) return MM_ERR_ARG;
diff --git a/metamaps_amd/csrc/mm_batch_rules.hpp b/metamaps_amd/csrc/mm_batch_rules.hpp
--- /dev/null
+++ b/metamaps_amd/csrc/mm_batch_rules.hpp
@@ -0,0 +1,51 @@
+#pragma once
+#include <cstddef>
+#include <cstdint>
+
+namespace mm {
+
+constexpr size_t ARENA_ALIGN = 256;
+
+constexpr size_t MB_MZ_TOTAL = 0;
+constexpr size_t MB_MZ_OVF = 8;
+constexpr size_t MB_FB_N = 24;
+constexpr size_t MB_SF_TICKET = 28;
+constexpr size_t MB_GRP_CTR = 32;
+constexpr size_t MB_BIG_N = 48;
+constexpr size_t MB_OVF_N = 52;
+constexpr int MB_OVF_GENS = 3;
+constexpr size_t MB_NREC = 64;
+constexpr size_t MB_COUNTERS = 128;
+constexpr size_t MB_BYTES = 256;
+inline size_t mb_ovf_n(int gen) { return MB_OVF_N + 4 * (size_t)gen; }
+
+enum ArenaPiece { AP_MBOX = 0, AP_RAW_PER_READ, AP_SURV, AP_CAND_N, AP_AMB_USED, AP_SLOT_FLAGS, AP_COUNT };
+struct ArenaLayout {
+  size_t off[AP_COUNT], bytes[AP_COUNT], total;
+};
+inline size_t arena_round(size_t b) { return (b + ARENA_ALIGN - 1) / ARENA_ALIGN * ARENA_ALIGN; }
+inline ArenaLayout arena_layout(int64_t n, size_t slots) {
+  const size_t nn = n > 0 ? (size_t)n : 0;
+  ArenaLayout L{};
+  L.bytes[AP_MBOX] = MB_BYTES;
+  L.bytes[AP_RAW_PER_READ] = nn * 4;
+  L.bytes[AP_SURV] = (nn + 1) * 4;
+  L.bytes[AP_CAND_N] = (nn + 1) * 4;
+  L.bytes[AP_AMB_USED] = nn;
+  L.bytes[AP_SLOT_FLAGS] = slots * 4;
+  size_t at = 0;
+  for (int i = 0; i < AP_COUNT; ++i) { L.off[i] = at; at += arena_round(L.bytes[i] ? L.bytes[i] : 1); }
+  L.total = at;
+  return L;
+}
+
+constexpr int64_t SCAN_SINGLE_MAX = 4096;
+enum ScanForm { SCAN_AUTO = 0, SCAN_SINGLE = 1, SCAN_THREE = 3 };
+inline bool scan_is_single(int64_t n, int form) { return form == SCAN_SINGLE || (form == SCAN_AUTO && n <= SCAN_SINGLE_MAX); }
+
+inline unsigned fallback_grid(int64_t n, int cus) {
+  const int64_t g = 2 * (int64_t)(cus > 0 ? cus : 1);
+  return (unsigned)(n < 1 ? 1 : (n < g ? n : g));
+}
+
+}
diff --git a/metamaps_amd/csrc/mm_common.hpp b/metamaps_amd/csrc/mm_common.hpp
--- a/metamaps_amd/csrc/mm_common.hpp
+++ b/metamaps_amd/csrc/mm_common.hpp
@@ -129,6 +129,8 @@
   int lut_k = 0; float lut_pi = 0;
   mm::GrowBuf l2_codes, l2_masks;
   void* pinned = nullptr; size_t pinned_bytes = 0;
+  void* mbox_host = nullptr;
+  unsigned char* mbox_host_ready() { if (!mbox_host) MM_HIP(hipHostMalloc(&mbox_host, 256, hipHostMallocDefault)); return static_cast<unsigned char*>(mbox_host); }
   void* pinned_up = nullptr; size_t pinned_up_bytes = 0;
   std::unique_ptr<TaskPool> pack_pool;
   void* pinned_up_at_least(size_t bytes) {
diff --git a/metamaps_amd/csrc/mm_map.hip b/metamaps_amd/csrc/mm_map.hip
--- a/metamaps_amd/csrc/mm_map.hip
+++ b/metamaps_amd/csrc/mm_map.hip
@@ -2,6 +2,7 @@
 #include <functional>
 #include <memory>
 #include "mm_prims.hpp"
+#include "mm_batch_rules.hpp"
 #include "mm_l2_core.hpp"
 #include "mm_size_classes.hpp"
 #include "mm_l2.hpp"
@@ -137,6 +138,17 @@
 
 void set_lds(const void* fn, size_t bytes) { if (bytes > 64 * 1024) MM_HIP(hipFuncSetAttribute(fn, hipFuncAttributeMaxDynamicSharedMemorySize, (int)bytes)); }
 
+template <typename T>
+struct Piece {
+  T* p = nullptr; size_t n = 0;
+  std::vector<T> to_host(hipStream_t st, size_t count = (size_t)-1) const {
+    std::vector<T> v(count == (size_t)-1 ? n : count);
+    if (!v.empty()) MM_HIP(hipMemcpyAsync(v.data(), p, v.size() * sizeof(T), hipMemcpyDeviceToHost, st));
+    MM_HIP(mm::stream_sync(st));
+    return v;
+  }
+};
+
 struct MapRun {
   mm_ctx* const ctx; const mm_index* const I; const mm_seqset* const reads; const mm_map_params& P; mm_mapping* const M;
   const hipStream_t st;
@@ -151,31 +163,36 @@
   std::vector<int64_t> eager_reads, lazy_reads;
   std::vector<std::unique_ptr<AmbState>> amb_states;
   IndexView IV{};
+  DBuf<uint8_t> arena; ArenaLayout AL{};
+  template <typename T> Piece<T> piece(ArenaPiece which) const { return Piece<T>{reinterpret_cast<T*>(arena.p + AL.off[which]), AL.bytes[which] / sizeof(T)}; }
+  template <typename T> Piece<T> mbox(size_t byte_off, size_t count) const { return Piece<T>{reinterpret_cast<T*>(arena.p + AL.off[AP_MBOX] + byte_off), count}; }
   DBuf<uint32_t> probe_cnt;
   DBuf<uint64_t> probe_start;
   DBuf<uint64_t> hit_off, scan_tmp;
-  DBuf<uint8_t> need_old; DBuf<uint32_t> raw_per_read;
+  DBuf<uint8_t> need_old; Piece<uint32_t> raw_per_read;
+  DBuf<int32_t> fb_list;
+  bool by_list = false;
   int64_t n_fused = 0, n_wide = 0;
   uint64_t raw_hits = 0;
-  DBuf<unsigned long long> raw_sum;
-  DBuf<uint32_t> surv;
+  Piece<uint32_t> surv, fb_n, sf_ticket;
   DBuf<uint64_t> stage, stage_off;
   const uint8_t* only = nullptr;
-  DBuf<uint32_t> cand_n;
+  Piece<uint32_t> cand_n;
   DBuf<int32_t> cand_hint;
   DBuf<int64_t> cand_rng;
   DBuf<int32_t> d_gA0, d_gAn, d_gS0, d_gSn;
-  DBuf<unsigned int> grp_ctr;
+  Piece<unsigned int> grp_ctr;
   std::vector<int32_t> listG; int smG = 0;
-  DBuf<unsigned long long> counters;
+  Piece<unsigned long long> counters;
   DBuf<int32_t> ovf;
-  DBuf<unsigned int> ovf_n;
-  DBuf<uint8_t> amb_used;
+  Piece<unsigned int> ovf_n;
+  int ovf_gen = 0;
+  Piece<uint8_t> amb_used;
   uint8_t* amb_used_p = nullptr;
   struct SkipClasses {
-    DBuf<unsigned int> slot_flags;
+    Piece<unsigned int> slot_flags;
     DBuf<int32_t> big;
-    DBuf<unsigned int> big_n;
+    Piece<unsigned int> big_n;
     std::vector<int32_t> gA0, gAn, gB0, gBn, gD0, gDn, listC, gS0, gSn;
     int smA = 0, smB = 0, smC = 0, smD = 0;
     std::vector<int32_t> listL; int smL = 0;
@@ -208,6 +225,22 @@
       if (ok) { M->stats.n_reads_long_enough++; M->stats.bases_long_enough += L; }
     }
     t_total = T.begin(&M->stats.ms_total);
+    AL = arena_layout(n, std::max((size_t)std::max(ctx->cus, 1) * 64, sw.l2_slots));
+    arena.alloc(AL.total); arena.zero(st);
+    raw_per_read = piece<uint32_t>(AP_RAW_PER_READ); surv = piece<uint32_t>(AP_SURV); cand_n = piece<uint32_t>(AP_CAND_N); amb_used = piece<uint8_t>(AP_AMB_USED);
+    fb_n = mbox<uint32_t>(MB_FB_N, 1); sf_ticket = mbox<uint32_t>(MB_SF_TICKET, 1);
+    grp_ctr = mbox<unsigned int>(MB_GRP_CTR, 4); counters = mbox<unsigned long long>(MB_COUNTERS, 16); ovf_n = mbox<unsigned int>(mb_ovf_n(0), 1);
+  }
+  template <typename T> const T* fetch_mbox(size_t byte_off, size_t count) {
+    static_assert(MB_BYTES <= 256, "the context's pinned mailbox image holds 256 bytes");
+    unsigned char* const h = ctx->mbox_host_ready() + byte_off;
+    MM_HIP(hipMemcpyAsync(h, arena.p + AL.off[AP_MBOX] + byte_off, count * sizeof(T), hipMemcpyDeviceToHost, st));
+    MM_HIP(mm::stream_sync(st));
+    return reinterpret_cast<const T*>(h);
+  }
+  void next_ovf_gen() {
+    MM_REQUIRE(++ovf_gen < MB_OVF_GENS, MM_ERR_STATE, "more hand-back rounds than the batch's mailbox has counters");
+    ovf_n = mbox<unsigned int>(mb_ovf_n(ovf_gen), 1);
   }
 
   void minimizers() {
@@ -223,7 +256,7 @@
       if (same_ctx) M->sk_hash.share_from(dn->sk_hash); else dcopy(M->sk_hash, donor->sk_hash);
       dcopy(M->sk_strand, donor->sk_strand); dcopy(M->sk_n, donor->sk_n); dcopy(M->amb, donor->amb);
       T.end(t);
-    } else { size_t t = T.begin(&M->stats.ms_minimizer); run_minimizers(ctx, reads, P.k, P.w, M->active, false, M->mz); T.end(t); }
+    } else { size_t t = T.begin(&M->stats.ms_minimizer); run_minimizers(ctx, reads, P.k, P.w, M->active, false, M->mz, mbox<uint64_t>(MB_MZ_TOTAL, 2).p); T.end(t); }
     total_mz = M->mz.total;
     if (!donor) {
       M->sk_hash.alloc((size_t)std::max<int64_t>(total_mz, 1));
@@ -407,8 +440,7 @@
   void seed_hits() {
     probe_cnt.alloc((size_t)total_mz + 1);
     probe_start.alloc((size_t)total_mz + 1);
-    if (filtering()) { raw_per_read.alloc((size_t)n); raw_per_read.zero(st); }
-    else if (total_mz > 0) probe_cnt.zero(st);
+    if (!filtering() && total_mz > 0) probe_cnt.zero(st);
     if (filtering()) {
       std::vector<uint8_t> h_need((size_t)n, 0);
       for (int64_t r = 0; r < n; ++r) {
@@ -421,12 +453,12 @@
     }
     hl("K3 prep (need_old etc.)");
     const size_t t_pg = T.begin(&M->stats.ms_probe_gather);
-    M->read_hit_off.alloc((size_t)n + 1);
-    raw_sum.alloc(1);
+    M->read_hit_off.alloc((size_t)n + 2);
     if (filtering()) seed_stage_and_fused();
     only = filtering() ? need_old.p : nullptr;
     if (n > 0 && total_mz > 0) {
-      probe_kernel<<<dim3((unsigned)n), dim3(256), 0, st>>>(IV, M->sk_hash.p, M->mz.off.p, M->sk_n.p, probe_cnt.p, probe_start.p, only);
+      if (by_list) probe_list_kernel<<<dim3(fallback_grid(n, ctx->cus)), dim3(256), 0, st>>>(IV, M->sk_hash.p, M->mz.off.p, M->sk_n.p, probe_cnt.p, probe_start.p, only, fb_list.p, fb_n.p);
+      else probe_kernel<<<dim3((unsigned)n), dim3(256), 0, st>>>(IV, M->sk_hash.p, M->mz.off.p, M->sk_n.p, probe_cnt.p, probe_start.p, only);
       MM_KERNEL_CHECK();
     }
     if (!filtering()) {
@@ -439,17 +471,14 @@
       const size_t t_hf = time_old ? T.begin(&M->stats.ms_hit_filter) : 0;
       launch_hit_filter<false>(nullptr, nullptr, sw.hf_dbg, raw_per_read.p);
       if (time_old) T.end(t_hf);
-      raw_sum.zero(st);
-      sum_u32_kernel<<<dim3(256), dim3(256), 0, st>>>(raw_per_read.p, n, raw_sum.p);
-      MM_KERNEL_CHECK();
-      MM_HIP(hipMemcpyAsync(&raw_hits, raw_sum.p, sizeof raw_hits, hipMemcpyDeviceToHost, st));
-      exclusive_scan_u32_u64(surv.p, n, M->read_hit_off.p, scan_tmp, st);
+      exclusive_scan_with_side_sum(surv.p, raw_per_read.p, n, M->read_hit_off.p, scan_tmp, st);
     } else {
       read_hit_bounds_kernel<<<dim3((unsigned)ceil_div(n + 1, 256)), dim3(256), 0, st>>>(M->mz.off.p, hit_off.p, n, M->read_hit_off.p);
       MM_KERNEL_CHECK();
     }
     hl("K3 launches");
-    M->h_read_hit_off = M->read_hit_off.to_host(st);
+    M->h_read_hit_off = M->read_hit_off.to_host(st, (size_t)n + (raw_rides() ? 2 : 1));
+    if (raw_rides()) { raw_hits = M->h_read_hit_off.back(); M->h_read_hit_off.pop_back(); }
     hl("K3 wait + hit_off download");
     total_hits = (int64_t)M->h_read_hit_off[(size_t)n];
     M->stats.sum_hits = (int64_t)raw_hits;
@@ -465,9 +494,17 @@
     T.end(t_pg);
   }
 
+  bool raw_rides() const { return filtering(); }
+
   template <bool WRITE>
   void launch_hit_filter(const uint64_t* hit_off_p, uint64_t* hits_p, int dbg, uint32_t* raw_p) {
     using HfN = HitFilterCfg<HF_SLOT_BITS_NARROW>; using HfW = HitFilterCfg<HF_SLOT_BITS_WIDE>;
+    if (by_list) {
+      hit_filter_list_kernel<WRITE, HF_SLOT_BITS_NARROW><<<dim3(fallback_grid(n, ctx->cus)), dim3(HfN::THREADS), HfN::LDS, st>>>(IV, M->mz.off.p, M->sk_n.p, probe_cnt.p, probe_start.p,
+          M->d_read_len.p, M->min_hits.p, surv.p, hit_off_p, hits_p, stage.p, stage_off.p, dbg, only, raw_p, fb_list.p, fb_n.p);
+      MM_KERNEL_CHECK();
+      return;
+    }
     hit_filter_kernel<WRITE, HF_SLOT_BITS_NARROW><<<dim3((unsigned)n), dim3(HfN::THREADS), HfN::LDS, st>>>(IV, M->mz.off.p, M->sk_n.p, probe_cnt.p, probe_start.p, M->d_read_len.p,
                                                                    M->min_hits.p, surv.p, hit_off_p, hits_p, stage.p, stage_off.p, dbg, only, raw_p);
     if (n_wide > 0) {
@@ -480,7 +517,6 @@
   }
 
   void seed_stage_and_fused() {
-    surv.alloc((size_t)n + 1); surv.zero(st);
     std::vector<uint64_t> h_stage_off((size_t)n + 1, 0);
     for (int64_t r = 0; r < n; ++r)
       h_stage_off[(size_t)r + 1] = h_stage_off[(size_t)r] + (M->h_sk_n[(size_t)r] > 0 ? (sw.hf_stage_cap.set ? (uint64_t)sw.hf_stage_cap.v : 1024 + 2 * (uint64_t)M->h_sk_n[(size_t)r]) : 0);
@@ -492,8 +528,8 @@
     const size_t lds = sizeof(SeedFilterStreamLds);
     MM_HIP(hipFuncSetAttribute((const void*)seed_filter_stream_kernel<false>, hipFuncAttributeMaxDynamicSharedMemorySize, (int)lds));
     MM_HIP(hipFuncSetAttribute((const void*)seed_filter_stream_kernel<true>, hipFuncAttributeMaxDynamicSharedMemorySize, (int)lds));
-    DBuf<uint32_t> sf_ticket(1);
-    sf_ticket.zero(st);
+    fb_list.alloc((size_t)n);
+    by_list = n_fused == n;
     DBuf<unsigned long long> sf_prof;
     if (sw.sf_prof) { sf_prof.alloc(16); sf_prof.zero(st); }
     int sf_grid = (int)std::min<int64_t>(n, std::max(ctx->cus, 1));
@@ -501,10 +537,10 @@
     const size_t t_sf = T.begin(&M->stats.ms_hit_filter);
     if (sf_prof.p)
       seed_filter_stream_kernel<true><<<dim3((unsigned)sf_grid), dim3(SF_THREADS), lds, st>>>(IV, M->sk_hash.p, M->mz.off.p, M->sk_n.p, M->d_read_len.p, M->min_hits.p, surv.p, stage.p, stage_off.p,
-                                                                         need_old.p, reinterpret_cast<const uint32_t*>(need_old.p), raw_per_read.p, (int)n, sf_ticket.p, sf_prof.p);
+                                                                         need_old.p, reinterpret_cast<const uint32_t*>(need_old.p), raw_per_read.p, (int)n, sf_ticket.p, fb_list.p, fb_n.p, sf_prof.p);
     else
       seed_filter_stream_kernel<false><<<dim3((unsigned)sf_grid), dim3(SF_THREADS), lds, st>>>(IV, M->sk_hash.p, M->mz.off.p, M->sk_n.p, M->d_read_len.p, M->min_hits.p, surv.p, stage.p, stage_off.p,
-                                                                         need_old.p, reinterpret_cast<const uint32_t*>(need_old.p), raw_per_read.p, (int)n, sf_ticket.p, nullptr);
+                                                                         need_old.p, reinterpret_cast<const uint32_t*>(need_old.p), raw_per_read.p, (int)n, sf_ticket.p, fb_list.p, fb_n.p, nullptr);
     MM_KERNEL_CHECK();
     T.end(t_sf);
     if (sf_prof.p) {
@@ -607,7 +643,6 @@
 
   void l1_candidates() {
     t_l1 = T.begin(&M->stats.ms_l1_scan);
-    cand_n.alloc((size_t)n + 1); cand_n.zero(st);
     M->cand_off.alloc((size_t)n + 2);
     const unsigned rblk = (unsigned)ceil_div(std::max<int64_t>(n, 1), 128);
     if (n > 0) {
@@ -680,7 +715,7 @@
     MM_KERNEL_CHECK();
     T.end(t_l2);
     hl("K5 wait");
-    auto hc = counters.to_host(st);
+    const unsigned long long* const hc = fetch_mbox<unsigned long long>(MB_COUNTERS, 16);
     M->stats.sum_l2_stream_entries = (int64_t)hc[0];
     M->stats.sum_l2_evals = (int64_t)hc[1];
     M->stats.n_l2_rebuilds = (int64_t)hc[2];
@@ -693,10 +728,8 @@
       l2_ranges_kernel<<<dim3((unsigned)ceil_div(ncand, 256)), dim3(256), 0, st>>>(IV, M->cand.p, M->cand_read.p, M->d_read_len.p, ncand, cand_rng.p);
       MM_KERNEL_CHECK();
     }
-    grp_ctr.alloc(4);
     if (sw.dev_groups) {
       d_gA0.alloc((size_t)ncand); d_gAn.alloc((size_t)ncand); d_gS0.alloc((size_t)ncand); d_gSn.alloc((size_t)ncand);
-      grp_ctr.zero(st);
       l2_group_kernel<<<dim3((unsigned)ceil_div(n, 256)), dim3(256), 0, st>>>(M->cand_off.p, M->sk_n.p, M->d_read_len.p, n, min_mapped_len(), sw.dense_from,
                                                                             sw.no_small_groups ? 1 : 0, d_gA0.p, d_gAn.p, d_gS0.p, d_gSn.p, grp_ctr.p);
       MM_KERNEL_CHECK();
@@ -709,15 +742,12 @@
       for (uint64_t c0 = M->h_cand_off[(size_t)r]; c0 < M->h_cand_off[(size_t)r + 1]; ++c0) listG.push_back((int32_t)c0);
     }
     MM_REQUIRE(lds_wide <= 160 * 1024, MM_ERR_LIMIT, "L2 window state does not fit LDS");
-    counters.alloc(16); counters.zero(st);
     if (sw.has_l2_debug_word()) {
       const unsigned long long v = sw.l2_debug_word();
       MM_HIP(hipMemcpyAsync(counters.p + 11, &v, sizeof v, hipMemcpyHostToDevice, st));
       MM_HIP(mm::stream_sync(st));
     }
     ovf.alloc((size_t)ncand);
-    ovf_n.alloc(1); ovf_n.zero(st);
-    if (!lazy_reads.empty()) { amb_used.alloc((size_t)n); amb_used.zero(st); }
     amb_used_p = lazy_reads.empty() ? nullptr : amb_used.p;
     finish_tiebreak();
   }
@@ -771,9 +801,9 @@
 
   void l2_skip_classes() {
     sk = std::make_unique<SkipClasses>();
-    sk->slot_flags.alloc(std::max((size_t)ctx->cus * 64, sw.l2_slots)); sk->slot_flags.zero(st);
+    sk->slot_flags = piece<unsigned int>(AP_SLOT_FLAGS);
     sk->big.alloc((size_t)(sw.v2 ? ncand : 1));
-    sk->big_n.alloc(1); sk->big_n.zero(st);
+    sk->big_n = mbox<unsigned int>(MB_BIG_N, 1);
     l2_host_groups();
     l2_dense(sk->listL, sk->smL, amb_used_p);
     sk->d_gB0.alloc(sk->gB0.size()); sk->d_gBn.alloc(sk->gBn.size()); sk->d_listC.alloc(sk->listC.size());
@@ -804,7 +834,7 @@
   void l2_host_groups() {
     SkipClasses& s = *sk;
     hl("K5 prep before grouping");
-    if (sw.dev_groups) s.gctr = grp_ctr.to_host(st);
+    if (sw.dev_groups) { const unsigned int* const g = fetch_mbox<unsigned int>(MB_GRP_CTR, 4); s.gctr.assign(g, g + 4); }
     s.smA = (int)s.gctr[3];
     for (int64_t r = 0; r < n && (!sw.dev_groups || s.gctr[2] > 0); ++r) {
       const uint64_t c_lo = M->h_cand_off[(size_t)r], c_hi = M->h_cand_off[(size_t)r + 1];
@@ -884,22 +914,20 @@
 
   void l2_fallback(uint8_t* amb_ptr, bool read_ovf, unsigned int h_ovf) {
     if (read_ovf) {
-      MM_HIP(hipMemcpyAsync(&h_ovf, ovf_n.p, sizeof h_ovf, hipMemcpyDeviceToHost, st));
-      MM_HIP(mm::stream_sync(st));
+      h_ovf = *fetch_mbox<unsigned int>(mb_ovf_n(ovf_gen), 1);
     }
     if (!h_ovf) return;
     launch_l2_full(ovf.p, h_ovf, amb_ptr);
-    ovf_n.zero(st);
+    next_ovf_gen();
     sk->n_fallback += h_ovf;
   }
 
   void l2_handbacks() {
     unsigned int h_ovf0 = 0;
     if (sw.v2) {
-      unsigned int h_big = 0;
-      MM_HIP(hipMemcpyAsync(&h_big, sk->big_n.p, sizeof h_big, hipMemcpyDeviceToHost, st));
-      MM_HIP(hipMemcpyAsync(&h_ovf0, ovf_n.p, sizeof h_ovf0, hipMemcpyDeviceToHost, st));
-      MM_HIP(mm::stream_sync(st));
+      static_assert(MB_OVF_N == MB_BIG_N + 4, "big_n and the first hand-back counter are fetched as one pair");
+      const unsigned int* const h2 = fetch_mbox<unsigned int>(MB_BIG_N, 2);
+      const unsigned int h_big = h2[0]; h_ovf0 = h2[1];
       if (h_big) {
         launch_l2_wide(sk->big.p, h_big, std::max(std::max(sk->smA, sk->smB), sk->smD), amb_used_p);
         sk->n_big = h_big;
@@ -940,10 +968,8 @@
     DBuf<uint64_t> rank((size_t)ncand + 1);
     accept_flags_kernel<<<dim3((unsigned)ceil_div(ncand, 256)), dim3(256), 0, st>>>(M->l2.p, ncand, flag.p);
     MM_KERNEL_CHECK();
-    exclusive_scan_u32_u64(flag.p, ncand, rank.p, scan_tmp, st);
-    uint64_t nrec = 0;
-    MM_HIP(hipMemcpyAsync(&nrec, rank.p + ncand, sizeof nrec, hipMemcpyDeviceToHost, st));
-    MM_HIP(mm::stream_sync(st));
+    exclusive_scan_u32_u64(flag.p, ncand, rank.p, scan_tmp, st, mbox<uint64_t>(MB_NREC, 1).p);
+    const uint64_t nrec = *fetch_mbox<uint64_t>(MB_NREC, 1);
     M->n_rec = (int64_t)nrec;
     M->rec.alloc((size_t)std::max<uint64_t>(nrec, 1));
     write_records_kernel<<<dim3((unsigned)ceil_div(ncand, 256)), dim3(256), 0, st>>>(M->l2.p, M->cand_read.p, M->sk_n.p, flag.p, rank.p, ncand, M->rec.p);
diff --git a/metamaps_amd/csrc/mm_minimizer.hpp b/metamaps_amd/csrc/mm_minimizer.hpp
--- a/metamaps_amd/csrc/mm_minimizer.hpp
+++ b/metamaps_amd/csrc/mm_minimizer.hpp
@@ -383,7 +383,7 @@
 };
 
 void run_minimizers(mm_ctx* ctx, const mm_seqset* S, int k, int w, const std::vector<uint8_t>& active, bool want_rec_seq,
-                    MinimizerSet& out);
+                    MinimizerSet& out, uint64_t* d_mbox = nullptr);
 
 SeqView make_view(const mm_seqset* S);
 
diff --git a/metamaps_amd/csrc/mm_scan.hpp b/metamaps_amd/csrc/mm_scan.hpp
--- a/metamaps_amd/csrc/mm_scan.hpp
+++ b/metamaps_amd/csrc/mm_scan.hpp
@@ -1,5 +1,6 @@
 #pragma once
 #include "mm_common.hpp"
+#include "mm_batch_rules.hpp"
 
 namespace mm {
 
@@ -17,38 +18,48 @@
   return v;
 }
 
-__device__ inline uint64_t block_excl_scan_u64(uint64_t v, uint64_t* total) {
-  __shared__ uint64_t wsum[SCAN_THREADS / 64];
+template <int THREADS>
+__device__ inline uint64_t block_excl_scan_u64_of(uint64_t v, uint64_t* total) {
+  __shared__ uint64_t wsum[THREADS / 64];
   const int lane = threadIdx.x & 63, wid = threadIdx.x >> 6;
   uint64_t inc = wave_incl_scan_u64(v);
   if (lane == 63) wsum[wid] = inc;
   __syncthreads();
   uint64_t base = 0, tot = 0;
 #pragma unroll
-  for (int i = 0; i < SCAN_THREADS / 64; ++i) { if (i < wid) base += wsum[i]; tot += wsum[i]; }
+  for (int i = 0; i < THREADS / 64; ++i) { if (i < wid) base += wsum[i]; tot += wsum[i]; }
   __syncthreads();
   if (total) *total = tot;
   return base + inc - v;
 }
+__device__ inline uint64_t block_excl_scan_u64(uint64_t v, uint64_t* total) { return block_excl_scan_u64_of<SCAN_THREADS>(v, total); }
 
-static __global__ void __launch_bounds__(SCAN_THREADS) scan_reduce_kernel(const uint32_t* __restrict__ in, int64_t n, uint64_t* __restrict__ tile_sum) {
+template <bool SIDE>
+static __global__ void __launch_bounds__(SCAN_THREADS) scan_reduce_kernel(const uint32_t* __restrict__ in, int64_t n, uint64_t* __restrict__ tile_sum,
+                                                                      const uint32_t* __restrict__ side, uint64_t* __restrict__ tile_side) {
   int64_t base = (int64_t)blockIdx.x * SCAN_TILE;
-  uint64_t s = 0;
+  uint64_t s = 0, s2 = 0;
 #pragma unroll
   for (int i = 0; i < SCAN_ITEMS; ++i) {
     int64_t j = base + (int64_t)i * SCAN_THREADS + threadIdx.x;
-    if (j < n) s += in[j];
+    if (j < n) { s += in[j]; if (SIDE) s2 += side[j]; }
   }
   uint64_t tot;
   block_excl_scan_u64(s, &tot);
   if (threadIdx.x == 0) tile_sum[blockIdx.x] = tot;
+  if (SIDE) {
+    block_excl_scan_u64(s2, &tot);
+    if (threadIdx.x == 0) tile_side[blockIdx.x] = tot;
+  }
 }
 
-static __global__ void __launch_bounds__(SCAN_THREADS) scan_tiles_kernel(uint64_t* __restrict__ tile_sum, int64_t ntiles, uint64_t* __restrict__ grand) {
-  uint64_t carry = 0;
+static __global__ void __launch_bounds__(SCAN_THREADS) scan_tiles_kernel(uint64_t* __restrict__ tile_sum, int64_t ntiles, uint64_t* __restrict__ grand, uint64_t* __restrict__ grand2,
+                                                                     const uint64_t* __restrict__ tile_side, uint64_t* __restrict__ side_total) {
+  uint64_t carry = 0, sacc = 0;
   for (int64_t base = 0; base < ntiles; base += SCAN_THREADS) {
     int64_t j = base + threadIdx.x;
     uint64_t v = j < ntiles ? tile_sum[j] : 0;
+    if (tile_side && j < ntiles) sacc += tile_side[j];
     uint64_t tot;
     uint64_t ex = block_excl_scan_u64(v, &tot);
     if (j < ntiles) tile_sum[j] = carry + ex;
@@ -56,6 +67,12 @@
     __syncthreads();
   }
   if (threadIdx.x == 0 && grand) *grand = carry;
+  if (threadIdx.x == 0 && grand2) *grand2 = carry;
+  if (tile_side) {
+    uint64_t stot;
+    block_excl_scan_u64(sacc, &stot);
+    if (threadIdx.x == 0) *side_total = stot;
+  }
 }
 
 static __global__ void __launch_bounds__(SCAN_THREADS) scan_apply_kernel(const uint32_t* __restrict__ in, int64_t n, const uint64_t* __restrict__ tile_sum,
@@ -70,16 +87,58 @@
   for (int i = 0; i < SCAN_ITEMS; ++i) { int64_t j = base + i; if (j < n) out[j] = ex; ex += v[i]; }
 }
 
-inline void exclusive_scan_u32_u64(const uint32_t* in, int64_t n, uint64_t* out, DBuf<uint64_t>& tile_tmp, hipStream_t st) {
-  if (n <= 0) { MM_HIP(hipMemsetAsync(out, 0, sizeof(uint64_t), st)); return; }
+constexpr int SCAN1_THREADS = 1024;
+constexpr int SCAN1_ITEMS = 16;
+constexpr int SCAN1_TILE = SCAN1_THREADS * SCAN1_ITEMS;
+static __global__ void __launch_bounds__(SCAN1_THREADS) scan_single_kernel(const uint32_t* __restrict__ in, int64_t n, uint64_t* __restrict__ out, uint64_t* __restrict__ total2,
+                                                                       const uint32_t* __restrict__ side) {
+  auto load = [&](int64_t base, uint32_t (&v)[SCAN1_ITEMS]) {
+    const int64_t b = base + (int64_t)threadIdx.x * SCAN1_ITEMS;
+#pragma unroll
+    for (int i = 0; i < SCAN1_ITEMS; ++i) v[i] = b + i < n ? in[b + i] : 0u;
+  };
+  uint64_t carry = 0, sacc = 0;
+  uint32_t nxt[SCAN1_ITEMS];
+  load(0, nxt);
+  for (int64_t base = 0; base < n; base += SCAN1_TILE) {
+    uint32_t v[SCAN1_ITEMS];
+    uint64_t s = 0;
+#pragma unroll
+    for (int i = 0; i < SCAN1_ITEMS; ++i) { v[i] = nxt[i]; s += v[i]; }
+    if (base + SCAN1_TILE < n) load(base + SCAN1_TILE, nxt);
+    if (side) for (int64_t j = base + threadIdx.x; j < n && j < base + SCAN1_TILE; j += SCAN1_THREADS) sacc += side[j];
+    uint64_t tot;
+    uint64_t ex = carry + block_excl_scan_u64_of<SCAN1_THREADS>(s, &tot);
+    const int64_t b = base + (int64_t)threadIdx.x * SCAN1_ITEMS;
+#pragma unroll
+    for (int i = 0; i < SCAN1_ITEMS; ++i) { if (b + i < n) out[b + i] = ex; ex += v[i]; }
+    carry += tot;
+  }
+  uint64_t stot = 0;
+  if (side) block_excl_scan_u64_of<SCAN1_THREADS>(sacc, &stot);
+  if (threadIdx.x == 0) { out[n] = carry; if (total2) *total2 = carry; if (side) out[n + 1] = stot; }
+}
+
+inline void exclusive_scan_u32_u64(const uint32_t* in, int64_t n, uint64_t* out, DBuf<uint64_t>& tile_tmp, hipStream_t st, uint64_t* total2 = nullptr, int form = SCAN_AUTO,
+                                   const uint32_t* side = nullptr) {
+  if (n <= 0) { MM_HIP(hipMemsetAsync(out, 0, sizeof(uint64_t), st)); if (total2) MM_HIP(hipMemsetAsync(total2, 0, sizeof(uint64_t), st)); return; }
+  if (scan_is_single(n, form)) {
+    scan_single_kernel<<<dim3(1), dim3(SCAN1_THREADS), 0, st>>>(in, n, out, total2, side);
+    MM_KERNEL_CHECK();
+    return;
+  }
   int64_t ntiles = ceil_div(n, SCAN_TILE);
-  if ((int64_t)tile_tmp.n < ntiles) tile_tmp.alloc((size_t)ntiles);
-  scan_reduce_kernel<<<dim3((unsigned)ntiles), dim3(SCAN_THREADS), 0, st>>>(in, n, tile_tmp.p);
+  if ((int64_t)tile_tmp.n < (side ? 2 : 1) * ntiles) tile_tmp.alloc((size_t)((side ? 2 : 1) * ntiles));
+  if (side) scan_reduce_kernel<true><<<dim3((unsigned)ntiles), dim3(SCAN_THREADS), 0, st>>>(in, n, tile_tmp.p, side, tile_tmp.p + ntiles);
+  else scan_reduce_kernel<false><<<dim3((unsigned)ntiles), dim3(SCAN_THREADS), 0, st>>>(in, n, tile_tmp.p, nullptr, nullptr);
   MM_KERNEL_CHECK();
-  scan_tiles_kernel<<<dim3(1), dim3(SCAN_THREADS), 0, st>>>(tile_tmp.p, ntiles, out + n);
+  scan_tiles_kernel<<<dim3(1), dim3(SCAN_THREADS), 0, st>>>(tile_tmp.p, ntiles, out + n, total2, side ? tile_tmp.p + ntiles : nullptr, side ? out + n + 1 : nullptr);
   MM_KERNEL_CHECK();
   scan_apply_kernel<<<dim3((unsigned)ntiles), dim3(SCAN_THREADS), 0, st>>>(in, n, tile_tmp.p, out);
   MM_KERNEL_CHECK();
 }
+inline void exclusive_scan_with_side_sum(const uint32_t* in, const uint32_t* side, int64_t n, uint64_t* out, DBuf<uint64_t>& tile_tmp, hipStream_t st) {
+  exclusive_scan_u32_u64(in, n, out, tile_tmp, st, nullptr, SCAN_AUTO, side);
+}
 
 }
diff --git a/metamaps_amd/csrc/mm_seed.hpp b/metamaps_amd/csrc/mm_seed.hpp
--- a/metamaps_amd/csrc/mm_seed.hpp
+++ b/metamaps_amd/csrc/mm_seed.hpp
@@ -3,11 +3,8 @@
 
 namespace mm {
 
-__global__ void __launch_bounds__(256) probe_kernel(IndexView I, const uint32_t* __restrict__ sk_hash, const uint64_t* __restrict__ off,
-                                                    const int32_t* __restrict__ sk_n, uint32_t* __restrict__ probe_cnt,
-                                                    uint64_t* __restrict__ probe_start, const uint8_t* __restrict__ only ) {
-  const int r = blockIdx.x;
-  if (only && !only[r]) return;
+__device__ __forceinline__ void probe_read(const IndexView& I, const uint32_t* __restrict__ sk_hash, const uint64_t* __restrict__ off,
+                                           const int32_t* __restrict__ sk_n, uint32_t* __restrict__ probe_cnt, uint64_t* __restrict__ probe_start, const int r) {
   const uint64_t o = off[r];
   const int s = sk_n[r];
   const int grp = threadIdx.x >> 2, sub = threadIdx.x & 3, gshift = (threadIdx.x & 63) & ~3;
@@ -41,6 +38,23 @@
     for (int u = 0; u < NP; ++u) resolve(hq[u], sq[u], vq[u], i0 + 64 * u < s, i0 + 64 * u);
   }
 }
+__global__ void __launch_bounds__(256) probe_kernel(IndexView I, const uint32_t* __restrict__ sk_hash, const uint64_t* __restrict__ off,
+                                                    const int32_t* __restrict__ sk_n, uint32_t* __restrict__ probe_cnt,
+                                                    uint64_t* __restrict__ probe_start, const uint8_t* __restrict__ only ) {
+  const int r = blockIdx.x;
+  if (only && !only[r]) return;
+  probe_read(I, sk_hash, off, sk_n, probe_cnt, probe_start, r);
+}
+__global__ void __launch_bounds__(256) probe_list_kernel(IndexView I, const uint32_t* __restrict__ sk_hash, const uint64_t* __restrict__ off,
+                                                         const int32_t* __restrict__ sk_n, uint32_t* __restrict__ probe_cnt,
+                                                         uint64_t* __restrict__ probe_start, const uint8_t* __restrict__ only,
+                                                         const int32_t* __restrict__ list, const uint32_t* __restrict__ list_n) {
+  const uint32_t nl = *list_n;
+  for (uint32_t i = blockIdx.x; i < nl; i += gridDim.x) {
+    const int r = list[i];
+    if (only[r]) probe_read(I, sk_hash, off, sk_n, probe_cnt, probe_start, r);
+  }
+}
 
 __global__ void __launch_bounds__(256) gather_hits_kernel(IndexView I, const uint64_t* __restrict__ off, const int32_t* __restrict__ sk_n,
                                                           const uint32_t* __restrict__ probe_cnt, const uint64_t* __restrict__ probe_start,
@@ -64,13 +78,13 @@
   static constexpr size_t LDS = (size_t)SLOTS * 4 + (size_t)THREADS * 8 + 16;
 };
 template <bool WRITE, int SLOT_BITS>
-__global__ void __launch_bounds__(HitFilterCfg<SLOT_BITS>::THREADS) hit_filter_kernel(IndexView I, const uint64_t* __restrict__ off, const int32_t* __restrict__ sk_n,
-                                                         const uint32_t* __restrict__ probe_cnt, const uint64_t* __restrict__ probe_start,
-                                                         const int32_t* __restrict__ read_len, const int32_t* __restrict__ min_hits,
-                                                         uint32_t* __restrict__ surv_n, const uint64_t* __restrict__ read_hit_off,
-                                                         uint64_t* __restrict__ hits, uint64_t* __restrict__ stage, const uint64_t* __restrict__ stage_off, int dbg,
-                                                         const uint8_t* __restrict__ cls ,
-                                                         uint32_t* __restrict__ raw_hits ) {
+__device__ __forceinline__ void hit_filter_read(const IndexView& I, const uint64_t* __restrict__ off, const int32_t* __restrict__ sk_n,
+                                                const uint32_t* __restrict__ probe_cnt, const uint64_t* __restrict__ probe_start,
+                                                const int32_t* __restrict__ read_len, const int32_t* __restrict__ min_hits,
+                                                uint32_t* __restrict__ surv_n, const uint64_t* __restrict__ read_hit_off,
+                                                uint64_t* __restrict__ hits, uint64_t* __restrict__ stage, const uint64_t* __restrict__ stage_off, int dbg,
+                                                const uint8_t* __restrict__ cls ,
+                                                uint32_t* __restrict__ raw_hits , const int r) {
   using Cfg = HitFilterCfg<SLOT_BITS>;
   constexpr int SLOTS = Cfg::SLOTS, THREADS = Cfg::THREADS, EPL = Cfg::EPL;
   constexpr bool NARROW = SLOT_BITS == HF_SLOT_BITS_NARROW;
@@ -79,7 +93,6 @@
   uint32_t* const good = cnt + SLOTS;
   uint32_t* const alive = good + THREADS;
   uint32_t& cursor = alive[THREADS];
-  const int r = blockIdx.x;
   const int my_cls = cls[r];
   if (!WRITE && my_cls != Cfg::CLS) return;
   if (WRITE && (my_cls == 2) != (Cfg::CLS == 2)) return;
@@ -196,6 +209,29 @@
     for (int i = threadIdx.x; i < SLOTS; i += THREADS) acc += cnt[i];
     for (int d = 32; d > 0; d >>= 1) acc += __shfl_xor(acc, d, 64);
     if ((threadIdx.x & 63) == 0 && acc) atomicAdd(&raw_hits[r], acc);
+  }
+}
+template <bool WRITE, int SLOT_BITS>
+__global__ void __launch_bounds__(HitFilterCfg<SLOT_BITS>::THREADS) hit_filter_kernel(IndexView I, const uint64_t* __restrict__ off, const int32_t* __restrict__ sk_n,
+                                                         const uint32_t* __restrict__ probe_cnt, const uint64_t* __restrict__ probe_start,
+                                                         const int32_t* __restrict__ read_len, const int32_t* __restrict__ min_hits,
+                                                         uint32_t* __restrict__ surv_n, const uint64_t* __restrict__ read_hit_off,
+                                                         uint64_t* __restrict__ hits, uint64_t* __restrict__ stage, const uint64_t* __restrict__ stage_off, int dbg,
+                                                         const uint8_t* __restrict__ cls, uint32_t* __restrict__ raw_hits) {
+  hit_filter_read<WRITE, SLOT_BITS>(I, off, sk_n, probe_cnt, probe_start, read_len, min_hits, surv_n, read_hit_off, hits, stage, stage_off, dbg, cls, raw_hits, (int)blockIdx.x);
+}
+template <bool WRITE, int SLOT_BITS>
+__global__ void __launch_bounds__(HitFilterCfg<SLOT_BITS>::THREADS) hit_filter_list_kernel(IndexView I, const uint64_t* __restrict__ off, const int32_t* __restrict__ sk_n,
+                                                         const uint32_t* __restrict__ probe_cnt, const uint64_t* __restrict__ probe_start,
+                                                         const int32_t* __restrict__ read_len, const int32_t* __restrict__ min_hits,
+                                                         uint32_t* __restrict__ surv_n, const uint64_t* __restrict__ read_hit_off,
+                                                         uint64_t* __restrict__ hits, uint64_t* __restrict__ stage, const uint64_t* __restrict__ stage_off, int dbg,
+                                                         const uint8_t* __restrict__ cls, uint32_t* __restrict__ raw_hits,
+                                                         const int32_t* __restrict__ list, const uint32_t* __restrict__ list_n) {
+  const uint32_t nl = *list_n;
+  for (uint32_t i = blockIdx.x; i < nl; i += gridDim.x) {
+    hit_filter_read<WRITE, SLOT_BITS>(I, off, sk_n, probe_cnt, probe_start, read_len, min_hits, surv_n, read_hit_off, hits, stage, stage_off, dbg, cls, raw_hits, list[i]);
+    __syncthreads();
   }
 }
 
@@ -227,6 +263,7 @@
                                                                         uint64_t* __restrict__ stage, const uint64_t* __restrict__ stage_off,
                                                                         uint8_t* need_old, const uint32_t* __restrict__ cls_words ,
                                                                         uint32_t* __restrict__ raw_hits, int n_reads, uint32_t* __restrict__ ticket,
+                                                                        int32_t* __restrict__ fb_list, uint32_t* __restrict__ fb_n ,
                                                                         unsigned long long* __restrict__ prof ) {
   extern __shared__ __align__(16) unsigned char sf_dyn[];
   SeedFilterStreamLds& L = *reinterpret_cast<SeedFilterStreamLds*>(sf_dyn);
@@ -360,7 +397,7 @@
       }
       lds_barrier();
       lapp(2);
-      if (L.fallback) { if (tid == 0) { need_old[r] = 1; surv_n[r] = 0; raw_hits[r] = 0; } }
+      if (L.fallback) { if (tid == 0) { need_old[r] = 1; surv_n[r] = 0; raw_hits[r] = 0; fb_list[atomicAdd(fb_n, 1u)] = r; } }
       else {
         load_hashes(s_next, o_next);
         {
@@ -455,7 +492,7 @@
         lds_barrier();
         lapp(5);
         const uint32_t n_s = L.cursor;
-        if (n_s > sv_cap) { if (tid == 0) { need_old[r] = 1; surv_n[r] = 0; raw_hits[r] = 0; } }
+        if (n_s > sv_cap) { if (tid == 0) { need_old[r] = 1; surv_n[r] = 0; raw_hits[r] = 0; fb_list[atomicAdd(fb_n, 1u)] = r; } }
         else {
           for (uint32_t j = tid; j < n_s; j += SF_THREADS) {
             const uint32_t e = sv[j], q = e >> 3;
@@ -463,7 +500,7 @@
             while ((uint32_t)L.coff8[li + 1] <= q) ++li;
             dst[j] = I.occ[((uint64_t)L.lstart8[li] << 3) + (uint64_t)(q - (uint32_t)L.coff8[li]) * 8u + (e & 7u)] & ~(uint64_t)(PW_DP | PW_DN);
           }
-          if (tid == 0) { surv_n[r] = n_s; raw_hits[r] = L.hraw; }
+          if (tid == 0) { surv_n[r] = n_s; raw_hits[r] = L.hraw; if (n_s == 1u || n_s > (uint32_t)HIT_SORT_LDS_MAX) fb_list[atomicAdd(fb_n, 1u)] = r; }
         }
       }
     }
@@ -485,13 +522,6 @@
   const uint64_t s0 = sb[blockIdx.x], n = se[blockIdx.x] - s0, d0 = db[blockIdx.x];
   for (uint64_t i = threadIdx.x; i < n; i += 256) dst[d0 + i] = src[s0 + i];
 }
-__global__ void __launch_bounds__(256) sum_u32_kernel(const uint32_t* __restrict__ v, int64_t n, unsigned long long* __restrict__ out) {
-  unsigned long long acc = 0;
-  for (int64_t i = (int64_t)blockIdx.x * 256 + threadIdx.x; i < n; i += (int64_t)gridDim.x * 256) acc += v[i];
-  for (int d = 32; d > 0; d >>= 1) acc += __shfl_xor(acc, d, 64);
-  if ((threadIdx.x & 63) == 0 && acc) atomicAdd(out, acc);
-}
-
 __global__ void __launch_bounds__(256) probed_list_hist_kernel(IndexView I, const uint32_t* __restrict__ sk_hash, const uint64_t* __restrict__ off,
                                                                const int32_t* __restrict__ sk_n, int nb, unsigned long long* __restrict__ hist) {
   const int r = blockIdx.x, s = sk_n[r];
diff --git a/metamaps_amd/csrc/mm_seq.hip b/metamaps_amd/csrc/mm_seq.hip
--- a/metamaps_amd/csrc/mm_seq.hip
+++ b/metamaps_amd/csrc/mm_seq.hip
@@ -21,7 +21,7 @@
 }
 
 void run_minimizers(mm_ctx* ctx, const mm_seqset* S, int k, int w, const std::vector<uint8_t>& active, bool want_rec_seq,
-                    MinimizerSet& out) {
+                    MinimizerSet& out, uint64_t* d_mbox) {
   MM_REQUIRE(S->frozen, MM_ERR_STATE, "sequence set not uploaded");
   MM_REQUIRE(k >= 1 && k <= MZ_MAX_K, MM_ERR_ARG, "k must be in [1,64]");
   MM_REQUIRE(w >= 1 && w <= MZ_MAX_W, MM_ERR_ARG, "window size must be in [1,4096]");
@@ -60,21 +60,24 @@
   DBuf<uint64_t> tout((size_t)ntiles + 1), tmp;
   bool single_pass = !want_rec_seq && (size_t)ntiles * MZ_STAGE * sizeof(Rec) <= ((size_t)6 << 30);
   DBuf<Rec> stage;
-  DBuf<int> d_ovf(1); d_ovf.zero(st);
+  DBuf<uint64_t> own_mbox;
+  if (!d_mbox) { own_mbox.alloc(2); own_mbox.zero(st); d_mbox = own_mbox.p; }
+  int* const d_ovf = reinterpret_cast<int*>(d_mbox + 1);
   if (single_pass) {
     stage.alloc((size_t)ntiles * MZ_STAGE);
     { const char* e = getenv("MM_MZ_DBG"); int v = e ? atoi(e) : 0; MM_HIP(hipMemcpyToSymbolAsync(HIP_SYMBOL(mz_dbg_stop), &v, sizeof v, 0, hipMemcpyHostToDevice, st)); }
-    minimizer_kernel<2><<<dim3((unsigned)ntiles), dim3(MZ_THREADS), lds, st>>>(V, d_tf.p, k, w, d_js.p, tcount.p, nullptr, stage.p, nullptr, d_ovf.p);
+    minimizer_kernel<2><<<dim3((unsigned)ntiles), dim3(MZ_THREADS), lds, st>>>(V, d_tf.p, k, w, d_js.p, tcount.p, nullptr, stage.p, nullptr, d_ovf);
   } else {
     minimizer_kernel<0><<<dim3((unsigned)ntiles), dim3(MZ_THREADS), lds, st>>>(V, d_tf.p, k, w, d_js.p, tcount.p, nullptr, nullptr, nullptr, nullptr);
   }
   MM_KERNEL_CHECK();
-  exclusive_scan_u32_u64(tcount.p, ntiles, tout.p, tmp, st);
-  uint64_t total = 0;
-  int h_ovf = 0;
-  MM_HIP(hipMemcpyAsync(&total, tout.p + ntiles, sizeof total, hipMemcpyDeviceToHost, st));
-  MM_HIP(hipMemcpyAsync(&h_ovf, d_ovf.p, sizeof h_ovf, hipMemcpyDeviceToHost, st));
-  MM_HIP(mm::stream_sync(st));
+  exclusive_scan_u32_u64(tcount.p, ntiles, tout.p, tmp, st, d_mbox);
+  static_assert(MB_MZ_TOTAL == 0 && MB_MZ_OVF == 8, "the pair is fetched as 16 bytes");
+  unsigned char* const h_mbox = ctx->mbox_host_ready();
+  MM_HIP(hipMemcpyAsync(h_mbox, d_mbox, 16, hipMemcpyDeviceToHost, st));
+  MM_HIP(mm::stream_sync(st));
+  const uint64_t total = *reinterpret_cast<const uint64_t*>(h_mbox + MB_MZ_TOTAL);
+  const int h_ovf = *reinterpret_cast<const int*>(h_mbox + MB_MZ_OVF);
   if (h_ovf) single_pass = false;
   out.total = (int64_t)total;
   out.rec.alloc((size_t)total);
```

Result: no change. 26.19 (median of 5 runs) (+1.3%).
